# AssafSinger94/dino-tracker

Hardware: AMD Instinct MI355X
Metric: query-points*frames/s (higher is better)
Workload: dtype mixed: fp16 ViT operands (one per value), f16 conv operands in Delta-DINO, f16 candidates + f32 deciders in the tracker; f32 accumulate; 1 GPU; 854x480x90 synthetic video (model res 854x476, 67x121 tokens, C=384), 1024 grid queries; 1 video(s) per step over 1 GPU(s); features=vit, mode=single, track_method=mfma, anchor_pairs=92091, correlation_maps_per_video=8380350, rccl_ranks=1, parallelism=video-parallel x1

## Files before the change

### dino_tracker_amd/_lib.py

```python
from __future__ import annotations

import ctypes
import os

_HERE = os.path.dirname(os.path.abspath(__file__))
LIB_PATH = os.path.join(_HERE, "csrc", "libdtk.so")

c_int, c_float, c_void_p, c_size_t = ctypes.c_int, ctypes.c_float, ctypes.c_void_p, ctypes.c_size_t


class Geom(ctypes.Structure):
    _fields_ = [("T", ctypes.c_int32), ("C", ctypes.c_int32), ("ph", ctypes.c_int32), ("pw", ctypes.c_int32),
                ("video_h", ctypes.c_int32), ("video_w", ctypes.c_int32), ("patch", ctypes.c_int32),
                ("stride", ctypes.c_int32), ("radius", ctypes.c_float)]

    @property
    def HW(self) -> int:
        return self.ph * self.pw


def make_geom(T: int, C: int, video_h: int, video_w: int, patch: int = 14, stride: int = 7, radius: float = 35.0) -> Geom:
    ph = 1 + (video_h - patch) // stride
    pw = 1 + (video_w - patch) // stride
    return Geom(T, C, ph, pw, video_h, video_w, patch, stride, radius)


class VitLayer(ctypes.Structure):
    _fields_ = [(n, c_void_p) for n in ("ln1_w", "ln1_b", "qkv_w", "qkv_b", "proj_w", "proj_b", "ls1", "ln2_w", "ln2_b",
                                        "fc1_w", "fc1_b", "fc2_w", "fc2_b", "ls2",
                                        "qkv_w_lo", "proj_w_lo", "fc1_w_lo", "fc2_w_lo")] + [("w_scale", ctypes.c_float)]


class VitModel(ctypes.Structure):
    _fields_ = [("D", ctypes.c_int32), ("heads", ctypes.c_int32), ("depth", ctypes.c_int32), ("patch", ctypes.c_int32),
                ("stride", ctypes.c_int32), ("ln_eps", ctypes.c_float), ("flags", ctypes.c_int32),
                ("patch_w", c_void_p), ("patch_b", c_void_p),
                ("cls_pos", c_void_p), ("pos", c_void_p), ("mean_std", c_void_p), ("layers", ctypes.POINTER(VitLayer)),
                ("frame_batch", ctypes.c_int32), ("overflow", c_void_p),
                ("tap_out", c_void_p), ("tap_mask", ctypes.c_uint64), ("tap_scale", ctypes.c_float),
                ("ffn", ctypes.c_int32), ("hidden", ctypes.c_int32)]


VIT_TILED_GEMMS, VIT_BF16, VIT_CHECK_RANGE, VIT_GEMM_WS_V1, VIT_ATTENTION_V4, VIT_GEMM_WIDE_V1, VIT_NO_LN_FUSION = 1, 2, 4, 16, 32, 64, 128
OPERAND_F16, OPERAND_BF16, OPERAND_ATTENTION_V4 = 0, 1, 0x2000
VIT_GEMM_QKV, VIT_GEMM_QKV_FACET, VIT_GEMM_PROJ, VIT_GEMM_FC1, VIT_GEMM_FC2 = 0, 1, 2, 3, 4
VIT_GEMM_FC1_SWIGLU, VIT_GEMM_FC2_SWIGLU = 5, 6
VIT_FFN_GELU, VIT_FFN_SWIGLU = 0, 1


class VitGemmArgs(ctypes.Structure):
    _fields_ = ([(n, ctypes.c_int32) for n in ("role", "D", "flags", "operand_type")] + [("rows", ctypes.c_int64)] +
                [("S", ctypes.c_int32), ("Sp", ctypes.c_int32), ("ln_eps", ctypes.c_float), ("w_scale", ctypes.c_float)] +
                [(n, c_void_p) for n in ("a", "a_lo", "w", "w_lo", "bias", "gamma", "q", "k", "vt", "q_lo", "k_lo", "vt_lo", "out",
                                         "out_lo", "out_f32", "x", "ln_x", "ln_w", "ln_b", "ln_out", "ovf")])


class TrackOpts(ctypes.Structure):
    _fields_ = [("method", ctypes.c_int32), ("normalized", ctypes.c_int32), ("round_sources", ctypes.c_int32),
                ("tier", ctypes.c_int32), ("emb_rows", ctypes.c_int32)]


ADAM_MAX_TENSORS, ADAM_MAX_GROUPS = 32, 4


class AdamArgs(ctypes.Structure):
    _fields_ = [("param", ctypes.c_void_p * ADAM_MAX_TENSORS), ("grad", ctypes.c_void_p * ADAM_MAX_TENSORS),
                ("exp_avg", ctypes.c_void_p * ADAM_MAX_TENSORS), ("exp_avg_sq", ctypes.c_void_p * ADAM_MAX_TENSORS),
                ("numel", ctypes.c_int64 * ADAM_MAX_TENSORS), ("group", ctypes.c_int32 * ADAM_MAX_TENSORS),
                ("step", ctypes.c_int32 * ADAM_MAX_TENSORS), ("n_tensors", ctypes.c_int32), ("lr", ctypes.c_double * ADAM_MAX_GROUPS),
                ("beta1", ctypes.c_double), ("beta2", ctypes.c_double), ("eps", ctypes.c_double)]


RAFT_SPLIT, RAFT_FP16 = 0, 1
RAFT_ACT_NONE, RAFT_ACT_RELU, RAFT_ACT_SIGMOID, RAFT_ACT_TANH = 0, 1, 2, 3
RAFT_NUM_CONVS = 48


class RaftConvDesc(ctypes.Structure):
    _fields_ = ([("w_hi", c_void_p), ("w_lo", c_void_p), ("bias", c_void_p)] +
                [(n, ctypes.c_int32) for n in ("cin", "cout", "kh", "kw", "stride", "pad_h", "pad_w")] + [("inv_wscale", c_float)])


class RaftConvArgs(ctypes.Structure):
    _fields_ = ([("conv", RaftConvDesc)] +
                [(n, ctypes.c_int32) for n in ("N", "H", "W", "mode", "act", "res_relu", "in_split", "reserved")] +
                [(n, c_void_p) for n in ("in_", "in2", "out", "res", "mul", "gate")] +
                [(n, ctypes.c_int64) for n in ("in_stride", "in2_stride", "out_stride", "res_stride", "mul_stride", "gate_stride")])


class RaftModel(ctypes.Structure):
    _fields_ = [("conv", RaftConvDesc * RAFT_NUM_CONVS)]


class TrackStats(ctypes.Structure):
    _fields_ = [("sources", ctypes.c_int32), ("whole_map_tier", ctypes.c_int32), ("exact_tier", ctypes.c_int32),
                ("syncs", ctypes.c_int32)]

    def as_dict(self):
        return {k: int(getattr(self, k)) for k, _ in self._fields_}


SIGNATURES = {
    "dtk_version": (c_int, []),
    "dtk_last_error": (ctypes.c_char_p, []),
    "dtk_profile_enable": (c_int, [c_int]),
    "dtk_profile_collect": (c_int, []),
    "dtk_profile_name": (ctypes.c_char_p, [c_int]),
    "dtk_profile_ms": (ctypes.c_double, [c_int]),
    "dtk_profile_launches": (ctypes.c_longlong, [c_int]),
    "dtk_pack_features": (c_int, [c_void_p, c_void_p, c_void_p, c_int, c_int, c_int, c_void_p]),
    "dtk_unpack_features": (c_int, [c_void_p, c_void_p, c_int, c_int, c_int, c_void_p]),
    "dtk_feature_norms": (c_int, [c_void_p, c_void_p, c_int, c_int, c_int, c_void_p]),
    "dtk_vit_workspace_bytes": (c_size_t, [ctypes.POINTER(VitModel), c_int, c_int, c_int]),
    "dtk_vit_forward": (c_int, [ctypes.POINTER(VitModel), c_void_p, c_int, c_int, c_int, c_void_p, c_void_p, c_void_p,
                                c_void_p, c_size_t, c_void_p]),
    "dtk_vit_attention": (c_int, [c_void_p, c_void_p, c_void_p, c_void_p, c_int, c_int, c_int, c_int, c_int, c_void_p]),
    "dtk_vit_attention_split": (c_int, [c_void_p] * 8 + [c_int, c_int, c_int, c_int, c_int, c_void_p]),
    "dtk_vit_gemm": (c_int, [ctypes.POINTER(VitGemmArgs), c_void_p]),
    "dtk_vit_gemm_split": (c_int, [ctypes.POINTER(VitGemmArgs), c_void_p]),
    "dtk_delta_dino_packed_floats": (c_size_t, [c_int, c_int]),
    "dtk_delta_dino_pack": (c_int, [c_int, c_int, c_void_p, c_void_p, c_void_p, c_void_p, c_void_p, c_void_p, c_float,
                                    c_void_p, c_void_p]),
    "dtk_delta_dino_workspace_bytes": (c_size_t, [ctypes.POINTER(Geom)]),
    "dtk_delta_dino_refine": (c_int, [ctypes.POINTER(Geom), c_void_p, c_void_p, ctypes.POINTER(c_void_p), c_void_p,
                                      c_void_p, c_int, c_int, c_void_p, c_size_t, c_void_p]),
    "dtk_delta_dino_refine_mode": (c_int, [ctypes.POINTER(Geom), c_void_p, c_void_p, ctypes.POINTER(c_void_p), c_void_p,
                                           c_void_p, c_int, c_int, c_int, c_void_p, c_size_t, c_void_p]),
    "dtk_sample_points": (c_int, [ctypes.POINTER(Geom), c_void_p, c_void_p, c_void_p, c_void_p, c_void_p, c_int, c_void_p]),
    "dtk_sample_grid": (c_int, [c_void_p, c_int, c_int, c_int, c_int, c_void_p, c_void_p, c_int, c_void_p]),
    "dtk_normalized_conv2d": (c_int, [c_void_p, c_void_p, c_void_p, c_void_p, c_int, c_int, c_int, c_int, c_int, c_int,
                                      c_void_p]),
    "dtk_corr_maps": (c_int, [ctypes.POINTER(Geom), c_void_p, c_void_p, c_void_p, c_void_p, c_void_p, c_void_p, c_void_p,
                              c_int, c_int, c_void_p]),
    "dtk_head_prepare": (c_int, [c_void_p, c_void_p, c_void_p, c_void_p, c_void_p, c_void_p]),
    "dtk_head_forward": (c_int, [ctypes.POINTER(Geom), c_void_p, c_void_p, c_void_p, c_int, c_int, c_void_p]),
    "dtk_head_forward_train": (c_int, [ctypes.POINTER(Geom), c_void_p, c_void_p, c_void_p, c_void_p, c_int, c_int, c_void_p]),
    "dtk_conv_split_weight_halves": (c_size_t, [c_int, c_int]),
    "dtk_conv_split_pack": (c_int, [c_void_p, c_int, c_int, c_int, c_void_p, c_void_p, c_void_p]),
    "dtk_conv_split_input": (c_int, [c_void_p, c_int, c_int, c_int, c_int, c_int, c_void_p, c_void_p, c_void_p, c_void_p]),
    "dtk_conv_split_run": (c_int, [c_void_p, c_void_p, c_void_p, c_void_p, c_void_p, c_int, c_int, c_int, c_int, c_int, c_int,
                                   c_int, c_int, c_void_p]),
    "dtk_conv_split_output": (c_int, [c_void_p, c_int, c_int, c_int, c_int, c_int, c_int, c_void_p, c_void_p, c_void_p]),
    "dtk_conv_wgrad_split_workspace_bytes": (c_size_t, [c_int, c_int, c_int, c_int, c_int, c_int]),
    "dtk_conv_wgrad_split": (c_int, [c_void_p, c_void_p, c_void_p, c_int, c_int, c_int, c_int, c_int, c_int, c_int, c_void_p,
                                     c_int, c_void_p, c_size_t, c_void_p]),
    "dtk_gemm_nt_f32_indexed": (c_int, [c_void_p, c_void_p, c_void_p, c_int, c_int, c_int, ctypes.c_int64, ctypes.c_int64,
                                        ctypes.c_int64, c_int, ctypes.c_int64, ctypes.c_int64, ctypes.c_int64, c_int, c_int,
                                        c_void_p, c_void_p, c_void_p, c_void_p, c_void_p]),
    "dtk_contrastive_workspace_bytes": (c_size_t, [c_int, c_int, c_int, c_int]),
    "dtk_contrastive_forward": (c_int, [c_void_p, c_void_p, c_void_p, ctypes.c_float, c_int, c_int, c_int, c_int, c_int, c_void_p,
                                        c_void_p, c_void_p, c_void_p, c_void_p, c_void_p]),
    "dtk_contrastive_backward": (c_int, [c_void_p, c_void_p, c_void_p, ctypes.c_float, c_int, c_int, c_int, c_int, c_int, c_void_p,
                                         c_void_p, c_void_p, c_void_p, c_void_p, c_void_p, c_void_p, c_void_p, c_size_t, c_void_p]),
    "dtk_emb_reg_forward": (c_int, [c_void_p, c_void_p, c_int, c_int, c_int, c_void_p, c_void_p, c_void_p]),
    "dtk_sample_bilinear_forward": (c_int, [c_void_p, c_void_p, c_void_p, ctypes.c_int32, ctypes.c_int32, ctypes.c_int32, ctypes.c_int32, ctypes.c_int32, c_void_p]),
    "dtk_sample_bilinear_backward": (c_int, [c_void_p, c_void_p, c_void_p, ctypes.c_int32, ctypes.c_int32, ctypes.c_int32, ctypes.c_int32, ctypes.c_int32, c_void_p]),
    "dtk_pow2_scale": (c_int, [c_void_p, ctypes.c_int64, c_void_p, c_void_p, c_void_p]),
    "dtk_adam_step": (c_int, [ctypes.POINTER(AdamArgs), c_void_p]),
    "dtk_adam_scalars": (c_int, [ctypes.POINTER(AdamArgs), ctypes.POINTER(ctypes.c_float)]),
    "dtk_adam_step_dev": (c_int, [ctypes.POINTER(AdamArgs), c_void_p, c_void_p]),
    "dtk_emb_reg_backward": (c_int, [c_void_p, c_void_p, c_void_p, c_void_p, c_int, c_int, c_int, c_void_p, c_void_p]),
    "dtk_corr_window_backward": (c_int, [ctypes.POINTER(Geom), c_void_p, c_void_p, c_void_p, c_void_p, c_void_p, c_void_p, c_void_p,
                                         c_void_p, c_void_p, c_int, c_void_p]),
    "dtk_head_backward": (c_int, [ctypes.POINTER(Geom), c_void_p, c_void_p, c_void_p, c_void_p, c_void_p, c_void_p, c_int, c_int,
                                  c_void_p]),
    "dtk_track_workspace_bytes": (c_size_t, [ctypes.POINTER(Geom), c_int, ctypes.POINTER(TrackOpts)]),
    "dtk_track": (c_int, [ctypes.POINTER(Geom), c_void_p, c_void_p, c_void_p, c_void_p, c_void_p, c_void_p, c_void_p,
                          c_void_p, c_void_p, c_int, c_void_p, ctypes.POINTER(TrackOpts), ctypes.POINTER(TrackStats),
                          c_void_p, c_size_t, c_void_p]),
    "dtk_argmax_cells": (c_int, [ctypes.POINTER(Geom), c_void_p, c_void_p, c_void_p, c_void_p, c_void_p, c_void_p, c_void_p,
                                 c_void_p, c_int, c_int, c_void_p, c_size_t, c_void_p]),
    "dtk_bb_nms_workspace_bytes": (c_size_t, [ctypes.POINTER(Geom), c_int]),
    "dtk_bb_nms": (c_int, [ctypes.POINTER(Geom), c_void_p, c_void_p, c_void_p, c_void_p, c_void_p, c_float, c_float, c_int,
                           c_void_p, c_void_p, c_int, c_void_p, c_size_t, c_void_p]),
    "dtk_traj_start_fg": (c_int, [c_void_p, c_int, c_int, c_void_p, c_int, c_int, c_int, c_void_p, c_void_p, c_void_p]),
    "dtk_nearest_traj_workspace_bytes": (c_size_t, [c_int, c_int, c_int, c_int]),
    "dtk_nearest_traj": (c_int, [c_void_p, c_int, c_int, c_int, c_int, c_float, c_float, c_void_p, c_void_p, c_size_t, c_void_p]),
    "dtk_of_filter_keep": (c_int, [c_void_p, c_int, c_int, c_void_p, c_int, c_int, c_float, c_float, c_void_p, c_void_p,
                                   c_void_p, c_void_p, c_int, c_void_p, c_void_p, c_void_p]),
    "dtk_feat_f16_bytes": (c_size_t, [ctypes.POINTER(Geom)]),
    "dtk_make_feat_f16": (c_int, [ctypes.POINTER(Geom), c_void_p, c_void_p, c_void_p, c_void_p]),
    "dtk_traj_cos_sims": (c_int, [c_void_p, c_void_p, c_void_p, c_int, c_int, c_int, c_void_p]),
    "dtk_build_anchor_sources": (c_int, [c_void_p, c_float, c_int, c_int, c_void_p, c_void_p, c_void_p, c_void_p,
                                         c_void_p, c_void_p, c_void_p, c_void_p, c_void_p]),
    "dtk_occlusion": (c_int, [c_void_p, c_void_p, c_void_p, c_void_p, c_void_p, c_float, c_float, c_void_p, c_int,
                              c_int, c_void_p]),
    "dtk_build_anchor_sources_needed": (c_int, [c_void_p, c_float, c_float, c_int, c_int, c_void_p, c_void_p, c_void_p,
                                                c_void_p, c_void_p, c_void_p, c_void_p, c_void_p, c_void_p]),
    "dtk_occlusion_needed": (c_int, [c_void_p, c_void_p, c_void_p, c_void_p, c_void_p, c_float, c_float, c_void_p, c_int,
                                     c_int, c_void_p]),
    "dtk_tapvid_counts": (c_int, [c_void_p, c_void_p, c_void_p, c_void_p, c_void_p, c_float, c_float, c_float, c_float,
                                  c_int, c_int, c_int, c_void_p, c_void_p]),
    "dtk_badja_counts": (c_int, [c_void_p, c_void_p, c_void_p, c_void_p, c_int, c_float, c_float, c_int, c_int, c_int, c_int, c_int,
                                 c_void_p, c_void_p, c_void_p]),
    "dtk_blurpool_forward": (c_int, [c_void_p, c_void_p, ctypes.c_int64, c_int, c_int, c_void_p]),
    "dtk_blurpool_backward": (c_int, [c_void_p, c_void_p, ctypes.c_int64, c_int, c_int, c_void_p]),
    "dtk_gemm_nt_f32": (c_int, [c_void_p, c_void_p, c_void_p, c_int, c_int, c_int, ctypes.c_int64, ctypes.c_int64, ctypes.c_int64,
                                c_int, ctypes.c_int64, ctypes.c_int64, ctypes.c_int64, c_int, c_int, c_void_p, c_void_p, c_void_p]),
    "dtk_im2col": (c_int, [c_void_p, c_void_p, c_int, c_int, c_int, c_int, c_int, c_int, c_int, c_int, c_int, c_int,
                           ctypes.c_int64, c_void_p]),
    "dtk_col2im": (c_int, [c_void_p, c_void_p, c_int, c_int, c_int, c_int, c_int, c_int, c_int, c_int, c_int, c_void_p]),
    "dtk_transpose_f32": (c_int, [c_void_p, c_void_p, ctypes.c_int64, ctypes.c_int64, c_int, c_void_p]),
    "dtk_resample2d_forward": (c_int, [c_void_p, c_void_p, ctypes.c_int64, c_int, c_int, c_int, c_int, c_void_p, c_void_p, c_void_p,
                                       c_void_p, c_void_p]),
    "dtk_resample2d_backward": (c_int, [c_void_p, c_void_p, ctypes.c_int64, c_int, c_int, c_int, c_int, c_void_p, c_void_p,
                                        c_void_p, c_void_p, c_void_p]),
    "dtk_batchnorm_workspace_bytes": (c_size_t, [c_int]),
    "dtk_batchnorm_train_forward": (c_int, [c_void_p, c_void_p, c_void_p, c_void_p, c_void_p, c_void_p, c_float, c_float,
                                            c_int, c_void_p, c_void_p, c_void_p, c_int, c_int, c_int, c_void_p, c_size_t,
                                            c_void_p]),
    "dtk_batchnorm_train_backward": (c_int, [c_void_p, c_void_p, c_void_p, c_void_p, c_void_p, c_void_p, c_int, c_void_p,
                                             c_void_p, c_void_p, c_void_p, c_int, c_int, c_int, c_void_p, c_size_t, c_void_p]),
    "dtk_pca_moments_workspace_bytes": (c_size_t, [ctypes.c_int64, c_int, ctypes.c_int64]),
    "dtk_pca_moments": (c_int, [c_void_p, ctypes.c_int64, c_int, c_int, ctypes.c_int64, c_void_p, c_void_p, c_void_p, c_size_t,
                                c_void_p]),
    "dtk_pca_project_workspace_bytes": (c_size_t, [ctypes.c_int64]),
    "dtk_pca_project": (c_int, [c_void_p, ctypes.c_int64, c_int, c_int, c_void_p, c_int, c_void_p, c_void_p, c_void_p, c_size_t,
                                c_void_p]),
    "dtk_fg_mask": (c_int, [c_void_p, c_int, c_int, c_void_p, c_float, c_int, c_int, c_int, c_int, c_int, c_int, c_void_p, c_void_p,
                            c_void_p]),
    "dtk_flow_pack": (c_int, [c_void_p, c_void_p, c_int, c_int, c_int, c_void_p]),
    "dtk_flow_cycle_masks": (c_int, [c_void_p, c_void_p, c_int, c_int, c_int, c_float, c_void_p, c_void_p]),
    "dtk_flow_traj_workspace_bytes": (c_size_t, [c_int, c_int, c_int]),
    "dtk_flow_traj_start": (c_int, [c_void_p, c_void_p, c_void_p, c_void_p, c_int, c_int, c_int, c_int, c_float, c_int, c_void_p,
                                    c_void_p, c_int, c_float, c_void_p, c_void_p, c_size_t, c_void_p]),
    "dtk_flow_traj_emit": (c_int, [c_int, c_int, c_int, c_int, c_int, c_int, c_void_p, c_void_p, c_void_p, c_size_t, c_void_p]),
    "dtk_render_prim_count": (ctypes.c_int64, [c_int, c_int, c_int, c_int]),
    "dtk_render_group_bytes": (c_size_t, [ctypes.c_int64, ctypes.c_int64, c_int, c_int, c_int]),
    "dtk_render_prims": (c_int, [c_void_p, c_void_p, c_void_p, c_void_p, c_int, c_int, c_int, c_int, c_int, c_int, c_int, c_int,
                                 c_float, c_float, c_int, c_void_p, c_void_p]),
    "dtk_render_pred_gt_prims": (c_int, [c_void_p, c_void_p, c_void_p, c_void_p, c_void_p, c_int, c_int, c_int, c_int, c_int,
                                         c_int, c_int, c_void_p, c_void_p]),
    "dtk_render_tile_counts": (c_int, [c_void_p, ctypes.c_int64, c_int, c_int, c_int, c_void_p, c_void_p]),
    "dtk_render_tile_keys": (c_int, [c_void_p, c_void_p, ctypes.c_int64, c_int, c_int, c_int, ctypes.c_int64, c_void_p, c_void_p]),
    "dtk_render_blend": (c_int, [c_void_p, c_void_p, ctypes.c_int64, c_void_p, ctypes.c_int64, c_void_p, c_int, c_int, c_int,
                                 c_void_p, c_void_p, c_void_p]),
    "dtk_resize_workspace_bytes": (c_size_t, [c_int, c_int, c_int, c_int, c_int, c_int, c_int, c_int]),
    "dtk_resize_u8": (c_int, [c_void_p, c_int, c_int, c_int, c_int, c_int, c_int, c_void_p, c_void_p, c_int, c_void_p, c_void_p, c_int,
                              c_void_p, c_int, c_int, c_void_p, c_void_p, c_size_t, c_void_p]),
    "dtk_raft_conv_packed_halves": (c_size_t, [c_int, c_int, c_int, c_int]),
    "dtk_raft_conv_pack": (c_int, [c_void_p, c_int, c_int, c_int, c_int, c_float, c_void_p, c_void_p, c_void_p]),
    "dtk_raft_conv": (c_int, [ctypes.POINTER(RaftConvArgs), c_void_p]),
    "dtk_raft_instance_norm_workspace_bytes": (c_size_t, [c_int, c_int, c_int, c_int]),
    "dtk_raft_instance_norm": (c_int, [c_void_p, c_void_p, c_void_p, c_int, c_int, c_int, c_int, c_float, c_int, c_void_p, c_size_t,
                                       c_void_p]),
    "dtk_raft_pyramid_floats": (c_size_t, [c_int, c_int, c_int]),
    "dtk_raft_corr_pyramid": (c_int, [c_void_p, c_void_p, c_int, c_int, c_int, c_int, c_int, c_void_p, c_void_p]),
    "dtk_raft_lookup": (c_int, [c_void_p, c_void_p, ctypes.c_int64, c_int, c_int, c_int, c_void_p, ctypes.c_int64, c_void_p]),
    "dtk_raft_upsample": (c_int, [c_void_p, ctypes.c_int64, c_void_p, c_int, c_int, c_int, c_void_p, c_void_p]),
    "dtk_raft_workspace_bytes": (c_size_t, [c_int, c_int, c_int]),
    "dtk_raft_forward": (c_int, [ctypes.POINTER(RaftModel), c_void_p, c_void_p, c_int, c_int, c_int, c_int, c_int, c_void_p, c_void_p,
                                 c_size_t, c_void_p]),
}

_LIB = None


def lib() -> ctypes.CDLL:
    global _LIB
    if _LIB is None:
        if not os.path.isfile(LIB_PATH):
            raise RuntimeError(
                f"{LIB_PATH} is missing: build the HIP extension first (python -c 'import __graft_entry__ as g; "
                "g.build()' or make -C dino_tracker_amd/csrc). There is no CPU fallback for the hot path.")
        handle = ctypes.CDLL(LIB_PATH)
        for name, (res, args) in SIGNATURES.items():
            fn = getattr(handle, name)
            fn.restype = res
            fn.argtypes = args
        _LIB = handle
    return _LIB


def check(rc: int) -> None:
    if rc != 0:
        raise RuntimeError(f"libdtk error {rc}: {lib().dtk_last_error().decode()}")
```

### dino_tracker_amd/csrc/vit.hip

```cpp
#include <stdlib.h>
#include "common.h"
#include "vit_attention4.h"
#include "vit_attention6.h"
#include "vit_gemm_common.h"
#include "vit_gemm_tiled.h"
#include "vit_gemm_ws.h"
#include "vit_gemm_ws_ln.h"
#include "vit_gemm_wide.h"
#include "vit_split.h"

namespace {

__global__ __launch_bounds__(256) void patch_embed_kernel(const float* __restrict__ frames, const float* __restrict__ Wp,
                                                          const float* __restrict__ bp, const float* __restrict__ pos,
                                                          const float* __restrict__ cls_pos,
                                                          const float* __restrict__ mean_std, float* __restrict__ x,
                                                          int H, int W, int ph, int pw, int D, int patch, int stride,
                                                          int S) {
    const int HW = ph * pw;
    const int K = 3 * patch * patch;
    const int frame = blockIdx.z;
    const int tid = threadIdx.x, lane = tid & 63, w = tid >> 6;
    const int p0 = blockIdx.x * 64 + (w >> 1) * 32;
    const int n0 = blockIdx.y * 64 + (w & 1) * 32;
    const int li = lane & 31, lk = lane >> 5;
    const float* img = frames + (size_t)frame * 3 * H * W;
    const int p = min(p0 + li, HW - 1);
    const int pr = p / pw, pc = p % pw;
    const int n = min(n0 + li, D - 1);
    const float* wrow = Wp + (size_t)n * K;
    f16v acc;
#pragma unroll
    for (int r = 0; r < 16; ++r) acc[r] = 0.f;
    for (int k = lk; k < K; k += 2) {
        const int ch = k / (patch * patch), rem = k - ch * patch * patch;
        const int ky = rem / patch, kx = rem - ky * patch;
        const float px = img[((size_t)ch * H + pr * stride + ky) * W + pc * stride + kx];
        const float a = (px - mean_std[ch]) / mean_std[3 + ch];
        acc = __builtin_amdgcn_mfma_f32_32x32x2f32(a, wrow[k], acc, 0, 0, 0);
    }
    const int co = n0 + li;
    if (co < D) {
        const float b = bp[co];
#pragma unroll
        for (int r = 0; r < 16; ++r) {
            const int i = (r & 3) + 8 * (r >> 2) + 4 * lk;
            const int pp = p0 + i;
            if (pp < HW) x[((size_t)frame * S + 1 + pp) * D + co] = acc[r] + b + pos[(size_t)pp * D + co];
        }
    }
    if (blockIdx.x == 0 && (w >> 1) == 0 && lk == 0 && co < D) x[(size_t)frame * S * D + co] = cls_pos[co];
}

constexpr int PE_P = 14, PE_S = 7, PE_TOK = 128, PE_NF = 96;
constexpr int PE_ROWPX = (PE_TOK - 1) * PE_S + PE_P;
constexpr int PE_K = PE_P * PE_P * 4;
constexpr int PE_CK = 2 * PE_P * 4;
constexpr int PE_WP = PE_CK + 8;
constexpr float PE_WSCALE = 256.f;

__global__ __launch_bounds__(256) void frame_split4_kernel(const float* __restrict__ frames, const float* __restrict__ mean_std,
                                                           h4v* __restrict__ hi_, h4v* __restrict__ lo_, int H, int W,
                                                           long long npix) {
    const long long i = (long long)blockIdx.x * 256 + threadIdx.x;
    if (i >= npix) return;
    const long long f = i / ((long long)H * W), p = i - f * (long long)H * W;
    const float* fr = frames + f * 3 * (long long)H * W + p;
    h4v h, l;
#pragma unroll
    for (int c = 0; c < 3; ++c) {
        const float v = (fr[(long long)c * H * W] - mean_std[c]) / mean_std[3 + c];
        h[c] = (half_t)v;
        l[c] = (half_t)(v - (float)h[c]);
    }
    h[3] = (half_t)0.f;
    l[3] = (half_t)0.f;
    hi_[i] = h;
    lo_[i] = l;
}

__global__ void pack_patch_split_kernel(const float* __restrict__ w, int D, half_t* __restrict__ Wh, half_t* __restrict__ Wl) {
    const long long idx = (long long)blockIdx.x * 256 + threadIdx.x;
    if (idx >= (long long)D * PE_K) return;
    const int n = (int)(idx / PE_K), k = (int)(idx - (long long)n * PE_K);
    const int tap = k >> 2, c = k & 3;
    const float v = c < 3 ? w[((size_t)n * 3 + c) * (PE_P * PE_P) + tap] * PE_WSCALE : 0.f;
    const half_t h = (half_t)v;
    Wh[idx] = h;
    Wl[idx] = (half_t)(v - (float)h);
}

__global__ __launch_bounds__(256) void patch_embed_split_kernel(const h4v* __restrict__ in_hi, const h4v* __restrict__ in_lo,
                                                                const half_t* __restrict__ Wh, const half_t* __restrict__ Wl,
                                                                const float* __restrict__ bp, const float* __restrict__ pos,
                                                                const float* __restrict__ cls_pos, float* __restrict__ x,
                                                                int H, int W, int ph, int pw, int D, int S, int groups_x,
                                                                int units, int slabs) {
    __shared__ h4v Xh[2 * PE_ROWPX], Xl[2 * PE_ROWPX];
    __shared__ __attribute__((aligned(16))) half_t Wsh[PE_NF * PE_WP], Wsl[PE_NF * PE_WP];
    const int tid = threadIdx.x, lane = tid & 63, w = tid >> 6;
    const int per_xcd = (units + 7) / 8;
    const int within = blockIdx.x >> 3;
    const int unit = (blockIdx.x & 7) * per_xcd + within / slabs;
    if (within / slabs >= per_xcd || unit >= units) return;
    const int n0 = (within % slabs) * PE_NF;
    const int pc0 = (unit % groups_x) * PE_TOK, pr = (unit / groups_x) % ph;
    const size_t frame = unit / (groups_x * ph);
    const int li = lane & 31, hh = lane >> 5;
    const h4v* fh = in_hi + frame * (size_t)H * W;
    const h4v* fl = in_lo + frame * (size_t)H * W;
    const int tokl = w * 32 + li;
    f16v acc[3];
#pragma unroll
    for (int n = 0; n < 3; ++n)
#pragma unroll
        for (int r = 0; r < 16; ++r) acc[n][r] = 0.f;
    for (int c = 0; c < PE_P / 2; ++c) {
        __syncthreads();
        for (int idx = tid; idx < 2 * PE_ROWPX; idx += 256) {
            const int r = idx / PE_ROWPX, px = idx - r * PE_ROWPX;
            const size_t g = (size_t)(pr * PE_S + 2 * c + r) * W + min(pc0 * PE_S + px, W - 1);
            Xh[idx] = fh[g];
            Xl[idx] = fl[g];
        }
        for (int idx = tid; idx < PE_NF * (PE_CK / 8); idx += 256) {
            const int f = idx / (PE_CK / 8), piece = idx - f * (PE_CK / 8);
            const size_t src = (size_t)min(n0 + f, D - 1) * PE_K + c * PE_CK + piece * 8;
            *reinterpret_cast<uint4*>(Wsh + f * PE_WP + piece * 8) = *reinterpret_cast<const uint4*>(Wh + src);
            *reinterpret_cast<uint4*>(Wsl + f * PE_WP + piece * 8) = *reinterpret_cast<const uint4*>(Wl + src);
        }
        __syncthreads();
#pragma unroll
        for (int ls = 0; ls < PE_CK / 16; ++ls) {
            const int t0 = 2 * (2 * ls + hh);
            const int p0 = (t0 / PE_P) * PE_ROWPX + tokl * PE_S + t0 % PE_P;
            const h4v a0 = Xh[p0], a1 = Xh[p0 + 1], b0 = Xl[p0], b1 = Xl[p0 + 1];
            const h8 xh = {a0[0], a0[1], a0[2], a0[3], a1[0], a1[1], a1[2], a1[3]};
            const h8 xl = {b0[0], b0[1], b0[2], b0[3], b1[0], b1[1], b1[2], b1[3]};
#pragma unroll
            for (int n = 0; n < 3; ++n) {
                const int wo = (n * 32 + li) * PE_WP + ls * 16 + hh * 8;
                const h8 wh = *reinterpret_cast<const h8*>(Wsh + wo), wl = *reinterpret_cast<const h8*>(Wsl + wo);
                acc[n] = __builtin_amdgcn_mfma_f32_32x32x16_f16(xl, wh, acc[n], 0, 0, 0);
                acc[n] = __builtin_amdgcn_mfma_f32_32x32x16_f16(xh, wl, acc[n], 0, 0, 0);
                acc[n] = __builtin_amdgcn_mfma_f32_32x32x16_f16(xh, wh, acc[n], 0, 0, 0);
            }
        }
    }
#pragma unroll
    for (int n = 0; n < 3; ++n) {
        const int co = n0 + n * 32 + li;
        if (co >= D) continue;
        const float b = bp[co];
#pragma unroll
        for (int r = 0; r < 16; ++r) {
            const int pc = pc0 + w * 32 + (r & 3) + 8 * (r >> 2) + 4 * hh;
            if (pc < pw) {
                const int pp = pr * pw + pc;
                x[((size_t)frame * S + 1 + pp) * D + co] = acc[n][r] * (1.f / PE_WSCALE) + b + pos[(size_t)pp * D + co];
            }
        }
        if (pr == 0 && pc0 == 0 && w == 0 && hh == 0) x[(size_t)frame * S * D + co] = cls_pos[co];
    }
}

template <typename T, int NIT = 4>
__global__ __launch_bounds__(256) void layernorm_kernel(float* __restrict__ x, const T* __restrict__ delta,
                                                        const float* __restrict__ gam, const float* __restrict__ bet,
                                                        T* __restrict__ y, long long rows, int D, float eps,
                                                        int* __restrict__ overflow) {
    typedef typename Vec<T>::t8 T8;
    typedef typename Vec<T>::t4 T4;
    (void)sizeof(T8); (void)sizeof(T4);
    operand_mode<T>();
    const long long row = (long long)blockIdx.x * 4 + (threadIdx.x >> 6);
    if (row >= rows) return;
    const int lane = threadIdx.x & 63;
    float* p = x + row * D;
    float4 v[NIT];
    float s = 0.f;
    bool sat = false;
#pragma unroll
    for (int it = 0; it < NIT; ++it) {
        const int c = lane * 4 + it * 256;
        if (c < D) {
            v[it] = *reinterpret_cast<const float4*>(p + c);
            if (delta) {
                const T4 d = *reinterpret_cast<const T4*>(delta + row * D + c);
                const float d0 = (float)d[0], d1 = (float)d[1], d2 = (float)d[2], d3 = (float)d[3];
                if (IsF16<T>::value) sat |= !(fmaxf(fmaxf(fabsf(d0), fabsf(d1)), fmaxf(fabsf(d2), fabsf(d3))) < 65504.f);
                v[it].x += d0; v[it].y += d1; v[it].z += d2; v[it].w += d3;
                *reinterpret_cast<float4*>(p + c) = v[it];
            }
            s += (v[it].x + v[it].y) + (v[it].z + v[it].w);
        }
    }
    if (IsF16<T>::value && overflow && __any(sat) && lane == 0) atomicOr(overflow, 1);
    const float mean = wave_sum(s) / (float)D;
    float q = 0.f;
#pragma unroll
    for (int it = 0; it < NIT; ++it) {
        if (lane * 4 + it * 256 < D) {
            const float a = v[it].x - mean, b = v[it].y - mean, cc = v[it].z - mean, d = v[it].w - mean;
            q += (a * a + b * b) + (cc * cc + d * d);
        }
    }
    const float rstd = rsqrtf(wave_sum(q) / (float)D + eps);
    if (!y) return;
    T* o = y + row * D;
#pragma unroll
    for (int it = 0; it < NIT; ++it) {
        const int c = lane * 4 + it * 256;
        if (c < D) {
            const float4 g = *reinterpret_cast<const float4*>(gam + c), b = *reinterpret_cast<const float4*>(bet + c);
            T4 r = {(T)((v[it].x - mean) * rstd * g.x + b.x), (T)((v[it].y - mean) * rstd * g.y + b.y),
                     (T)((v[it].z - mean) * rstd * g.z + b.z), (T)((v[it].w - mean) * rstd * g.w + b.w)};
            *reinterpret_cast<T4*>(o + c) = r;
        }
    }
}

__global__ __launch_bounds__(256) void zero_kernel(uint4* __restrict__ p, long long n16) {
    const long long i = (long long)blockIdx.x * 256 + threadIdx.x;
    if (i < n16) p[i] = make_uint4(0, 0, 0, 0);
}

template <typename T>
__global__ __launch_bounds__(256) void final_update_kernel(const float* __restrict__ x, const T* __restrict__ delta,
                                                           float* __restrict__ tokens_out, float* __restrict__ feat_out, int S, int D,
                                                           long long total4, int* __restrict__ overflow) {
    typedef typename Vec<T>::t4 T4;
    const long long i = (long long)blockIdx.x * 256 + threadIdx.x;
    bool sat = false;
    if (i < total4) {
        const int d4 = D / 4;
        const long long row = i / d4;
        const int c = (int)(i - row * d4);
        const long long f = row / S, s = row - f * S;
        float4 v = reinterpret_cast<const float4*>(x)[i];
        const T4 d = reinterpret_cast<const T4*>(delta)[i];
        const float d0 = (float)d[0], d1 = (float)d[1], d2 = (float)d[2], d3 = (float)d[3];
        if (IsF16<T>::value) sat = !(fmaxf(fmaxf(fabsf(d0), fabsf(d1)), fmaxf(fabsf(d2), fabsf(d3))) < 65504.f);
        v.x += d0; v.y += d1; v.z += d2; v.w += d3;
        if (tokens_out) reinterpret_cast<float4*>(tokens_out)[i] = v;
        if (feat_out && s > 0) reinterpret_cast<float4*>(feat_out)[(f * (S - 1) + s - 1) * d4 + c] = v;
    }
    if (IsF16<T>::value && overflow && __any(sat) && (threadIdx.x & 63) == 0) atomicOr(overflow, 1);
}

template <typename T>
__global__ __launch_bounds__(256) void tap_kernel(const float* __restrict__ x, const T* __restrict__ delta, float* __restrict__ out,
                                                  float scale, long long total4) {
    typedef typename Vec<T>::t4 T4;
    const long long i = (long long)blockIdx.x * 256 + threadIdx.x;
    if (i >= total4) return;
    float4 v = reinterpret_cast<const float4*>(x)[i];
    if (delta) {
        const T4 d = reinterpret_cast<const T4*>(delta)[i];
        v.x += (float)d[0]; v.y += (float)d[1]; v.z += (float)d[2]; v.w += (float)d[3];
    }
    float4 o = reinterpret_cast<float4*>(out)[i];
    o.x += scale * v.x; o.y += scale * v.y; o.z += scale * v.z; o.w += scale * v.w;
    reinterpret_cast<float4*>(out)[i] = o;
}

__global__ __launch_bounds__(256) void drop_cls_kernel(const float* __restrict__ x, float* __restrict__ out, int S, int D,
                                                       long long total4) {
    const long long i = (long long)blockIdx.x * 256 + threadIdx.x;
    if (i >= total4) return;
    const int d4 = D / 4;
    const long long row = i / d4;
    const int c = (int)(i - row * d4);
    const long long f = row / (S - 1), s = row - f * (S - 1);
    reinterpret_cast<float4*>(out)[i] = reinterpret_cast<const float4*>(x)[(f * S + 1 + s) * d4 + c];
}

constexpr int VIT_FRAME_BATCH = 90;

struct VitPlan {
    int S, Sp, FB;
    size_t x, xn, q, k, vt, ao, hid, delta, total;
    bool split;
    size_t xn_lo, q_lo, k_lo, vt_lo, ao_lo, hid_lo;
};

inline bool vit_layer_split(const dtk_vit_layer& L) { return L.qkv_w_lo != nullptr; }

VitPlan vit_plan(const dtk_vit_model* m, int ph, int pw, int frames) {
    VitPlan p;
    p.S = ph * pw + 1;
    p.Sp = (p.S + 127) / 128 * 128;
    const int fb = m->frame_batch > 0 ? m->frame_batch : VIT_FRAME_BATCH;
    p.FB = frames < fb ? frames : fb;
    auto al = [](size_t v) { return (v + 255) & ~(size_t)255; };
    size_t off = 0;
    const size_t rows = (size_t)p.FB * p.S;
    p.x = off; off = al(off + rows * m->D * 4);
    p.xn = off; off = al(off + rows * m->D * 2);
    p.q = off; off = al(off + (size_t)p.FB * m->heads * p.Sp * 64 * 2);
    p.k = off; off = al(off + (size_t)p.FB * m->heads * p.Sp * 64 * 2);
    p.vt = off; off = al(off + (size_t)p.FB * m->heads * p.Sp * 64 * 2);
    p.ao = off; off = al(off + rows * m->D * 2);
    p.hid = off; off = al(off + rows * 4 * m->D * 2);
    p.delta = off; off = al(off + rows * m->D * 2);
    p.split = false;
    for (int l = 0; l < m->depth; ++l) p.split |= vit_layer_split(m->layers[l]);
    p.xn_lo = p.q_lo = p.k_lo = p.vt_lo = p.ao_lo = p.hid_lo = 0;
    if (p.split) {
        p.xn_lo = off; off = al(off + rows * m->D * 2);
        p.q_lo = off; off = al(off + (size_t)p.FB * m->heads * p.Sp * 64 * 2);
        p.k_lo = off; off = al(off + (size_t)p.FB * m->heads * p.Sp * 64 * 2);
        p.vt_lo = off; off = al(off + (size_t)p.FB * m->heads * p.Sp * 64 * 2);
        p.ao_lo = off; off = al(off + rows * m->D * 2);
        p.hid_lo = off; off = al(off + rows * 4 * m->D * 2);
    }
    p.total = off;
    return p;
}

template <typename T>
int attention_launch(const T* q, const T* k, const T* vt, T* o, int S, int Sp, int heads, int D, int FH, bool v4, hipStream_t st) {
    int QB;
    if (v4) {
        const unsigned grid = attn::attention_grid(FH, S, 256, &QB);
        DTK_LAUNCH("vit_attention", (attn::attention4_kernel<T, 0>), dim3(grid), dim3(256), 0, st, q, k, vt, o, S, Sp, heads, D,
                   FH, QB);
    } else {
        const unsigned grid = attn::attention_grid(FH, S, 128 * attn::A6_NQ, &QB);
        DTK_LAUNCH("vit_attention", (attn::attention6_kernel<T, 0>), dim3(grid), dim3(256), 0, st, q, k, vt, o, S, Sp, heads, D,
                   FH, QB);
    }
    return DTK_OK;
}

template <typename T>
__global__ __launch_bounds__(256) void range_scan_kernel(const T* __restrict__ p, long long n8, int* __restrict__ flag, int bit) {
    typedef typename Vec<T>::t8 T8;
    bool bad = false;
    for (long long i = (long long)blockIdx.x * 256 + threadIdx.x; i < n8; i += (long long)gridDim.x * 256) {
        const T8 v = reinterpret_cast<const T8*>(p)[i];
#pragma unroll
        for (int e = 0; e < 8; ++e) bad |= !(fabsf((float)v[e]) < 65504.f);
    }
    if (__any(bad) && (threadIdx.x & 63) == 0) atomicOr(flag, bit);
}

constexpr int VIT_MAX_D = 1536;
template <typename T>
int launch_layernorm(float* x, const T* delta, const float* gam, const float* bet, T* y, long long rows, int D, float eps, int* ovf,
                     hipStream_t st) {
    if (D <= 1024)
        DTK_LAUNCH("vit_layernorm", (layernorm_kernel<T, 4>), dim3(dtk_cdiv(rows, 4)), dim3(256), 0, st, x, delta, gam, bet, y, rows, D, eps, ovf);
    else
        DTK_LAUNCH("vit_layernorm", (layernorm_kernel<T, 6>), dim3(dtk_cdiv(rows, 4)), dim3(256), 0, st, x, delta, gam, bet, y, rows, D, eps, ovf);
    return DTK_OK;
}
template <typename T>
int launch_layernorm_split(float* x, const T* delta, const float* gam, const float* bet, T* y_hi, T* y_lo, long long rows, int D,
                           float eps, int* ovf, hipStream_t st) {
    if (D <= 1024)
        DTK_LAUNCH("vit_layernorm_split", (layernorm_split_kernel<T, 4>), dim3(dtk_cdiv(rows, 4)), dim3(256), 0, st, x, delta, gam, bet, y_hi,
                   y_lo, rows, D, eps, ovf);
    else
        DTK_LAUNCH("vit_layernorm_split", (layernorm_split_kernel<T, 6>), dim3(dtk_cdiv(rows, 4)), dim3(256), 0, st, x, delta, gam, bet, y_hi,
                   y_lo, rows, D, eps, ovf);
    return DTK_OK;
}

struct GemmPath {
    bool tiled;
    bool ws;
    bool wide;
    bool ws_v1;
    bool wide_v1;
    bool fc2_ln;
    bool proj_ln;
};
inline GemmPath gemm_path(int D, int f) {
    const bool tiled = (f & DTK_VIT_TILED_GEMMS) != 0, ws = !tiled && D == WS_K, wide_v1 = (f & DTK_VIT_GEMM_WIDE_V1) != 0;
    static_assert(WS_K == WD_N, "fc2 of the weight-stationary width is gemm_wide_delta_kernel's shape");
    const bool ws_v1 = (f & DTK_VIT_GEMM_WS_V1) != 0, fc2_ln = ws && !wide_v1 && !(f & DTK_VIT_NO_LN_FUSION);
    return {tiled, ws, !tiled && D % W2_N == 0, ws_v1, wide_v1, fc2_ln, fc2_ln && !ws_v1};
}
inline GemmPath gemm_path(const dtk_vit_model* m) { return gemm_path(m->D, m->flags); }

template <typename T, int EPI>
int launch_gemm(const char* name, const GemmPath& path, const T* A, const T* W, long long rows, int N, int K, const GemmEpi<T>& e,
                hipStream_t st) {
    if constexpr (EPI != EPI_F32) {
        const bool ws_fits = EPI != EPI_QKV || e.S >= WS_ROWS || rows <= e.S;
        if constexpr (EPI == EPI_DELTA) {
            if (path.ws && K == WS_K && N == WS_K && e.ln_out) {
                const auto gr = gemm_ws_ln_grid(rows);
                DTK_LAUNCH(name, (gemm_ws_ln_kernel<T>), gr.first, dim3(256), 0, st, A, W, rows, e, gr.second);
                return DTK_OK;
            }
        }
        if (path.ws && K == WS_K && ws_fits) {
            const auto gr = gemm_ws_grid(N, rows);
            if (path.ws_v1)
                DTK_LAUNCH(name, (gemm_ws_kernel<T, EPI, 0>), gr.first, dim3(256), 0, st, A, W, rows, N, e, gr.second);
            else if (N % 64 != 0 || DTK_DBG(e.no_store, 128))
                DTK_LAUNCH(name, (gemm_ws_kernel<T, EPI, 3, false>), gr.first, dim3(256), 0, st, A, W, rows, N, e, gr.second);
            else
                DTK_LAUNCH(name, (gemm_ws_kernel<T, EPI>), gr.first, dim3(256), 0, st, A, W, rows, N, e, gr.second);
            return DTK_OK;
        }
        if (path.ws && EPI == EPI_DELTA) {
            const dim3 grid(dtk_cdiv(rows, WD_M));
            if (path.wide_v1)
                DTK_LAUNCH(name, (gemm_wide_delta_kernel<T, false>), grid, dim3(512), 0, st, A, W, rows, K, e);
            else if (e.ln_out)
                DTK_LAUNCH(name, (gemm_wide_delta_kernel<T, true, true>), grid, dim3(512), 0, st, A, W, rows, K, e);
            else
                DTK_LAUNCH(name, (gemm_wide_delta_kernel<T, true>), grid, dim3(512), 0, st, A, W, rows, K, e);
            return DTK_OK;
        }
        if (path.wide) {
            const dim3 grid(gemm_wide_grid(N, rows));
            if (path.wide_v1)
                DTK_LAUNCH(name, (gemm_wide_kernel<T, EPI, false>), grid, dim3(512), 0, st, A, W, rows, N, K, e);
            else
                DTK_LAUNCH(name, (gemm_wide_kernel<T, EPI, true>), grid, dim3(512), 0, st, A, W, rows, N, K, e);
            return DTK_OK;
        }
    }
    DTK_LAUNCH(name, (gemm_tiled_kernel<T, EPI>), dim3(gemm_grid(N, rows)), dim3(256), 0, st, A, W, rows, N, K, e);
    return DTK_OK;
}

template <typename T>
int launch_gemm_swiglu(const char* name, const GemmPath& path, const T* A, const T* W, long long rows, int N, int K, const GemmEpi<T>& e,
                       hipStream_t st) {
    if (path.wide)
        DTK_LAUNCH(name, (gemm_wide_kernel<T, EPI_SWIGLU, true>), dim3(gemm_wide_grid(N, rows)), dim3(512), 0, st, A, W, rows, N, K, e);
    else
        DTK_LAUNCH(name, (gemm_tiled_kernel<T, EPI_SWIGLU>), dim3(gemm_grid(N, rows)), dim3(256), 0, st, A, W, rows, N, K, e);
    return DTK_OK;
}
inline bool vit_swiglu_flags_ok(int flags, const char* who) {
    if (!(flags & (DTK_VIT_GEMM_WIDE_V1 | DTK_VIT_GEMM_WS_V1))) return true;
    dtk_set_error("%s: the SwiGLU feed-forward has no A / B kernel forms: clear %s", who,
                  (flags & DTK_VIT_GEMM_WIDE_V1) ? "DTK_VIT_GEMM_WIDE_V1" : "DTK_VIT_GEMM_WS_V1");
    return false;
}

template <typename T, int SEPI>
int launch_gemm_split(const char* name, const GemmPath& path, const T* Ah, const T* Al, const T* Wh, const T* Wl, long long rows,
                      int N, int K, const SplitEpi<T>& se, hipStream_t st) {
    if (!path.tiled && N % SD_N == 0) {
        const dim3 grid(gemm_split_dma_grid(N, rows));
        if constexpr (SEPI == SEPI_SWIGLU)
            DTK_LAUNCH(name, (gemm_split_dma_kernel<T, SEPI, true>), grid, dim3(512), 0, st, Ah, Al, Wh, Wl, rows, N, K, se);
        else if (path.wide_v1)
            DTK_LAUNCH(name, (gemm_split_dma_kernel<T, SEPI, false>), grid, dim3(512), 0, st, Ah, Al, Wh, Wl, rows, N, K, se);
        else
            DTK_LAUNCH(name, (gemm_split_dma_kernel<T, SEPI, true>), grid, dim3(512), 0, st, Ah, Al, Wh, Wl, rows, N, K, se);
        return DTK_OK;
    }
    DTK_LAUNCH(name, (gemm_split_kernel<T, SEPI>), dim3(gemm_split_grid(N, rows)), dim3(256), 0, st, Ah, Al, Wh, Wl, rows, N, K, se);
    return DTK_OK;
}

template <typename T>
int vit_run(const dtk_vit_model* m, const float* frames, int nframes, int video_h, int video_w, float* tokens_out,
            float* feat_out, float* qkv_out, unsigned char* ws, const VitPlan& p, int ph, int pw, hipStream_t st) {
    const int HW = ph * pw, D = m->D;
    const bool swiglu = m->ffn == DTK_VIT_FFN_SWIGLU;
    const int HID = m->hidden > 0 ? m->hidden : 4 * D;
    float* x = reinterpret_cast<float*>(ws + p.x);
    auto at = [&](size_t off) { return reinterpret_cast<T*>(ws + off); };
    T *xn = at(p.xn), *q = at(p.q), *k = at(p.k), *vt = at(p.vt), *ao = at(p.ao), *hid = at(p.hid), *delta = at(p.delta);
    T *xn_lo = at(p.xn_lo), *q_lo = at(p.q_lo), *k_lo = at(p.k_lo), *vt_lo = at(p.vt_lo), *ao_lo = at(p.ao_lo), *hid_lo = at(p.hid_lo);
    int* ovf = m->overflow;
    const bool scan_all = ovf && (m->flags & DTK_VIT_CHECK_RANGE);
    int* const epi_ovf = IsF16<T>::value ? ovf : nullptr;
    const int S = p.S, Sp = p.Sp;
    {
        const long long n16 = (long long)((p.ao - p.q) / 16);
        DTK_LAUNCH("vit_zero", zero_kernel, dim3(dtk_cdiv(n16, 256)), dim3(256), 0, st, reinterpret_cast<uint4*>(q), n16);
        if (p.split) {
            const long long m16 = (long long)((p.ao_lo - p.q_lo) / 16);
            DTK_LAUNCH("vit_zero", zero_kernel, dim3(dtk_cdiv(m16, 256)), dim3(256), 0, st, reinterpret_cast<uint4*>(q_lo), m16);
        }
    }
    for (int f0 = 0; f0 < nframes; f0 += p.FB) {
        const int nf = (nframes - f0) < p.FB ? (nframes - f0) : p.FB;
        const long long rows = (long long)nf * S;
        auto scan_range = [&](const T* t, long long n, int bit) -> int {
            const int blocks = (int)(dtk_cdiv(n / 8, 256) < 1024 ? dtk_cdiv(n / 8, 256) : 1024);
            DTK_LAUNCH("vit_range_scan", range_scan_kernel<T>, dim3(blocks), dim3(256), 0, st, t, n / 8, ovf, bit);
            return DTK_OK;
        };
        const bool pe_fits = (size_t)nf * video_h * video_w * 16 <= p.delta - p.hid &&
                             (size_t)D * PE_K * 4 <= p.total - p.delta;
        if (m->patch == PE_P && m->stride == PE_S && pe_fits) {
            h4v* fh = reinterpret_cast<h4v*>(hid);
            h4v* fl = fh + (size_t)nf * video_h * video_w;
            half_t* wh = reinterpret_cast<half_t*>(delta);
            half_t* wl = wh + (size_t)D * PE_K;
            const long long npix = (long long)nf * video_h * video_w;
            DTK_LAUNCH("vit_frame_split", frame_split4_kernel, dim3(dtk_cdiv(npix, 256)), dim3(256), 0, st,
                       frames + (size_t)f0 * 3 * video_h * video_w, m->mean_std, fh, fl, video_h, video_w, npix);
            DTK_LAUNCH("vit_frame_split", pack_patch_split_kernel, dim3(dtk_cdiv((long long)D * PE_K, 256)), dim3(256), 0, st,
                       m->patch_w, D, wh, wl);
            const int groups_x = dtk_cdiv(pw, PE_TOK);
            const int units = groups_x * ph * nf, slabs = dtk_cdiv(D, PE_NF);
            DTK_LAUNCH("vit_patch_embed", patch_embed_split_kernel, dim3(8 * dtk_cdiv(units, 8) * slabs), dim3(256), 0, st, fh,
                       fl, wh, wl, m->patch_b, m->pos, m->cls_pos, x, video_h, video_w, ph, pw, D, S, groups_x, units, slabs);
        } else {
            DTK_LAUNCH("vit_patch_embed", patch_embed_kernel, dim3(dtk_cdiv(HW, 64), dtk_cdiv(D, 64), nf), dim3(256), 0, st,
                       frames + (size_t)f0 * 3 * video_h * video_w, m->patch_w, m->patch_b, m->pos, m->cls_pos, m->mean_std,
                       x, video_h, video_w, ph, pw, D, m->patch, m->stride, S);
        }
        const GemmPath path = gemm_path(m);
        const int dbg_ns = DTK_DBG(dtk_dev_flags() >> 16, 0xff);
        bool pending = false;
        bool ln1_done = false;
        auto tap = [&](int l, bool with_delta) -> int {
            if (!m->tap_out || !((m->tap_mask >> l) & 1)) return DTK_OK;
            const long long t4 = rows * (D / 4);
            DTK_LAUNCH("vit_tap", tap_kernel<T>, dim3(dtk_cdiv(t4, 256)), dim3(256), 0, st, x, with_delta ? (const T*)delta : (const T*)nullptr,
                       m->tap_out + (size_t)f0 * S * D, m->tap_scale, t4);
            return DTK_OK;
        };
        for (int l = 0; l < m->depth; ++l) {
            const dtk_vit_layer& L = m->layers[l];
            const T* qkv_w = reinterpret_cast<const T*>(L.qkv_w);
            const T* proj_w = reinterpret_cast<const T*>(L.proj_w);
            const T* fc1_w = reinterpret_cast<const T*>(L.fc1_w);
            const T* fc2_w = reinterpret_cast<const T*>(L.fc2_w);
            if (vit_layer_split(L)) {
                const T* qkv_wl = reinterpret_cast<const T*>(L.qkv_w_lo);
                const T* proj_wl = reinterpret_cast<const T*>(L.proj_w_lo);
                const T* fc1_wl = reinterpret_cast<const T*>(L.fc1_w_lo);
                const T* fc2_wl = reinterpret_cast<const T*>(L.fc2_w_lo);
                const float inv_ws = 1.f / (L.w_scale > 0.f ? L.w_scale : 1.f);
                if (launch_layernorm_split<T>(x, pending ? (const T*)delta : (const T*)nullptr, L.ln1_w, L.ln1_b, xn, xn_lo, rows, D, m->ln_eps,
                                              ovf, st)) return DTK_E_HIP;
                pending = false;
                SplitEpi<T> se{};
                if (qkv_out && l == m->depth - 1) {
                    se.bias = L.qkv_b; se.inv_wscale = inv_ws; se.out_f32 = qkv_out + (size_t)f0 * S * 3 * D;
                    if (launch_gemm_split<T, SEPI_F32>("vit_gemm_qkv_facet", path, xn, xn_lo, qkv_w, qkv_wl, rows, 3 * D, D, se, st)) return DTK_E_HIP;
                    se = SplitEpi<T>{};
                }
                se.bias = L.qkv_b; se.inv_wscale = inv_ws; se.q_hi = q; se.q_lo = q_lo; se.k_hi = k; se.k_lo = k_lo; se.vt_hi = vt;
                se.vt_lo = vt_lo; se.S = S; se.Sp = Sp; se.heads = m->heads; se.D = D; se.qscale = 0.125f * 1.4426950408889634f;
                se.ovf = epi_ovf;
                if (launch_gemm_split<T, SEPI_QKV>("vit_gemm_qkv_split", path, xn, xn_lo, qkv_w, qkv_wl, rows, 3 * D, D, se, st)) return DTK_E_HIP;
                const int nqb = dtk_cdiv(Sp, 128);
                DTK_LAUNCH("vit_attention_split", attention_split_kernel<T>, dim3((unsigned)(nf * m->heads * nqb)), dim3(256), 0, st,
                           (const T*)q, (const T*)q_lo, (const T*)k, (const T*)k_lo, (const T*)vt, (const T*)vt_lo, ao, ao_lo, S, Sp,
                           m->heads, nqb);
                se = SplitEpi<T>{};
                se.bias = L.proj_b; se.inv_wscale = inv_ws; se.x = x; se.gamma = L.ls1;
                if (launch_gemm_split<T, SEPI_RESID>("vit_gemm_proj_split", path, ao, ao_lo, proj_w, proj_wl, rows, D, D, se, st)) return DTK_E_HIP;
                if (launch_layernorm_split<T>(x, (const T*)nullptr, L.ln2_w, L.ln2_b, xn, xn_lo, rows, D, m->ln_eps, ovf, st)) return DTK_E_HIP;
                se = SplitEpi<T>{};
                se.bias = L.fc1_b; se.inv_wscale = inv_ws; se.out_hi = hid; se.out_lo = hid_lo; se.ovf = epi_ovf;
                if (swiglu ? launch_gemm_split<T, SEPI_SWIGLU>("vit_gemm_fc1_split", path, xn, xn_lo, fc1_w, fc1_wl, rows, 2 * HID, D, se, st)
                           : launch_gemm_split<T, SEPI_GELU>("vit_gemm_fc1_split", path, xn, xn_lo, fc1_w, fc1_wl, rows, HID, D, se, st)) return DTK_E_HIP;
                se = SplitEpi<T>{};
                se.bias = L.fc2_b; se.inv_wscale = inv_ws; se.x = x; se.gamma = L.ls2;
                if (launch_gemm_split<T, SEPI_RESID>("vit_gemm_fc2_split", path, hid, hid_lo, fc2_w, fc2_wl, rows, D, HID, se, st)) return DTK_E_HIP;
                if (tap(l, false)) return DTK_E_HIP;
                continue;
            }
            GemmEpi<T> e{};
            if (!ln1_done && launch_layernorm<T>(x, pending ? (const T*)delta : (const T*)nullptr, L.ln1_w, L.ln1_b, xn, rows, D, m->ln_eps, ovf, st))
                return DTK_E_HIP;
            ln1_done = false;
            pending = true;
            if (qkv_out && l == m->depth - 1) {
                e.bias = L.qkv_b; e.out_f32 = qkv_out + (size_t)f0 * S * 3 * D;
                if (launch_gemm<T, EPI_F32>("vit_gemm_qkv_facet", path, xn, qkv_w, rows, 3 * D, D, e, st)) return DTK_E_HIP;
                e = GemmEpi<T>{};
            }
            e.bias = L.qkv_b; e.q = q; e.k = k; e.vt = vt; e.S = S; e.Sp = Sp; e.heads = m->heads; e.D = D;
            e.qscale = 0.125f * 1.4426950408889634f; e.no_store = dbg_ns; e.ovf = epi_ovf;
            if (launch_gemm<T, EPI_QKV>("vit_gemm_qkv", path, xn, qkv_w, rows, 3 * D, D, e, st)) return DTK_E_HIP;
            if (scan_all && scan_range(q, (long long)(p.ao - p.q) / 2, 2)) return DTK_E_HIP;
            if (attention_launch(q, k, vt, ao, S, Sp, m->heads, D, nf * m->heads, (m->flags & DTK_VIT_ATTENTION_V4) != 0, st)) return DTK_E_HIP;
            e = GemmEpi<T>{};
            e.bias = L.proj_b; e.delta = delta; e.gamma = L.ls1; e.no_store = dbg_ns;
            if (path.proj_ln) { e.ln_x = x; e.ln_w = L.ln2_w; e.ln_b = L.ln2_b; e.ln_out = xn; e.ln_eps = m->ln_eps; e.ln_ovf = ovf; }
            if (launch_gemm<T, EPI_DELTA>("vit_gemm_proj", path, ao, proj_w, rows, D, D, e, st)) return DTK_E_HIP;
            if (!path.proj_ln && launch_layernorm<T>(x, (const T*)delta, L.ln2_w, L.ln2_b, xn, rows, D, m->ln_eps, ovf, st)) return DTK_E_HIP;
            e = GemmEpi<T>{};
            e.bias = L.fc1_b; e.out = hid; e.no_store = dbg_ns; e.ovf = epi_ovf;
            if (swiglu ? launch_gemm_swiglu<T>("vit_gemm_fc1", path, xn, fc1_w, rows, 2 * HID, D, e, st)
                       : launch_gemm<T, EPI_GELU>("vit_gemm_fc1", path, xn, fc1_w, rows, HID, D, e, st)) return DTK_E_HIP;
            if (scan_all && scan_range(hid, rows * HID, 4)) return DTK_E_HIP;
            e = GemmEpi<T>{};
            e.bias = L.fc2_b; e.delta = delta; e.gamma = L.ls2; e.no_store = dbg_ns;
            if (path.fc2_ln && l + 1 < m->depth && !vit_layer_split(m->layers[l + 1])) {
                const dtk_vit_layer& Ln = m->layers[l + 1];
                e.ln_x = x; e.ln_w = Ln.ln1_w; e.ln_b = Ln.ln1_b; e.ln_out = xn; e.ln_eps = m->ln_eps; e.ln_ovf = ovf;
                pending = false;
                ln1_done = true;
            }
            if (launch_gemm<T, EPI_DELTA>("vit_gemm_fc2", path, hid, fc2_w, rows, D, HID, e, st)) return DTK_E_HIP;
            if (tap(l, pending)) return DTK_E_HIP;
        }
        if (pending && (tokens_out || feat_out)) {
            const long long t4 = rows * (D / 4);
            DTK_LAUNCH("vit_final_update", final_update_kernel<T>, dim3(dtk_cdiv(t4, 256)), dim3(256), 0, st, x, (const T*)delta,
                       tokens_out ? tokens_out + (size_t)f0 * S * D : (float*)nullptr,
                       feat_out ? feat_out + (size_t)f0 * HW * D : (float*)nullptr, S, D, t4, ovf);
        } else {
            if (pending &&
                launch_layernorm<T>(x, (const T*)delta, (const float*)nullptr, (const float*)nullptr, (T*)nullptr, rows, D, m->ln_eps, ovf, st))
                return DTK_E_HIP;
            if (tokens_out)
                DTK_HIP(hipMemcpyAsync(tokens_out + (size_t)f0 * S * D, x, (size_t)rows * D * sizeof(float),
                                       hipMemcpyDeviceToDevice, st));
            if (feat_out) {
                const long long total4 = (long long)nf * HW * (D / 4);
                DTK_LAUNCH("vit_drop_cls", drop_cls_kernel, dim3(dtk_cdiv(total4, 256)), dim3(256), 0, st, x,
                           feat_out + (size_t)f0 * HW * D, S, D, total4);
            }
        }
    }
    return DTK_OK;
}

constexpr int VITG_HIDDEN = 4096;
int vit_gemm_check(const dtk_vit_gemm_args* g, const char* who, bool split, int* N, int* K) {
    DTK_REQUIRE(g, "%s: null pointer", who);
    DTK_REQUIRE(g->D == 384 || g->D == 768 || g->D == 1024 || g->D == 1536, "%s: D must be 384, 768 or 1024, or ViT-g's 1536 (got %d)", who, g->D);
    DTK_REQUIRE(g->operand_type == DTK_OPERAND_F16 || g->operand_type == DTK_OPERAND_BF16, "%s: operand_type", who);
    DTK_REQUIRE(g->rows > 0 && g->rows < (1ll << 31), "%s: rows", who);
    DTK_REQUIRE(g->a && g->w && (!split || (g->a_lo && g->w_lo)), "%s: null operand", who);
    const int D = g->D;
    switch (g->role) {
        case DTK_VIT_GEMM_QKV:
            *N = 3 * D; *K = D;
            DTK_REQUIRE(g->q && g->k && g->vt && (!split || (g->q_lo && g->k_lo && g->vt_lo)), "%s: QKV needs q, k and vt", who);
            DTK_REQUIRE(g->S > 0 && g->Sp >= g->S && g->Sp % 64 == 0 && g->rows % g->S == 0,
                        "%s: bad sizes (Sp %% 64 == 0, Sp >= S, rows a multiple of S)", who);
            break;
        case DTK_VIT_GEMM_QKV_FACET:
            *N = 3 * D; *K = D;
            DTK_REQUIRE(g->out_f32, "%s: QKV_FACET needs out_f32", who);
            break;
        case DTK_VIT_GEMM_FC1:
            *N = 4 * D; *K = D;
            DTK_REQUIRE(g->out && (!split || g->out_lo), "%s: FC1 needs out", who);
            break;
        case DTK_VIT_GEMM_PROJ:
        case DTK_VIT_GEMM_FC2:
            *N = D; *K = g->role == DTK_VIT_GEMM_FC2 ? 4 * D : D;
            DTK_REQUIRE(g->gamma && (split ? g->x != nullptr : g->out != nullptr), "%s: PROJ / FC2 need gamma and %s", who, split ? "x" : "out");
            break;
        case DTK_VIT_GEMM_FC1_SWIGLU:
        case DTK_VIT_GEMM_FC2_SWIGLU:
            DTK_REQUIRE(D == 1536, "%s: the SwiGLU roles are ViT-g's, D = 1536 (got %d)", who, D);
            if (!vit_swiglu_flags_ok(g->flags, who)) return DTK_E_INVALID;
            if (g->role == DTK_VIT_GEMM_FC1_SWIGLU) {
                *N = 2 * VITG_HIDDEN; *K = D;
                DTK_REQUIRE(g->out && (!split || g->out_lo), "%s: FC1_SWIGLU needs out", who);
            } else {
                *N = D; *K = VITG_HIDDEN;
                DTK_REQUIRE(g->gamma && (split ? g->x != nullptr : g->out != nullptr), "%s: FC2_SWIGLU needs gamma and %s", who, split ? "x" : "out");
            }
            break;
        default:
            DTK_REQUIRE(false, "%s: unknown role %d", who, g->role);
    }
    return DTK_OK;
}

template <typename T>
int vit_gemm_stage(const dtk_vit_gemm_args* g, int N, int K, hipStream_t st) {
    const GemmPath path = gemm_path(g->D, g->flags);
    const T *A = reinterpret_cast<const T*>(g->a), *W = reinterpret_cast<const T*>(g->w);
    int* const epi_ovf = IsF16<T>::value ? g->ovf : nullptr;
    GemmEpi<T> e{};
    e.bias = g->bias;
    switch (g->role) {
        case DTK_VIT_GEMM_QKV:
            e.q = reinterpret_cast<T*>(g->q); e.k = reinterpret_cast<T*>(g->k); e.vt = reinterpret_cast<T*>(g->vt);
            e.S = g->S; e.Sp = g->Sp; e.heads = g->D / 64; e.D = g->D; e.qscale = 0.125f * 1.4426950408889634f; e.ovf = epi_ovf;
            return launch_gemm<T, EPI_QKV>("vit_gemm_qkv", path, A, W, g->rows, N, K, e, st);
        case DTK_VIT_GEMM_QKV_FACET:
            e.out_f32 = g->out_f32;
            return launch_gemm<T, EPI_F32>("vit_gemm_qkv_facet", path, A, W, g->rows, N, K, e, st);
        case DTK_VIT_GEMM_FC1:
            e.out = reinterpret_cast<T*>(g->out); e.ovf = epi_ovf;
            return launch_gemm<T, EPI_GELU>("vit_gemm_fc1", path, A, W, g->rows, N, K, e, st);
        case DTK_VIT_GEMM_FC1_SWIGLU:
            e.out = reinterpret_cast<T*>(g->out); e.ovf = epi_ovf;
            return launch_gemm_swiglu<T>("vit_gemm_fc1", path, A, W, g->rows, N, K, e, st);
        default:
            e.delta = reinterpret_cast<T*>(g->out); e.gamma = g->gamma;
            if (g->ln_out) {
                DTK_REQUIRE(g->role == DTK_VIT_GEMM_PROJ ? path.proj_ln : path.fc2_ln,
                            "dtk_vit_gemm: the fused LayerNorm is fc2's or the projection's at D = 384 without TILED_GEMMS / GEMM_WIDE_V1 / NO_LN_FUSION (the projection's: nor GEMM_WS_V1)");
                DTK_REQUIRE(g->ln_x && g->ln_w && g->ln_b, "dtk_vit_gemm: the fused LayerNorm needs ln_x, ln_w and ln_b");
                e.ln_x = g->ln_x; e.ln_w = g->ln_w; e.ln_b = g->ln_b; e.ln_out = reinterpret_cast<T*>(g->ln_out); e.ln_eps = g->ln_eps;
                e.ln_ovf = g->ovf;
            }
            return launch_gemm<T, EPI_DELTA>(g->role == DTK_VIT_GEMM_PROJ ? "vit_gemm_proj" : "vit_gemm_fc2", path, A, W, g->rows, N, K, e, st);
    }
}

template <typename T>
int vit_gemm_split_stage(const dtk_vit_gemm_args* g, int N, int K, hipStream_t st) {
    const GemmPath path = gemm_path(g->D, g->flags);
    const T *Ah = reinterpret_cast<const T*>(g->a), *Al = reinterpret_cast<const T*>(g->a_lo);
    const T *Wh = reinterpret_cast<const T*>(g->w), *Wl = reinterpret_cast<const T*>(g->w_lo);
    int* const epi_ovf = IsF16<T>::value ? g->ovf : nullptr;
    SplitEpi<T> se{};
    se.bias = g->bias; se.inv_wscale = 1.f / (g->w_scale > 0.f ? g->w_scale : 1.f);
    switch (g->role) {
        case DTK_VIT_GEMM_QKV:
            se.q_hi = reinterpret_cast<T*>(g->q); se.q_lo = reinterpret_cast<T*>(g->q_lo); se.k_hi = reinterpret_cast<T*>(g->k);
            se.k_lo = reinterpret_cast<T*>(g->k_lo); se.vt_hi = reinterpret_cast<T*>(g->vt); se.vt_lo = reinterpret_cast<T*>(g->vt_lo);
            se.S = g->S; se.Sp = g->Sp; se.heads = g->D / 64; se.D = g->D; se.qscale = 0.125f * 1.4426950408889634f; se.ovf = epi_ovf;
            return launch_gemm_split<T, SEPI_QKV>("vit_gemm_qkv_split", path, Ah, Al, Wh, Wl, g->rows, N, K, se, st);
        case DTK_VIT_GEMM_QKV_FACET:
            se.out_f32 = g->out_f32;
            return launch_gemm_split<T, SEPI_F32>("vit_gemm_qkv_facet", path, Ah, Al, Wh, Wl, g->rows, N, K, se, st);
        case DTK_VIT_GEMM_FC1:
            se.out_hi = reinterpret_cast<T*>(g->out); se.out_lo = reinterpret_cast<T*>(g->out_lo); se.ovf = epi_ovf;
            return launch_gemm_split<T, SEPI_GELU>("vit_gemm_fc1_split", path, Ah, Al, Wh, Wl, g->rows, N, K, se, st);
        case DTK_VIT_GEMM_FC1_SWIGLU:
            se.out_hi = reinterpret_cast<T*>(g->out); se.out_lo = reinterpret_cast<T*>(g->out_lo); se.ovf = epi_ovf;
            return launch_gemm_split<T, SEPI_SWIGLU>("vit_gemm_fc1_split", path, Ah, Al, Wh, Wl, g->rows, N, K, se, st);
        default:
            se.x = g->x; se.gamma = g->gamma;
            return launch_gemm_split<T, SEPI_RESID>(g->role == DTK_VIT_GEMM_PROJ ? "vit_gemm_proj_split" : "vit_gemm_fc2_split", path, Ah, Al,
                                                    Wh, Wl, g->rows, N, K, se, st);
    }
}

constexpr int VIT_KNOWN_FLAGS = DTK_VIT_TILED_GEMMS | DTK_VIT_BF16 | DTK_VIT_CHECK_RANGE | DTK_VIT_GEMM_WS_V1 | DTK_VIT_ATTENTION_V4 |
                                DTK_VIT_GEMM_WIDE_V1 | DTK_VIT_NO_LN_FUSION;

}

extern "C" size_t dtk_vit_workspace_bytes(const dtk_vit_model* m, int video_h, int video_w, int frames) {
    if (!m || frames <= 0) return 0;
    const int ph = 1 + (video_h - m->patch) / m->stride, pw = 1 + (video_w - m->patch) / m->stride;
    return vit_plan(m, ph, pw, frames).total;
}

extern "C" int dtk_vit_forward(const dtk_vit_model* m, const float* frames, int nframes, int video_h, int video_w,
                               float* tokens_out, float* feat_out, float* qkv_out, void* workspace,
                               size_t workspace_bytes, void* stream) {
    DTK_REQUIRE(m && frames && workspace && (tokens_out || feat_out || qkv_out || m->tap_out), "dtk_vit_forward: null pointer");
    DTK_REQUIRE(!(m->flags & ~VIT_KNOWN_FLAGS), "dtk_vit_forward: unknown flag bits 0x%x (bit 8 selected a kernel that left the library)",
                (unsigned)(m->flags & ~VIT_KNOWN_FLAGS));
    DTK_REQUIRE(!qkv_out || m->depth > 0, "dtk_vit_forward: qkv_out needs at least one block");
    DTK_REQUIRE(m->D > 0 && m->heads > 0 && m->D == m->heads * 64, "dtk_vit_forward: d_head must be 64 (D=%d heads=%d)",
                m->D, m->heads);
    DTK_REQUIRE(m->D % 32 == 0 && m->depth >= 0 && m->layers, "dtk_vit_forward: bad model");
    DTK_REQUIRE(m->D <= VIT_MAX_D, "dtk_vit_forward: D = %d: the LayerNorm kernels hold rows of at most %d channels", m->D, VIT_MAX_D);
    if (m->ffn == DTK_VIT_FFN_SWIGLU) {
        DTK_REQUIRE(m->D == 1536 && m->hidden == VITG_HIDDEN, "dtk_vit_forward: the SwiGLU feed-forward is ViT-g's: D = 1536, hidden = %d (got D = %d, hidden = %d)",
                    VITG_HIDDEN, m->D, m->hidden);
        if (!vit_swiglu_flags_ok(m->flags, "dtk_vit_forward")) return DTK_E_INVALID;
    } else {
        DTK_REQUIRE(m->ffn == DTK_VIT_FFN_GELU, "dtk_vit_forward: unknown ffn %d", m->ffn);
        DTK_REQUIRE(m->hidden == 0 || m->hidden == 4 * m->D, "dtk_vit_forward: a GELU MLP has hidden = 4 D (got %d)", m->hidden);
    }
    DTK_REQUIRE(video_h >= m->patch && video_w >= m->patch, "dtk_vit_forward: frame smaller than a patch");
    const int ph = 1 + (video_h - m->patch) / m->stride, pw = 1 + (video_w - m->patch) / m->stride;
    const VitPlan p = vit_plan(m, ph, pw, nframes);
    if (workspace_bytes < p.total) {
        dtk_set_error("dtk_vit_forward: workspace %zu B < required %zu B", workspace_bytes, p.total);
        return DTK_E_WORKSPACE;
    }
    hipStream_t st = dtk_stream(stream);
    unsigned char* ws = reinterpret_cast<unsigned char*>(workspace);
    if (m->flags & DTK_VIT_BF16)
        return vit_run<__bf16>(m, frames, nframes, video_h, video_w, tokens_out, feat_out, qkv_out, ws, p, ph, pw, st);
    return vit_run<_Float16>(m, frames, nframes, video_h, video_w, tokens_out, feat_out, qkv_out, ws, p, ph, pw, st);
}

extern "C" int dtk_vit_attention(const void* q, const void* k, const void* vt, void* out, int frames, int heads, int S,
                                 int Sp, int operand_type, void* stream) {
    DTK_REQUIRE(q && k && vt && out, "dtk_vit_attention: null pointer");
    DTK_REQUIRE(frames > 0 && heads > 0 && S > 0 && Sp >= S && Sp % 64 == 0, "dtk_vit_attention: bad sizes (Sp %% 64 == 0, Sp >= S)");
    const bool v4 = (operand_type & DTK_OPERAND_ATTENTION_V4) != 0;
    operand_type &= ~DTK_OPERAND_ATTENTION_V4;
    DTK_REQUIRE(operand_type == DTK_OPERAND_F16 || operand_type == DTK_OPERAND_BF16, "dtk_vit_attention: operand_type");
    if (operand_type == DTK_OPERAND_BF16)
        return attention_launch(reinterpret_cast<const __bf16*>(q), reinterpret_cast<const __bf16*>(k),
                                reinterpret_cast<const __bf16*>(vt), reinterpret_cast<__bf16*>(out), S, Sp, heads, heads * 64,
                                frames * heads, v4, dtk_stream(stream));
    return attention_launch(reinterpret_cast<const _Float16*>(q), reinterpret_cast<const _Float16*>(k),
                            reinterpret_cast<const _Float16*>(vt), reinterpret_cast<_Float16*>(out), S, Sp, heads, heads * 64,
                            frames * heads, v4, dtk_stream(stream));
}

extern "C" int dtk_vit_attention_split(const void* q_hi, const void* q_lo, const void* k_hi, const void* k_lo, const void* vt_hi,
                                       const void* vt_lo, void* out_hi, void* out_lo, int frames, int heads, int S, int Sp,
                                       int operand_type, void* stream) {
    DTK_REQUIRE(q_hi && q_lo && k_hi && k_lo && vt_hi && vt_lo && out_hi && out_lo, "dtk_vit_attention_split: null pointer");
    DTK_REQUIRE(frames > 0 && heads > 0 && S > 0 && Sp >= S && Sp % 64 == 0, "dtk_vit_attention_split: bad sizes (Sp %% 64 == 0, Sp >= S)");
    DTK_REQUIRE(operand_type == DTK_OPERAND_F16 || operand_type == DTK_OPERAND_BF16, "dtk_vit_attention_split: operand_type");
    hipStream_t st = dtk_stream(stream);
    const int nqb = dtk_cdiv(Sp, 128);
    const unsigned grid = (unsigned)(frames * heads * nqb);
    if (operand_type == DTK_OPERAND_BF16) {
        typedef __bf16 T;
        DTK_LAUNCH("vit_attention_split", attention_split_kernel<T>, dim3(grid), dim3(256), 0, st, (const T*)q_hi, (const T*)q_lo,
                   (const T*)k_hi, (const T*)k_lo, (const T*)vt_hi, (const T*)vt_lo, (T*)out_hi, (T*)out_lo, S, Sp, heads, nqb);
    } else {
        typedef _Float16 T;
        DTK_LAUNCH("vit_attention_split", attention_split_kernel<T>, dim3(grid), dim3(256), 0, st, (const T*)q_hi, (const T*)q_lo,
                   (const T*)k_hi, (const T*)k_lo, (const T*)vt_hi, (const T*)vt_lo, (T*)out_hi, (T*)out_lo, S, Sp, heads, nqb);
    }
    return DTK_OK;
}


extern "C" int dtk_vit_gemm(const dtk_vit_gemm_args* g, void* stream) {
    int N = 0, K = 0;
    if (const int rc = vit_gemm_check(g, "dtk_vit_gemm", false, &N, &K)) return rc;
    if (g->operand_type == DTK_OPERAND_BF16) return vit_gemm_stage<__bf16>(g, N, K, dtk_stream(stream));
    return vit_gemm_stage<_Float16>(g, N, K, dtk_stream(stream));
}

extern "C" int dtk_vit_gemm_split(const dtk_vit_gemm_args* g, void* stream) {
    int N = 0, K = 0;
    if (const int rc = vit_gemm_check(g, "dtk_vit_gemm_split", true, &N, &K)) return rc;
    DTK_REQUIRE(!g->ln_out, "dtk_vit_gemm_split: the split blocks have their own LayerNorm");
    if (g->operand_type == DTK_OPERAND_BF16) return vit_gemm_split_stage<__bf16>(g, N, K, dtk_stream(stream));
    return vit_gemm_split_stage<_Float16>(g, N, K, dtk_stream(stream));
}
```

### dino_tracker_amd/csrc/vit_attention6.h

```cpp
#pragma once
#include "vit_attention_common.h"

namespace attn {

constexpr int A6_NQ = 4;

template <typename T>
__device__ __forceinline__ void a6_s_first(f16v& acc, const typename Operand<T>::v8& a, const typename Operand<T>::v8& b,
                                           const f16v& c) {
    if constexpr (Operand<T>::F16) asm volatile("v_mfma_f32_32x32x16_f16 %0, %1, %2, %3" : "=&v"(acc) : "a"(a), "a"(b), "v"(c));
    else asm volatile("v_mfma_f32_32x32x16_bf16 %0, %1, %2, %3" : "=&v"(acc) : "a"(a), "a"(b), "v"(c));
}
template <typename T>
__device__ __forceinline__ void a6_s_next(f16v& acc, const typename Operand<T>::v8& a, const typename Operand<T>::v8& b) {
    if constexpr (Operand<T>::F16) asm volatile("v_mfma_f32_32x32x16_f16 %0, %1, %2, %0" : "+v"(acc) : "a"(a), "a"(b));
    else asm volatile("v_mfma_f32_32x32x16_bf16 %0, %1, %2, %0" : "+v"(acc) : "a"(a), "a"(b));
}
template <typename T>
__device__ __forceinline__ void a6_pv(f16v& c, const typename Operand<T>::v8& a, const typename Operand<T>::v8& b) {
    if constexpr (Operand<T>::F16) asm volatile("v_mfma_f32_32x32x16_f16 %0, %1, %2, %0" : "+a"(c) : "a"(a), "v"(b));
    else asm volatile("v_mfma_f32_32x32x16_bf16 %0, %1, %2, %0" : "+a"(c) : "a"(a), "v"(b));
}
template <int OFF, typename V8>
__device__ __forceinline__ void a6_lds_frag(V8& dst, unsigned addr) {
    asm volatile("ds_read_b128 %0, %1 offset:%2" : "=a"(dst) : "v"(addr), "i"(OFF) : "memory");
}

template <typename T, int ABL = 0>
__global__ __launch_bounds__(256, 1) void attention6_kernel(const T* __restrict__ Q, const T* __restrict__ Kg,
                                                            const T* __restrict__ Vt, T* __restrict__ O, int S, int Sp,
                                                            int heads, int D, int FH, int QB) {
    typedef Operand<T> Op;
    typedef typename Op::v8 op8;
    typedef typename Op::v4 op4;
    typedef typename Op::v2 op2;
    constexpr int NQ = A6_NQ;
    __shared__ __attribute__((aligned(1024))) unsigned char tiles[A4_NB][TILE_BYTES];
    const int tid = threadIdx.x, lane = tid & 63;
    const int w = __builtin_amdgcn_readfirstlane(tid >> 6);
    const int xcd = blockIdx.x & 7, seq = blockIdx.x >> 3;
    const int fh = (seq / QB) * 8 + xcd;
    const int qb = seq % QB;
    if (fh >= FH) return;
    const int frame = fh / heads, head = fh - frame * heads;
    const int q0 = qb * (128 * NQ) + w * (32 * NQ);
    const int lq = lane & 31, hi = lane >> 5;
    const T* Qb = Q + (size_t)fh * Sp * 64;
    const T* Kb = Kg + (size_t)fh * Sp * 64;
    const T* Vb = Vt + (size_t)fh * 64 * Sp;
    if (Op::F16) dtk_fp16_saturate_mode();

    op8 qf[NQ][4];
#pragma unroll
    for (int qt = 0; qt < NQ; ++qt) {
        const int qrow = min(q0 + qt * 32 + lq, Sp - 1);
#pragma unroll
        for (int ks = 0; ks < 4; ++ks)
            asm volatile("global_load_dwordx4 %0, %1, off" : "=a"(qf[qt][ks]) : "v"(Qb + (size_t)qrow * 64 + ks * 16 + hi * 8) : "memory");
    }
    op8 kq[2 + NQ][4];
    if (!(ABL & 8)) {
#pragma unroll
        for (int blk = 0; blk < 2 + NQ; ++blk) {
            const int kr0 = blk < 2 ? blk * 32 : q0 + (blk - 2) * 32;
            const T* kp = Kb + (size_t)min(kr0 + lq, Sp - 1) * 64 + hi * 8;
#pragma unroll
            for (int ks = 0; ks < 4; ++ks) kq[blk][ks] = *reinterpret_cast<const op8*>(kp + ks * 16);
        }
    }
    unsigned kvo[2], vvo[2];
#pragma unroll
    for (int r = 0; r < 2; ++r) {
        const int lrow = (w * 2 + r) * 8 + (lane >> 3), lpc = (lane & 7) ^ ((lrow >> 1) & 7);
        kvo[r] = (unsigned)(lrow * 64 + lpc * 8) * 2u;
        vvo[r] = (unsigned)(lrow * Sp + lpc * 8) * 2u;
    }
    const unsigned lds_base = (unsigned)(size_t)&tiles[0][0];
    const int ntiles = (S + 63) / 64;
    const dtk_u4 srd_k = dtk_make_srd(Kb), srd_v = dtk_make_srd(Vb);
    unsigned dma_dst[4];
#pragma unroll
    for (int i = 0; i < 4; ++i) dma_dst[i] = __builtin_amdgcn_readfirstlane(lds_base + (i >> 1) * 8192 + (w * 2 + (i & 1)) * 1024);
    auto issue_one = [&](int t, auto buf_tag, int i) {
        constexpr int BUF = decltype(buf_tag)::value;
        const unsigned tt = (unsigned)min(t, ntiles - 1);
        if (i < 2) dtk_buffer_lds16<BUF * TILE_BYTES>(srd_k, tt * 8192u, kvo[i & 1], dma_dst[i]);
        else dtk_buffer_lds16<BUF * TILE_BYTES>(srd_v, tt * 128u, vvo[i & 1], dma_dst[i]);
    };
#pragma unroll
    for (int j = 0; j < 4; ++j) {
        issue_one(0, std::integral_constant<int, 0>{}, j);
        issue_one(1, std::integral_constant<int, 1>{}, j);
        issue_one(2, std::integral_constant<int, 2>{}, j);
    }
    static_assert(A4_AHEAD == 3 && A4_NB == 4, "prologue requests tiles 0..2 into a ring of four");
    asm volatile("s_waitcnt vmcnt(0)" ::: "memory");
#pragma unroll
    for (int qt = 0; qt < NQ; ++qt)
#pragma unroll
        for (int ks = 0; ks < 4; ++ks) asm volatile("" : "+a"(qf[qt][ks]));
    __syncthreads();

    float m_run[NQ], l_run[NQ];
#pragma unroll
    for (int qt = 0; qt < NQ; ++qt) { m_run[qt] = 0.f; l_run[qt] = 0.f; }
    if (!(ABL & 8)) {
#pragma unroll
        for (int qt = 0; qt < NQ; ++qt) {
            float tm = -3e38f;
#pragma unroll
            for (int blk = 0; blk < 3; ++blk) {
                const int kr0 = blk < 2 ? blk * 32 : q0 + qt * 32;
                const int kb = blk < 2 ? blk : 2 + qt;
                f16v so = {0.f, 0.f, 0.f, 0.f, 0.f, 0.f, 0.f, 0.f, 0.f, 0.f, 0.f, 0.f, 0.f, 0.f, 0.f, 0.f};
#pragma unroll
                for (int ks = 0; ks < 4; ++ks) so = Op::mfma(kq[kb][ks], qf[qt][ks], so);
#pragma unroll
                for (int r = 0; r < 16; ++r) {
                    const int key = kr0 + (r & 3) + 8 * (r >> 2) + 4 * hi;
                    tm = fmaxf(tm, key < S ? so[r] : -3e38f);
                }
            }
            float a, b;
            halves(tm, a, b);
            m_run[qt] = fmaxf(a, b);
        }
    }
    f16v negm[NQ];
#pragma unroll
    for (int qt = 0; qt < NQ; ++qt)
#pragma unroll
        for (int r = 0; r < 16; ++r) negm[qt][r] = -m_run[qt];

    f16v o[NQ][2];
    f16v sc[2][2];
    dtk_u4 pf[NQ][4];
    op8 kf[8], vf[8];
#pragma unroll
    for (int qt = 0; qt < NQ; ++qt) {
#pragma unroll
        for (int db = 0; db < 2; ++db)
#pragma unroll
            for (int r = 0; r < 16; ++r) o[qt][db][r] = 0.f;
#pragma unroll
        for (int g = 0; g < 4; ++g)
#pragma unroll
            for (int e = 0; e < 4; ++e) pf[qt][g][e] = 0u;
    }
#pragma unroll
    for (int s = 0; s < 2; ++s)
#pragma unroll
        for (int b = 0; b < 2; ++b)
#pragma unroll
            for (int r = 0; r < 16; ++r) sc[s][b][r] = -1e30f;
#pragma unroll
    for (int g = 0; g < 8; ++g) {
#pragma unroll
        for (int e = 0; e < 8; ++e) vf[g][e] = (T)0.f;
        asm volatile("" : "+a"(vf[g]));
    }
    const int krow = (lq & 19) | ((lq & 4) << 1) | ((lq & 8) >> 1);
    unsigned ka[4], va[4];
    {
        const unsigned koff0 = krow * 128 + ((hi ^ ((krow >> 1) & 7)) << 4);
        const unsigned voff0 = 8192 + lq * 128 + ((hi ^ ((lq >> 1) & 7)) << 4);
#pragma unroll
        for (int j = 0; j < 4; ++j) {
            ka[j] = lds_base + (koff0 ^ (j << 5));
            va[j] = lds_base + (voff0 ^ (j << 5));
        }
    }
#pragma unroll
    for (int f = 0; f < 8; ++f) {
        if (f & 1) a6_lds_frag<4096>(kf[f], ka[f >> 1]);
        else a6_lds_frag<0>(kf[f], ka[f >> 1]);
    }
    asm volatile("s_waitcnt lgkmcnt(0)" ::: "memory");

    auto mask_tail = [&](f16v (&s2)[2], int t) {
#pragma unroll
        for (int b = 0; b < 2; ++b)
#pragma unroll
            for (int r = 0; r < 16; ++r) {
                const int key = t * 64 + b * 32 + 16 * (r >> 3) + 8 * hi + (r & 7);
                if (key >= S) s2[b][r] = -1e30f;
            }
    };
    auto guard_tripped = [&](auto qt_tag, auto set_tag, float lsum, bool scores_live) {
        constexpr int qt = decltype(qt_tag)::value, set = decltype(set_tag)::value;
        asm volatile("; guard tripped" ::: "memory");
        agpr_settle();
        float a, b;
        halves(lsum, a, b);
        const float tot = a + b;
        if (!(a < Op::POISON_T && b < Op::POISON_T)) {
            l_run[qt] = __builtin_nanf("");
        } else if (tot >= Op::RESC_T) {
            const float k = floorf(__builtin_amdgcn_logf(tot));
            const float alpha = __builtin_amdgcn_exp2f(-k);
            m_run[qt] += k;
            if (scores_live) {
#pragma unroll
                for (int b2 = 0; b2 < 2; ++b2)
#pragma unroll
                    for (int r = 0; r < 16; ++r) sc[set][b2][r] -= k;
            }
            l_run[qt] *= alpha;
#pragma unroll
            for (int db = 0; db < 2; ++db)
#pragma unroll
                for (int r = 0; r < 16; ++r) o[qt][db][r] *= alpha;
#pragma unroll
            for (int r = 0; r < 16; ++r) negm[qt][r] = -m_run[qt];
        }
    };

    const int tail_tile = (S & 63) != 0 ? ntiles - 1 : -1;
    int pend[NQ];
    float lsum[NQ];
#pragma unroll
    for (int qt = 0; qt < NQ; ++qt) { pend[qt] = 0; lsum[qt] = 0.f; }

    auto sub_step = [&](auto u_tag, auto vb_tag, int t) {
        constexpr int U = decltype(u_tag)::value, VB = decltype(vb_tag)::value;
        constexpr int SET = U & 1, SQ = (U + NQ - 1) % NQ;
        constexpr int KB = (VB + 1) & (A4_NB - 1), DB = (VB + A4_AHEAD) & (A4_NB - 1);
        constexpr bool REFILL = U == NQ - 1, DMA = U == 0;
        float lta = 0.f, ltb = 0.f, q0e = 0.f, q1e = 0.f;
        auto chunk_exp = [&](int c, float& p0, float& p1) {
            const int bj = c >> 2, e = 2 * (c & 3);
            const float s0 = sc[1 - SET][bj >> 1][8 * (bj & 1) + e], s1 = sc[1 - SET][bj >> 1][8 * (bj & 1) + e + 1];
            p0 = (ABL & 1) ? s0 * 0.01f : __builtin_amdgcn_exp2f(s0);
            p1 = (ABL & 1) ? s1 * 0.01f : __builtin_amdgcn_exp2f(s1);
        };
        auto chunk_fin = [&](int c, float p0, float p1) {
            const int bj = c >> 2, e = 2 * (c & 3);
            if (c == 0) {
                lta = p0;
                ltb = p1;
            } else {
                asm volatile("v_add_f32 %0, %0, %1" : "+v"(lta) : "v"(p0));
                asm volatile("v_add_f32 %0, %0, %1" : "+v"(ltb) : "v"(p1));
            }
            unsigned wv;
            if constexpr (Op::F16) asm volatile("v_cvt_pk_f16_f32 %0, %1, %2" : "=v"(wv) : "v"(p0), "v"(p1));
            else asm volatile("v_cvt_pk_bf16_f32 %0, %1, %2" : "=v"(wv) : "v"(p0), "v"(p1));
            pf[SQ][bj][e >> 1] = wv;
        };
#pragma unroll
        for (int i = 0; i < 16; ++i) {
            const int j = i >> 1;
            if ((i & 1) == 0) {
                if (j < 2) a6_s_first<T>(sc[SET][j & 1], kf[j], qf[U][j >> 1], negm[U]);
                else a6_s_next<T>(sc[SET][j & 1], kf[j], qf[U][j >> 1]);
            } else {
                a6_pv<T>(o[U][j & 1], vf[j], __builtin_bit_cast(op8, pf[U][j >> 1]));
            }
            if (!(ABL & 128) && REFILL) {
                if (i & 1) {
                    if (j & 1) a6_lds_frag<VB * TILE_BYTES + 4096>(vf[j], va[j >> 1]);
                    else a6_lds_frag<VB * TILE_BYTES>(vf[j], va[j >> 1]);
                } else {
                    if (j & 1) a6_lds_frag<KB * TILE_BYTES + 4096>(kf[j], ka[j >> 1]);
                    else a6_lds_frag<KB * TILE_BYTES>(kf[j], ka[j >> 1]);
                }
            }
            if (DMA && (i & 3) == 2 && !((ABL & 2) && t > 0)) issue_one(t + A4_AHEAD, std::integral_constant<int, DB>{}, i >> 2);
            if (U == 0 && i == 7) asm volatile("s_waitcnt lgkmcnt(0)" ::: "memory");
            float p0, p1;
            chunk_exp(i, p0, p1);
            if (i > 0) chunk_fin(i - 1, q0e, q1e);
            asm volatile("" : "+v"(p0), "+v"(p1));
            q0e = p0;
            q1e = p1;
            __builtin_amdgcn_sched_barrier(0);
        }
        chunk_fin(15, q0e, q1e);
        const float lt = lta + ltb;
        l_run[SQ] += lt;
        if (t == tail_tile) {
            asm volatile("s_nop 15" ::: "memory");
            mask_tail(sc[SET], t);
        }
        if (ABL & 8) return;
        if (pend[U]) {
            guard_tripped(u_tag, std::integral_constant<int, SET>{}, lsum[U], true);
            pend[U] = 0;
        }
        lsum[SQ] = lt;
        pend[SQ] = __builtin_amdgcn_ballot_w64(!(lt < Op::RESC_T)) != 0ull;
    };
    auto key_tile = [&](auto vb_tag, int t) {
        dtk_vm_wait<4>();
        asm volatile("s_waitcnt lgkmcnt(8)" ::: "memory");
        if (!(ABL & 16)) __syncthreads();
        sub_step(std::integral_constant<int, 0>{}, vb_tag, t);
        sub_step(std::integral_constant<int, 1>{}, vb_tag, t);
        sub_step(std::integral_constant<int, 2>{}, vb_tag, t);
        sub_step(std::integral_constant<int, 3>{}, vb_tag, t);
    };
    static_assert(A6_NQ == 4, "score sets alternate by U & 1: an even number of tiles");
    for (int t = 0; t < ntiles; t += A4_NB) {
        key_tile(std::integral_constant<int, 0>{}, t);
        if (t + 1 < ntiles) key_tile(std::integral_constant<int, 1>{}, t + 1);
        if (t + 2 < ntiles) key_tile(std::integral_constant<int, 2>{}, t + 2);
        if (t + 3 < ntiles) key_tile(std::integral_constant<int, 3>{}, t + 3);
    }
    asm volatile("s_waitcnt lgkmcnt(0)" ::: "memory");
    {
        float lta = 0.f;
#pragma unroll
        for (int c = 0; c < 16; ++c) {
            const int bj = c >> 2, e = 2 * (c & 3);
            const float p0 = __builtin_amdgcn_exp2f(sc[1][bj >> 1][8 * (bj & 1) + e]), p1 = __builtin_amdgcn_exp2f(sc[1][bj >> 1][8 * (bj & 1) + e + 1]);
            lta += p0 + p1;
            const op2 pk = {(T)p0, (T)p1};
            pf[NQ - 1][bj][e >> 1] = __builtin_bit_cast(unsigned, pk);
        }
        l_run[NQ - 1] += lta;
        lsum[NQ - 1] = lta;
        pend[NQ - 1] = (ABL & 8) ? 0 : (__builtin_amdgcn_ballot_w64(!(lta < Op::RESC_T)) != 0ull);
        asm volatile("s_nop 4" ::: "memory");
#pragma unroll
        for (int g = 0; g < 8; ++g) a6_pv<T>(o[0][g & 1], vf[g], __builtin_bit_cast(op8, pf[0][g >> 1]));
#pragma unroll
        for (int g = 0; g < 8; ++g) a6_pv<T>(o[1][g & 1], vf[g], __builtin_bit_cast(op8, pf[1][g >> 1]));
#pragma unroll
        for (int g = 0; g < 8; ++g) a6_pv<T>(o[2][g & 1], vf[g], __builtin_bit_cast(op8, pf[2][g >> 1]));
#pragma unroll
        for (int g = 0; g < 8; ++g) a6_pv<T>(o[3][g & 1], vf[g], __builtin_bit_cast(op8, pf[3][g >> 1]));
    }
    if (pend[0]) guard_tripped(std::integral_constant<int, 0>{}, std::integral_constant<int, 0>{}, lsum[0], false);
    if (pend[1]) guard_tripped(std::integral_constant<int, 1>{}, std::integral_constant<int, 0>{}, lsum[1], false);
    if (pend[2]) guard_tripped(std::integral_constant<int, 2>{}, std::integral_constant<int, 0>{}, lsum[2], false);
    if (pend[3]) guard_tripped(std::integral_constant<int, 3>{}, std::integral_constant<int, 0>{}, lsum[3], false);
    agpr_settle();
    dtk_vm_wait<0>();
    float l_tot[NQ];
    bool redo = false;
#pragma unroll
    for (int qt = 0; qt < NQ; ++qt) {
        float a, b;
        halves(l_run[qt], a, b);
        l_tot[qt] = a + b;
        redo |= __any(!(l_tot[qt] > Op::LOW_T && l_tot[qt] < 0x1p120f));
    }
    if (redo && !(ABL & 8)) {
        safe_pass<T, 6>(Qb, Kb, Vb, O + (size_t)frame * S * D + head * 64, q0, 32 * NQ, S, Sp, D);
        return;
    }
#pragma unroll
    for (int qt = 0; qt < NQ; ++qt) {
        const float inv = 1.f / l_tot[qt];
        const int qi = q0 + qt * 32 + lq;
        if (qi < S) {
            T* orow = O + ((size_t)frame * S + qi) * D + head * 64;
#pragma unroll
            for (int db = 0; db < 2; ++db)
#pragma unroll
                for (int pr = 0; pr < 2; ++pr) {
                    typedef unsigned u2v __attribute__((ext_vector_type(2)));
                    const op4 ve = {(T)(o[qt][db][8 * pr + 0] * inv), (T)(o[qt][db][8 * pr + 1] * inv),
                                    (T)(o[qt][db][8 * pr + 2] * inv), (T)(o[qt][db][8 * pr + 3] * inv)};
                    const op4 vo = {(T)(o[qt][db][8 * pr + 4] * inv), (T)(o[qt][db][8 * pr + 5] * inv),
                                    (T)(o[qt][db][8 * pr + 6] * inv), (T)(o[qt][db][8 * pr + 7] * inv)};
                    const u2v e = __builtin_bit_cast(u2v, ve), od = __builtin_bit_cast(u2v, vo);
                    dtk_u4 out;
#pragma unroll
                    for (int k = 0; k < 2; ++k) {
                        const auto sw = __builtin_amdgcn_permlane32_swap(e[k], od[k], false, false);
                        const unsigned first = sw[0], second = sw[1];
                        out[k] = first;
                        out[2 + k] = second;
                    }
                    const int d = db * 32 + 16 * pr + 8 * hi;
                    *reinterpret_cast<dtk_u4*>(orow + d) = out;
                }
        }
    }
}

}
```

### dino_tracker_amd/csrc/vit_attention_common.h

```cpp
#pragma once
#include <type_traits>
#include "common.h"

namespace attn {

typedef float f2 __attribute__((ext_vector_type(2)));
typedef float f16v __attribute__((ext_vector_type(16)));

template <typename T>
struct Operand {
    typedef T v8 __attribute__((ext_vector_type(8)));
    typedef T v4 __attribute__((ext_vector_type(4)));
    typedef T v2 __attribute__((ext_vector_type(2)));
    static constexpr bool F16 = std::is_same<T, _Float16>::value;
    static __device__ __forceinline__ f16v mfma(v8 a, v8 b, f16v c) {
        if constexpr (F16) return __builtin_amdgcn_mfma_f32_32x32x16_f16(a, b, c, 0, 0, 0);
        else return __builtin_amdgcn_mfma_f32_32x32x16_bf16(a, b, c, 0, 0, 0);
    }
    static constexpr float RESC_T = F16 ? 0x1p9f : 0x1p40f;
    static constexpr float POISON_T = F16 ? 0x1p15f : 0x1p120f;
    static constexpr float LOW_T = F16 ? 0x1p-7f : 0x1p-100f;
};

constexpr int TILE_KEYS = 64;
constexpr int TILE_BYTES = 2 * TILE_KEYS * 64 * 2;
constexpr int A4_NB = 4;
constexpr int A4_AHEAD = 3;

inline unsigned attention_grid(int FH, int S, int queries, int* qb_out) {
    const int QB = (S + queries - 1) / queries;
    *qb_out = QB;
    return (unsigned)(((FH + 7) / 8) * 8 * QB);
}

__device__ __forceinline__ void halves(float x, float& lo_all, float& hi_all) {
    const auto sw = __builtin_amdgcn_permlane32_swap(__float_as_uint(x), __float_as_uint(x), false, false);
    const unsigned r0 = sw[0], r1 = sw[1];
    lo_all = __uint_as_float(r0);
    hi_all = __uint_as_float(r1);
}

template <typename T>
__device__ __forceinline__ void safe_pass_impl(const T* Qb, const T* Kb, const T* Vb, T* Ob, int q0, int nq, int S, int Sp,
                                               int D) {
    typedef Operand<T> Op;
    typedef typename Op::v8 op8;
    typedef typename Op::v4 op4;
    const int lane = threadIdx.x & 63, lq = lane & 31, hi = lane >> 5;
    const int krow = (lq & 19) | ((lq & 4) << 1) | ((lq & 8) >> 1);
    const int ntiles = (S + 63) / 64;
#pragma unroll 1
    for (int qq = q0; qq < q0 + nq; qq += 32) {
        op8 qf[4];
        const int qrow = min(qq + lq, Sp - 1);
#pragma unroll
        for (int ks = 0; ks < 4; ++ks) qf[ks] = *reinterpret_cast<const op8*>(Qb + (size_t)qrow * 64 + ks * 16 + hi * 8);
        f16v oa[2];
        float m = -3e38f;
        f2 l = {0.f, 0.f};
#pragma unroll
        for (int db = 0; db < 2; ++db)
#pragma unroll
            for (int r = 0; r < 16; ++r) oa[db][r] = 0.f;
#pragma unroll 1
        for (int t = 0; t < ntiles; ++t) {
            f16v s2[2];
#pragma unroll
            for (int b = 0; b < 2; ++b) {
#pragma unroll
                for (int r = 0; r < 16; ++r) s2[b][r] = 0.f;
#pragma unroll
                for (int ks = 0; ks < 4; ++ks) {
                    const op8 kf = *reinterpret_cast<const op8*>(Kb + (size_t)(t * 64 + b * 32 + krow) * 64 + ks * 16 + hi * 8);
                    s2[b] = Op::mfma(kf, qf[ks], s2[b]);
                }
            }
            float tm = -3e38f;
#pragma unroll
            for (int b = 0; b < 2; ++b)
#pragma unroll
                for (int r = 0; r < 16; ++r) {
                    const int key = t * 64 + b * 32 + 16 * (r >> 3) + 8 * hi + (r & 7);
                    if (key >= S) s2[b][r] = -1e30f;
                    tm = fmaxf(tm, s2[b][r]);
                }
            tm = fmaxf(tm, __shfl_xor(tm, 32, 64));
            const float mn = fmaxf(m, tm);
            const float alpha = __builtin_amdgcn_exp2f(m - mn);
            m = mn;
            l *= f2{alpha, alpha};
#pragma unroll
            for (int db = 0; db < 2; ++db)
#pragma unroll
                for (int r = 0; r < 16; ++r) oa[db][r] *= alpha;
#pragma unroll
            for (int bj = 0; bj < 4; ++bj) {
                op8 pfr;
#pragma unroll
                for (int e = 0; e < 8; ++e) {
                    const float pv = __builtin_amdgcn_exp2f(s2[bj >> 1][8 * (bj & 1) + e] - m);
                    l[e & 1] += pv;
                    pfr[e] = (T)pv;
                }
#pragma unroll
                for (int db = 0; db < 2; ++db) {
                    const op8 vf = *reinterpret_cast<const op8*>(Vb + (size_t)(db * 32 + lq) * Sp + t * 64 + bj * 16 + hi * 8);
                    oa[db] = Op::mfma(vf, pfr, oa[db]);
                }
            }
        }
        const float lh = l[0] + l[1];
        const float inv = 1.f / (lh + __shfl_xor(lh, 32, 64));
        const int qi = qq + lq;
        if (qi < S) {
            T* orow = Ob + (size_t)qi * D;
#pragma unroll
            for (int db = 0; db < 2; ++db)
#pragma unroll
                for (int rq = 0; rq < 4; ++rq) {
                    const int d = db * 32 + 8 * rq + 4 * hi;
                    op4 v = {(T)(oa[db][4 * rq + 0] * inv), (T)(oa[db][4 * rq + 1] * inv), (T)(oa[db][4 * rq + 2] * inv),
                             (T)(oa[db][4 * rq + 3] * inv)};
                    *reinterpret_cast<op4*>(orow + d) = v;
                }
        }
    }
}
template <typename T, int TAG>
__device__ __noinline__ void safe_pass(const T* Qb, const T* Kb, const T* Vb, T* Ob, int q0, int nq, int S, int Sp, int D) {
    safe_pass_impl(Qb, Kb, Vb, Ob, q0, nq, S, Sp, D);
}

template <typename T>
__device__ __forceinline__ void mfma_acc_agpr(f16v& c, typename Operand<T>::v8 a, typename Operand<T>::v8 b) {
    if constexpr (Operand<T>::F16) asm volatile("v_mfma_f32_32x32x16_f16 %0, %1, %2, %0" : "+a"(c) : "v"(a), "v"(b));
    else asm volatile("v_mfma_f32_32x32x16_bf16 %0, %1, %2, %0" : "+a"(c) : "v"(a), "v"(b));
}
__device__ __forceinline__ void agpr_settle() { asm volatile("s_nop 15\n\ts_nop 15\n\ts_nop 15" ::: "memory"); }

}
```

### dino_tracker_amd/csrc/vit_gemm_common.h

```cpp
#pragma once
#include "common.h"

namespace {

typedef float f2 __attribute__((ext_vector_type(2)));
typedef float f4 __attribute__((ext_vector_type(4)));
typedef float f16v __attribute__((ext_vector_type(16)));
typedef _Float16 half_t;
typedef _Float16 h8 __attribute__((ext_vector_type(8)));
typedef _Float16 h4v __attribute__((ext_vector_type(4)));
typedef __bf16 bf8 __attribute__((ext_vector_type(8)));

template <typename T> struct Vec {
    typedef T t8 __attribute__((ext_vector_type(8)));
    typedef T t4 __attribute__((ext_vector_type(4)));
    typedef T t2 __attribute__((ext_vector_type(2)));
};
template <typename T> struct IsF16 { static constexpr bool value = false; };
template <> struct IsF16<_Float16> { static constexpr bool value = true; };
__device__ __forceinline__ f4 mfma16(h8 a, h8 b, f4 c) { return __builtin_amdgcn_mfma_f32_16x16x32_f16(a, b, c, 0, 0, 0); }
__device__ __forceinline__ f4 mfma16(bf8 a, bf8 b, f4 c) { return __builtin_amdgcn_mfma_f32_16x16x32_bf16(a, b, c, 0, 0, 0); }
__device__ __forceinline__ f16v mfma32(h8 a, h8 b, f16v c) { return __builtin_amdgcn_mfma_f32_32x32x16_f16(a, b, c, 0, 0, 0); }
__device__ __forceinline__ f16v mfma32(bf8 a, bf8 b, f16v c) { return __builtin_amdgcn_mfma_f32_32x32x16_bf16(a, b, c, 0, 0, 0); }
template <typename T> __device__ __forceinline__ void operand_mode() {
    if (IsF16<T>::value) dtk_fp16_saturate_mode();
}

constexpr int GM = 128, GN = 128, GK = 32;
enum { EPI_QKV = 0, EPI_GELU = 1, EPI_DELTA = 2, EPI_F32 = 3, EPI_SWIGLU = 4 };

template <typename T>
struct GemmEpi {
    const float* bias;
    T* q;
    T* k;
    T* vt;
    int S, Sp, heads, D;
    float qscale;
    T* out;
    int no_store;
    T* delta;
    const float* gamma;
    float* out_f32;
    int* ovf;
    float* ln_x;
    const float *ln_w, *ln_b;
    T* ln_out;
    float ln_eps;
    int* ln_ovf;
};

__device__ __forceinline__ float amax2(float m, float a, float b) { return fmaxf(fmaxf(m, fabsf(a)), fabsf(b)); }
template <typename T, int EPI>
__device__ __forceinline__ void amax_report(float amax, int* ovf) {
    if (IsF16<T>::value && (EPI == EPI_QKV || EPI == EPI_GELU || EPI == EPI_SWIGLU) && ovf) {
        if (__any(amax >= 65488.f) && (threadIdx.x & 63) == 0) atomicOr(ovf, EPI == EPI_QKV ? 2 : 4);
    }
}

__device__ __forceinline__ int swiglu_col(int n) { return ((n >> 6) << 5) + (n & 31); }
__device__ __forceinline__ float silu_f32(float v) {
    const float e = __builtin_amdgcn_exp2f(v * -1.4426950408889634f);
    return v * __builtin_amdgcn_rcpf(1.f + e);
}
__device__ __forceinline__ float swiglu_pair(float gate, float value, float& amax) {
    const float h = silu_f32(gate) * value;
    amax = fmaxf(amax, fabsf(h));
    return h;
}

__device__ __forceinline__ int gswz_f(int row) { return (0x1230 >> (((row >> 2) & 3) * 4)) & 3; }
__device__ __forceinline__ int gswz(int row, int piece) { return row * 4 + (piece ^ gswz_f(row)); }
__device__ __forceinline__ uint4 staged16(const unsigned char* sp) {
    const uint2 lo = *reinterpret_cast<const uint2*>(sp), hi = *reinterpret_cast<const uint2*>(sp + 8);
    return make_uint4(lo.x, lo.y, hi.x, hi.y);
}

template <typename T, int EPI>
__device__ __forceinline__ void gemm_store_tile(const f4& a, long long mb, int n, float bias, long long M, int N,
                                                const GemmEpi<T>& e, float& amax) {
    if (IsF16<T>::value && (EPI == EPI_QKV || EPI == EPI_GELU)) {
        const float sc = (EPI == EPI_QKV && n < e.D) ? e.qscale : 1.f;
        if (EPI == EPI_GELU) amax = fmaxf(fmaxf(fmaxf(amax, a[0] + bias), fmaxf(a[1] + bias, a[2] + bias)), a[3] + bias);
        else amax = amax2(amax2(amax, (a[0] + bias) * sc, (a[1] + bias) * sc), (a[2] + bias) * sc, (a[3] + bias) * sc);
    }
    if (EPI == EPI_QKV) {
        const int which = n / e.D, rem = n - which * e.D;
        const int head = rem >> 6, dh = rem & 63;
        const int frame = (int)(mb / e.S);
        (void)frame;
        if (which == 2) {
#pragma unroll
            for (int r = 0; r < 4; ++r) {
                const long long m = mb + r;
                if (m < M) {
                    const int f = (int)(m / e.S), s = (int)(m - (long long)f * e.S);
                    e.vt[(((size_t)f * e.heads + head) * 64 + dh) * e.Sp + s] = (T)(a[r] + bias);
                }
            }
        } else {
            T* dst = which == 0 ? e.q : e.k;
            const float sc = which == 0 ? e.qscale : 1.f;
#pragma unroll
            for (int r = 0; r < 4; ++r) {
                const long long m = mb + r;
                if (m < M) {
                    const int f = (int)(m / e.S), s = (int)(m - (long long)f * e.S);
                    dst[(((size_t)f * e.heads + head) * e.Sp + s) * 64 + dh] = (T)((a[r] + bias) * sc);
                }
            }
        }
    } else if (EPI == EPI_GELU) {
#pragma unroll
        for (int r = 0; r < 4; ++r) {
            const long long m = mb + r;
            if (m < M) {
                const float v = a[r] + bias;
                e.out[m * N + n] = (T)(0.5f * v * (1.f + erff(v * 0.70710678118654752f)));
            }
        }
    } else if (EPI == EPI_F32) {
#pragma unroll
        for (int r = 0; r < 4; ++r) {
            const long long m = mb + r;
            if (m < M) e.out_f32[m * N + n] = a[r] + bias;
        }
    } else {
        const float gm = e.gamma[n];
#pragma unroll
        for (int r = 0; r < 4; ++r) {
            const long long m = mb + r;
            if (m < M) e.delta[m * N + n] = (T)(gm * (a[r] + bias));
        }
    }
}

template <typename T>
__device__ __forceinline__ void gemm_store_tile_swiglu(const f4& a, const f4& b, long long mb, int n, float bg, float bv, long long M,
                                                       int N, const GemmEpi<T>& e, float& amax) {
    const int hc = swiglu_col(n), NH = N >> 1;
#pragma unroll
    for (int r = 0; r < 4; ++r) {
        const float h = swiglu_pair(a[r] + bg, b[r] + bv, amax);
        if (mb + r < M) e.out[(mb + r) * NH + hc] = (T)h;
    }
}

template <int REQ, int I = 0>
__device__ __forceinline__ void wd_issue(const dtk_u4 (&srd)[REQ], const unsigned (&voff)[REQ], unsigned soff, unsigned lds_dst) {
    dtk_buffer_lds16<I * 1024>(srd[I], soff, voff[I], lds_dst);
    if constexpr (I + 1 < REQ) wd_issue<REQ, I + 1>(srd, voff, soff, lds_dst);
}

__device__ __forceinline__ f2 gelu2(f2 x) {
    const f2 c = {4.25f, 4.25f};
    const f2 sx = __builtin_elementwise_min(__builtin_elementwise_max(x, -c), c);
    const f2 u = sx * sx;
    f2 p = {1.112979639e-10f, 1.112979639e-10f};
    p = __builtin_elementwise_fma(p, u, f2{-1.065557687e-08f, -1.065557687e-08f});
    p = __builtin_elementwise_fma(p, u, f2{4.510875158e-07f, 4.510875158e-07f});
    p = __builtin_elementwise_fma(p, u, f2{-1.125288873e-05f, -1.125288873e-05f});
    p = __builtin_elementwise_fma(p, u, f2{1.868377149e-04f, 1.868377149e-04f});
    p = __builtin_elementwise_fma(p, u, f2{-2.217123518e-03f, -2.217123518e-03f});
    p = __builtin_elementwise_fma(p, u, f2{1.963194646e-02f, 1.963194646e-02f});
    p = __builtin_elementwise_fma(p, u, f2{-1.326889843e-01f, -1.326889843e-01f});
    p = __builtin_elementwise_fma(p, u, f2{7.978046536e-01f, 7.978046536e-01f});
    const f2 one = {1.f, 1.f};
    const f2 e = __builtin_elementwise_min(__builtin_elementwise_max(sx * p, -one), one);
    const f2 hx = x * f2{0.5f, 0.5f};
    return __builtin_elementwise_fma(hx, e, hx);
}

template <typename T, int EPI>
__device__ __forceinline__ void gemm_store_tile_t(const f4& a, long long m, int nb, long long M, int N, const GemmEpi<T>& e,
                                                  float& amax) {
    typedef typename Vec<T>::t4 T4;
    const float4 b4 = e.bias ? *reinterpret_cast<const float4*>(e.bias + nb) : make_float4(0.f, 0.f, 0.f, 0.f);
    float v[4] = {a[0] + b4.x, a[1] + b4.y, a[2] + b4.z, a[3] + b4.w};
    if (EPI == EPI_QKV) {
        const int which = nb / e.D, rem = nb - which * e.D;
        const int head = rem >> 6, dh = rem & 63;
        const float sc = which == 0 ? e.qscale : 1.f;
#pragma unroll
        for (int r = 0; r < 4; ++r) v[r] *= sc;
        if (IsF16<T>::value) amax = amax2(amax2(amax, v[0], v[1]), v[2], v[3]);
        if (m >= M || DTK_DBG(e.no_store, 4)) return;
        const int f = (int)(m / e.S), sp = (int)(m - (long long)f * e.S);
        if (which == 2) {
            T* vp = e.vt + (((size_t)f * e.heads + head) * 64 + dh) * e.Sp + sp;
#pragma unroll
            for (int r = 0; r < 4; ++r) vp[(size_t)r * e.Sp] = (T)v[r];
        } else {
            T* dst = (which == 0 ? e.q : e.k) + (((size_t)f * e.heads + head) * e.Sp + sp) * 64 + dh;
            *reinterpret_cast<T4*>(dst) = T4{(T)v[0], (T)v[1], (T)v[2], (T)v[3]};
        }
    } else if (EPI == EPI_GELU) {
        if (IsF16<T>::value) amax = fmaxf(fmaxf(fmaxf(amax, v[0]), fmaxf(v[1], v[2])), v[3]);
        if (m >= M || DTK_DBG(e.no_store, 4)) return;
        const f2 g0 = gelu2(f2{v[0], v[1]}), g1 = gelu2(f2{v[2], v[3]});
        *reinterpret_cast<T4*>(e.out + m * N + nb) = T4{(T)g0[0], (T)g0[1], (T)g1[0], (T)g1[1]};
    } else {
        if (m >= M || DTK_DBG(e.no_store, 4)) return;
        const float4 g4 = *reinterpret_cast<const float4*>(e.gamma + nb);
        *reinterpret_cast<T4*>(e.delta + m * N + nb) = T4{(T)(g4.x * v[0]), (T)(g4.y * v[1]), (T)(g4.z * v[2]), (T)(g4.w * v[3])};
    }
}

template <typename T, int EPI>
__device__ __forceinline__ typename Vec<T>::t4 gemm_value_tile_t(const f4& a, const float4& b4, const float4& g4, float& amax) {
    typedef typename Vec<T>::t4 T4;
    const float v[4] = {a[0] + b4.x, a[1] + b4.y, a[2] + b4.z, a[3] + b4.w};
    if (EPI == EPI_GELU) {
        if (IsF16<T>::value) amax = fmaxf(fmaxf(fmaxf(amax, v[0]), fmaxf(v[1], v[2])), v[3]);
        const f2 g0 = gelu2(f2{v[0], v[1]}), g1 = gelu2(f2{v[2], v[3]});
        return T4{(T)g0[0], (T)g0[1], (T)g1[0], (T)g1[1]};
    }
    return T4{(T)(g4.x * v[0]), (T)(g4.y * v[1]), (T)(g4.z * v[2]), (T)(g4.w * v[3])};
}

}
```

### dino_tracker_amd/csrc/vit_gemm_ws.h

```cpp
#pragma once
#include <type_traits>
#include <utility>
#include "vit_gemm_common.h"

namespace {

constexpr int WS_KS = 24, WS_K = 16 * WS_KS, WS_ROWS = 32, WS_COLS = 256;
constexpr int WS_TILE_BYTES = WS_ROWS * WS_K * 2;
constexpr int WS_LQ = WS_KS / 4;
constexpr int WS_PITCH = 144;
constexpr int WS_UNIT_BYTES = WS_ROWS * WS_PITCH;

template <class F, int... I>
__device__ __forceinline__ void ws_for_each(F&& f, std::integer_sequence<int, I...>) { (f(std::integral_constant<int, I>{}), ...); }
template <int N, class F>
__device__ __forceinline__ void ws_for_each(F&& f) { ws_for_each(f, std::make_integer_sequence<int, N>{}); }

template <typename T, int EPI, int V2M = 3, bool HC = (V2M == 3)>
__global__ __launch_bounds__(256) void gemm_ws_kernel(const T* __restrict__ A, const T* __restrict__ Wt,
                                                      long long M, int N, GemmEpi<T> e, int tiles_per_chunk) {
    typedef typename Vec<T>::t8 T8;
    typedef typename Vec<T>::t4 T4;
    (void)sizeof(T8); (void)sizeof(T4);
    constexpr bool V2 = (V2M & 1) != 0;
    constexpr bool V2D = (V2M & 2) != 0;
    static_assert(!HC || V2M == 3, "the hand-cut step is built on the AGPR weights and the descriptor LDS-DMA");
    operand_mode<T>();
    __shared__ __attribute__((aligned(1024))) unsigned char toks[3][WS_TILE_BYTES];
    __shared__ __attribute__((aligned(16))) unsigned char stage[4][2][WS_UNIT_BYTES];
    __shared__ __attribute__((aligned(16))) float s_bias[4][64], s_gamma[4][64];
    const int tid = threadIdx.x, lane = tid & 63;
    const int w = __builtin_amdgcn_readfirstlane(tid >> 6);
    const int j = lane & 31, h = lane >> 5;
    const int n0 = blockIdx.x * WS_COLS + w * 64;
    const long long total_tiles = (M + WS_ROWS - 1) / WS_ROWS;
    const long long tile0 = (long long)blockIdx.y * tiles_per_chunk;
    if (tile0 >= total_tiles) return;
    const int NT = (int)((total_tiles - tile0) < tiles_per_chunk ? (total_tiles - tile0) : tiles_per_chunk);
    const int nl = (j & 3) + 4 * (j >> 3) + 16 * ((j >> 2) & 1);
    T8 wf[2][WS_KS];
#pragma unroll
    for (int t = 0; t < 2; ++t) {
        const int row = min(n0 + t * 32 + nl, N - 1);
        const T* wp = Wt + (size_t)row * WS_K + h * 8;
#pragma unroll
        for (int ks = 0; ks < WS_KS; ++ks) {
            if (V2) asm volatile("global_load_dwordx4 %0, %1, off" : "=a"(wf[t][ks]) : "v"(wp + ks * 16) : "memory");
            else wf[t][ks] = *reinterpret_cast<const T8*>(wp + ks * 16);
        }
    }
    if (V2) {
        asm volatile("s_waitcnt vmcnt(0)" ::: "memory");
#pragma unroll
        for (int t = 0; t < 2; ++t)
#pragma unroll
            for (int ks = 0; ks < WS_KS; ++ks) asm volatile("" : "+a"(wf[t][ks]));
    }
    if constexpr (!HC) {
        const int n = min(n0 + lane, N - 1);
        s_bias[w][lane] = e.bias ? e.bias[n] : 0.f;
        s_gamma[w][lane] = (EPI == EPI_DELTA) ? e.gamma[n] : 1.f;
    }
    const int which = (EPI == EPI_QKV) ? min(n0, N - 1) / e.D : 0;
    const int head = (EPI == EPI_QKV) ? (min(n0, N - 1) - which * e.D) >> 6 : 0;
    const float qsc = (EPI == EPI_QKV && which == 0) ? e.qscale : 1.f;
    long long m_ep = tile0 * WS_ROWS + j;
    int f_ep = 0, s_ep = 0;
    if (EPI == EPI_QKV) { f_ep = (int)(m_ep / e.S); s_ep = (int)(m_ep - (long long)f_ep * e.S); }
    const unsigned lds_base = (unsigned)(size_t)&toks[0][0];
    const int l_tt = lane & 3, l_pp = lane >> 2;
    const dtk_u4 srd = dtk_make_srd(A + tile0 * WS_ROWS * WS_K);
    unsigned a_voff[2], a_voff_last[2];
    const int last_rows = (int)(M - (total_tiles - 1) * WS_ROWS);
#pragma unroll
    for (int gg = 0; gg < 2; ++gg) {
        const int g = 2 * w + gg;
        a_voff[gg] = (unsigned)(((4 * g + l_tt) * WS_K + ((l_pp - g) & 15) * 8) * 2);
        a_voff_last[gg] = (unsigned)((min(4 * g + l_tt, last_rows - 1) * WS_K + ((l_pp - g) & 15) * 8) * 2);
    }
    const unsigned a_dst = __builtin_amdgcn_readfirstlane(lds_base + (2 * w) * 3 * 1024);
    auto issue = [&](int n, int buf) {
        if (V2D) {
            const unsigned toff = __builtin_amdgcn_readfirstlane((unsigned)n * (unsigned)WS_TILE_BYTES);
            const unsigned dst = __builtin_amdgcn_readfirstlane(a_dst + (unsigned)buf * (unsigned)WS_TILE_BYTES);
            const bool last = tile0 + n == total_tiles - 1;
            const unsigned v0 = last ? a_voff_last[0] : a_voff[0], v1 = last ? a_voff_last[1] : a_voff[1];
            dtk_buffer_lds16<0>(srd, toff, v0, dst);
            dtk_buffer_lds16<1024>(srd, toff + 256u, v0, dst);
            dtk_buffer_lds16<2048>(srd, toff + 512u, v0, dst);
            dtk_buffer_lds16<3072>(srd, toff, v1, dst);
            dtk_buffer_lds16<4096>(srd, toff + 256u, v1, dst);
            dtk_buffer_lds16<5120>(srd, toff + 512u, v1, dst);
            return;
        }
#pragma unroll
        for (int gg = 0; gg < 2; ++gg) {
            const int g = 2 * w + gg;
            const long long m = min((tile0 + n) * WS_ROWS + 4 * g + l_tt, M - 1);
            const T* gp = A + m * WS_K + ((l_pp - g) & 15) * 8;
#pragma unroll
            for (int c = 0; c < 3; ++c)
                dtk_glds16(gp + c * 128, __builtin_amdgcn_readfirstlane(lds_base + buf * WS_TILE_BYTES + (g * 3 + c) * 1024));
        }
    };
    unsigned frag_off[8];
#pragma unroll
    for (int k8 = 0; k8 < 8; ++k8)
        frag_off[k8] = (unsigned)((j >> 2) * 3 * 1024 + ((((2 * k8 + h + (j >> 2)) & 15) * 4 + (j & 3)) * 16));
    float amax = 0.f;
    unsigned dbg_sink = 0;
    auto dbg_fold = [&](const auto& val) {
        unsigned b[sizeof(val) / 4];
        __builtin_memcpy(b, &val, sizeof(val));
#pragma unroll
        for (unsigned i = 0; i < sizeof(val) / 4; ++i) dbg_sink |= b[i];
    };
    if constexpr (HC) {
        typedef std::integral_constant<bool, true> Yes;
        typedef std::integral_constant<bool, false> No;
        if (n0 >= N) {
            issue(0, 0);
            issue(min(1, NT - 1), 1);
            dtk_vm_wait<WS_LQ>();
            __syncthreads();
            int b0 = 0;
            for (int n = 0; n + 1 < NT; n += 2) {
                const int b1 = b0 == 2 ? 0 : b0 + 1, b2 = b1 == 2 ? 0 : b1 + 1;
                issue(min(n + 2, NT - 1), b2);
                dtk_vm_wait<WS_LQ>();
                __syncthreads();
                issue(min(n + 3, NT - 1), b0);
                dtk_vm_wait<WS_LQ>();
                __syncthreads();
                b0 = b2;
            }
            dtk_vm_wait<0>();
            return;
        }
        float bia[2][16], gam[2][16];
#pragma unroll
        for (int t = 0; t < 2; ++t)
#pragma unroll
            for (int r = 0; r < 16; ++r) {
                const int nf = n0 + 32 * t + 16 * h + r;
                bia[t][r] = e.bias ? e.bias[nf] : 0.f;
                gam[t][r] = (EPI == EPI_DELTA) ? e.gamma[nf] : 1.f;
            }
        const bool dbg_nost = DTK_DBG(e.no_store, 3) || DTK_DBG(e.no_store, 32);
        const bool dbg_noar = DTK_DBG(e.no_store, 64);
        auto run = [&](auto vt_tag) {
            constexpr bool VT = decltype(vt_tag)::value;
            constexpr bool STG = EPI != EPI_GELU && !VT;
            const long long mt0 = tile0 * WS_ROWS;
            T* op = nullptr;
            T* up = nullptr;
            int s0 = 0;
            unsigned cross = 0;
            if constexpr (EPI == EPI_GELU) op = e.out + (mt0 + j) * N + n0 + 16 * h;
            if constexpr (EPI == EPI_DELTA) up = e.delta + mt0 * N + n0;
            if constexpr (EPI == EPI_QKV) {
                const int f0 = (int)(mt0 / e.S);
                s0 = (int)(mt0 - (long long)f0 * e.S);
                if (VT) {
                    up = e.vt + (((size_t)f0 * e.heads + head) * 64) * e.Sp + s0;
                    cross = (unsigned)(e.heads * 64 * e.Sp - e.S);
                } else {
                    up = (which == 0 ? e.q : e.k) + (((size_t)f0 * e.heads + head) * e.Sp + s0) * 64;
                    cross = (unsigned)((e.heads * e.Sp - e.S) * 64);
                }
            }
            const size_t out_step = (size_t)WS_ROWS * N;
            unsigned char* const sw = &stage[w][0][0] + j * WS_PITCH + 32 * h;
            const unsigned char* const sr = &stage[w][0][0] + (lane >> 3) * WS_PITCH + (lane & 7) * 16;
            auto next_tile = [&]() {
                if constexpr (EPI == EPI_GELU) op += out_step;
                if constexpr (EPI == EPI_DELTA) up += out_step;
                if constexpr (EPI == EPI_QKV) {
                    s0 += WS_ROWS;
                    up += VT ? WS_ROWS : WS_ROWS * 64;
                    if (s0 >= e.S) { s0 -= e.S; up += cross; }
                }
            };
            auto st16 = [&](T* p, unsigned off, dtk_u4 val, bool ok) {
                if (!dbg_nost) { if (ok) *reinterpret_cast<dtk_u4*>(p + off) = val; }
                else dbg_fold(val);
            };
            float v[8];
            f2 sx[4], uu[4], pp[4];
            T8 o;
            dtk_u4 fv[4];
            unsigned voff = 0;
            constexpr float GC[9] = {1.112979639e-10f, -1.065557687e-08f, 4.510875158e-07f, -1.125288873e-05f, 1.868377149e-04f,
                                     -2.217123518e-03f, 1.963194646e-02f, -1.326889843e-01f, 7.978046536e-01f};
            auto flush_reads = [&]() {
                ws_for_each<4>([&](auto p_tag) {
                    constexpr int p = decltype(p_tag)::value;
                    fv[p] = *reinterpret_cast<const dtk_u4*>(sr + 8 * p * WS_PITCH);
                });
            };
            auto flush_store = [&](auto pred_tag, auto p_tag, int valid) {
                constexpr int p = decltype(p_tag)::value;
                const int row = 8 * p + (lane >> 3);
                const bool ok = decltype(pred_tag)::value ? row < valid : true;
                if constexpr (EPI == EPI_DELTA) st16(up, (unsigned)(row * N + (lane & 7) * 8), fv[p], ok);
                else st16(up, (unsigned)(row * 64 + (lane & 7) * 8) + (s0 + row >= e.S ? cross : 0u), fv[p], ok);
            };
            auto slot = [&](auto pred_tag, auto fl_tag, const f16v (&acc)[2], auto s_tag, int valid) {
                constexpr bool PRED = decltype(pred_tag)::value, FL = decltype(fl_tag)::value;
                constexpr int s = decltype(s_tag)::value;
                const bool ok = PRED ? j < valid : true;
                if constexpr (EPI == EPI_GELU) {
                    constexpr int u = s / 12, ph = s % 12, t = u >> 1, hv = u & 1;
                    if (ph < 2) {
#pragma unroll
                        for (int r = 4 * ph; r < 4 * ph + 4; ++r) v[r] = acc[t][8 * hv + r] + bia[t][8 * hv + r];
                        if (IsF16<T>::value) {
#pragma unroll
                            for (int r = 4 * ph; r < 4 * ph + 4; r += 2) amax = fmaxf(fmaxf(amax, v[r]), v[r + 1]);
                        }
                    }
                    if (dbg_noar) {
                        if (ph == 9) {
#pragma unroll
                            for (int r = 0; r < 8; ++r) o[r] = (T)v[r];
                        }
                    } else if (ph == 2) {
                        const f2 c = {4.25f, 4.25f};
#pragma unroll
                        for (int q = 0; q < 4; ++q) sx[q] = __builtin_elementwise_min(__builtin_elementwise_max(f2{v[2 * q], v[2 * q + 1]}, -c), c);
#pragma unroll
                        for (int q = 0; q < 4; ++q) uu[q] = sx[q] * sx[q];
                    } else if (ph >= 3 && ph <= 6) {
#pragma unroll
                        for (int l = 2 * (ph - 3); l < 2 * (ph - 3) + 2; ++l)
#pragma unroll
                            for (int q = 0; q < 4; ++q)
                                pp[q] = __builtin_elementwise_fma(l == 0 ? f2{GC[0], GC[0]} : pp[q], uu[q], f2{GC[l + 1], GC[l + 1]});
                    } else if (ph == 7) {
                        const f2 one = {1.f, 1.f};
#pragma unroll
                        for (int q = 0; q < 4; ++q) pp[q] = __builtin_elementwise_min(__builtin_elementwise_max(sx[q] * pp[q], -one), one);
                    } else if (ph == 8) {
#pragma unroll
                        for (int q = 0; q < 4; ++q) {
                            const f2 hx = f2{v[2 * q], v[2 * q + 1]} * f2{0.5f, 0.5f};
                            uu[q] = __builtin_elementwise_fma(hx, pp[q], hx);
                        }
                    } else if (ph == 9) {
#pragma unroll
                        for (int q = 0; q < 4; ++q) { o[2 * q] = (T)uu[q][0]; o[2 * q + 1] = (T)uu[q][1]; }
                    }
                    if (ph == 10) {
                        st16(op, (unsigned)(32 * t + 8 * hv), __builtin_bit_cast(dtk_u4, o), ok);
                    }
                } else if constexpr (STG) {
                    if constexpr (FL && s == 0) flush_reads();
                    if constexpr (FL && s >= 1 && s <= 4) flush_store(No{}, std::integral_constant<int, s - 1>{}, WS_ROWS);
                    constexpr int u = s / 12, ph = s % 12, t = u >> 1, hv = u & 1;
                    if (ph & 1) {
                        if (ph < 9) {
                            constexpr int r0 = (ph - 1) & 7, r1 = ph & 7;
                            const float v0 = acc[t][8 * hv + r0] + bia[t][8 * hv + r0], v1 = acc[t][8 * hv + r1] + bia[t][8 * hv + r1];
                            if (EPI == EPI_QKV && IsF16<T>::value && !dbg_noar) amax = amax2(amax, v0 * qsc, v1 * qsc);
                            if (dbg_noar) { o[r0] = (T)v0; o[r1] = (T)v1; }
                            else if (EPI == EPI_DELTA) { o[r0] = (T)(v0 * gam[t][8 * hv + r0]); o[r1] = (T)(v1 * gam[t][8 * hv + r1]); }
                            else { o[r0] = (T)(v0 * qsc); o[r1] = (T)(v1 * qsc); }
                        } else if (ph == 9) {
                            *reinterpret_cast<T8*>(sw + 64 * t + 16 * hv) = o;
                        }
                    }
                } else {
                    if (s == 0) voff = (unsigned)(16 * h * e.Sp + j) + (s0 + j >= e.S ? cross : 0u);
                    if (s < 32) {
                        constexpr int u = (s & 31) / 8, r = s % 8, t = u >> 1, hv = u & 1;
                        v[r] = acc[t][8 * hv + r] + bia[t][8 * hv + r];
                        if (IsF16<T>::value && (r & 1) && !dbg_noar) amax = amax2(amax, v[r - 1] * qsc, v[r] * qsc);
                        const T val = (T)v[r];
                        T* const p = up + (size_t)(32 * t + 8 * hv + r) * e.Sp;
                        if (!dbg_nost) { if (ok) p[voff] = val; }
                        else dbg_fold(typename Vec<T>::t2{val, val});
                    }
                }
            };
            auto tail_epi = [&](const f16v (&acc)[2], int valid) {
                ws_for_each<2 * WS_KS>([&](auto s_tag) { slot(Yes{}, No{}, acc, s_tag, valid); });
                if (!STG) next_tile();
            };
            auto tail_flush = [&](int valid) {
                if constexpr (STG) {
                    flush_reads();
                    ws_for_each<4>([&](auto p_tag) { flush_store(Yes{}, p_tag, valid); });
                    next_tile();
                }
            };
            auto step = [&](auto prev_tag, auto fl_tag, int buf, f16v (&accN)[2], const f16v (&accP)[2]) {
                constexpr bool PREV = decltype(prev_tag)::value, FL = decltype(fl_tag)::value;
                const unsigned char* base = &toks[0][0] + buf * WS_TILE_BYTES;
                const f16v zero16 = {0.f, 0.f, 0.f, 0.f, 0.f, 0.f, 0.f, 0.f, 0.f, 0.f, 0.f, 0.f, 0.f, 0.f, 0.f, 0.f};
                T8 b[3];
                b[0] = *reinterpret_cast<const T8*>(base + frag_off[0]);
                b[1] = *reinterpret_cast<const T8*>(base + frag_off[1]);
                ws_for_each<2 * WS_KS>([&](auto s_tag) {
                    constexpr int ks = decltype(s_tag)::value / 2, t = decltype(s_tag)::value % 2;
                    if constexpr (t == 0 && ks + 2 < WS_KS)
                        b[(ks + 2) % 3] = *reinterpret_cast<const T8*>(base + frag_off[(ks + 2) & 7] + ((ks + 2) >> 3) * 1024);
                    accN[t] = mfma32(wf[t][ks], b[ks % 3], ks == 0 ? zero16 : accN[t]);
                    if constexpr (PREV) {
                        __builtin_amdgcn_sched_barrier(0);
                        slot(No{}, fl_tag, accP, s_tag, WS_ROWS);
                        __builtin_amdgcn_sched_barrier(0);
                    }
                });
                if (STG ? FL : PREV) next_tile();
            };
            f16v accA[2], accB[2];
            issue(0, 0);
            issue(min(1, NT - 1), 1);
            dtk_vm_wait<WS_LQ>();
            __syncthreads();
            int n = 0, b0 = 0;
            auto pair = [&](auto first_tag) {
                constexpr bool FIRST = decltype(first_tag)::value;
                const int b1 = b0 == 2 ? 0 : b0 + 1, b2 = b1 == 2 ? 0 : b1 + 1;
                issue(min(n + 2, NT - 1), b2);
                if (FIRST) step(No{}, No{}, b0, accA, accB);
                else step(Yes{}, Yes{}, b0, accA, accB);
                dtk_vm_wait<WS_LQ>();
                __syncthreads();
                issue(min(n + 3, NT - 1), b0);
                if (FIRST) step(Yes{}, No{}, b1, accB, accA);
                else step(Yes{}, Yes{}, b1, accB, accA);
                dtk_vm_wait<WS_LQ>();
                __syncthreads();
                b0 = b2;
                n += 2;
            };
            if (NT >= 2) pair(Yes{});
            while (n + 1 < NT) pair(No{});
            const long long left = M - (tile0 + NT - 1) * WS_ROWS;
            const int valid = left < WS_ROWS ? (int)left : WS_ROWS;
            const bool odd = n < NT;
            if (odd) {
                if (n > 0) step(Yes{}, Yes{}, b0, accA, accB);
                else step(No{}, No{}, b0, accA, accB);
            }
            if (NT > 1) tail_flush(WS_ROWS);
            const f16v accL[2] = {odd ? accA[0] : accB[0], odd ? accA[1] : accB[1]};
            tail_epi(accL, valid);
            tail_flush(valid);
        };
        if constexpr (EPI == EPI_QKV) {
            if (which == 2) run(Yes{});
            else run(No{});
        } else {
            run(No{});
        }
        if (DTK_DBG(e.no_store, 32) && dbg_sink == 0x9e3779b9u) amax = 65504.f;
        amax_report<T, EPI>(amax, e.ovf);
        dtk_vm_wait<0>();
        return;
    }
    auto epi8 = [&](const f16v (&acc)[2], int t, int hv) {
        const int fl = 32 * t + 16 * h + 8 * hv;
        const int nb = n0 + fl;
        const float4 b0 = *reinterpret_cast<const float4*>(&s_bias[w][fl]), b1 = *reinterpret_cast<const float4*>(&s_bias[w][fl + 4]);
        float v[8];
#pragma unroll
        for (int r = 0; r < 8; ++r) v[r] = acc[t][8 * hv + r];
        v[0] += b0.x; v[1] += b0.y; v[2] += b0.z; v[3] += b0.w;
        v[4] += b1.x; v[5] += b1.y; v[6] += b1.z; v[7] += b1.w;
        const bool ok = m_ep < M && nb < N && !DTK_DBG(e.no_store, 3);
        if (IsF16<T>::value && (EPI == EPI_QKV || EPI == EPI_GELU)) {
#pragma unroll
            for (int r = 0; r < 8; r += 2) {
                if (EPI == EPI_GELU) amax = fmaxf(fmaxf(amax, v[r]), v[r + 1]);
                else if (!DTK_DBG(e.no_store, 64)) amax = amax2(amax, v[r] * qsc, v[r + 1] * qsc);
            }
        }
        if (EPI == EPI_GELU) {
            T8 o;
#pragma unroll
            for (int r = 0; r < 8; r += 2) {
                const f2 g = DTK_DBG(e.no_store, 64) ? f2{v[r], v[r + 1]} : gelu2(f2{v[r], v[r + 1]});
                o[r] = (T)g[0];
                o[r + 1] = (T)g[1];
            }
            if (DTK_DBG(e.no_store, 32)) dbg_fold(o);
            else if (ok) *reinterpret_cast<T8*>(e.out + m_ep * N + nb) = o;
        } else if (EPI == EPI_DELTA) {
            const float4 g0 = *reinterpret_cast<const float4*>(&s_gamma[w][fl]), g1 = *reinterpret_cast<const float4*>(&s_gamma[w][fl + 4]);
            T8 o = {(T)(v[0] * g0.x), (T)(v[1] * g0.y), (T)(v[2] * g0.z), (T)(v[3] * g0.w),
                     (T)(v[4] * g1.x), (T)(v[5] * g1.y), (T)(v[6] * g1.z), (T)(v[7] * g1.w)};
            *reinterpret_cast<T8*>(&stage[w][0][0] + j * WS_PITCH + fl * 2) = o;
        } else {
            const int dh = fl;
            if (which == 2) {
                if (DTK_DBG(e.no_store, 32)) {
#pragma unroll
                    for (int r = 0; r < 8; r += 2) dbg_fold(typename Vec<T>::t2{(T)v[r], (T)v[r + 1]});
                } else if (ok) {
                    T* vp = e.vt + (((size_t)f_ep * e.heads + head) * 64 + dh) * e.Sp + s_ep;
#pragma unroll
                    for (int r = 0; r < 8; ++r) vp[(size_t)r * e.Sp] = (T)v[r];
                }
            } else {
                T8 o;
#pragma unroll
                for (int r = 0; r < 8; ++r) o[r] = DTK_DBG(e.no_store, 64) ? (T)v[r] : (T)(v[r] * qsc);
                *reinterpret_cast<T8*>(&stage[w][0][0] + j * WS_PITCH + fl * 2) = o;
            }
        }
    };
    long long mt_fl = tile0 * WS_ROWS;
    int f0_fl = 0, s0_fl = 0;
    if (EPI == EPI_QKV) { f0_fl = (int)(mt_fl / e.S); s0_fl = (int)(mt_fl - (long long)f0_fl * e.S); }
    auto flush = [&]() {
        if (EPI != EPI_GELU && n0 < N && !DTK_DBG(e.no_store, 3) && !(EPI == EPI_QKV && which == 2)) {
#pragma unroll
            for (int u = 0; u < 1; ++u) {
#pragma unroll
                for (int p = 0; p < 4; ++p) {
                    const int row = 8 * p + (lane >> 3), piece = lane & 7;
                    const uint4 val = *reinterpret_cast<const uint4*>(&stage[w][u][0] + row * WS_PITCH + piece * 16);
                    if (DTK_DBG(e.no_store, 32)) dbg_fold(val);
                    else if (mt_fl + row < M) {
                        if (EPI == EPI_DELTA) {
                            *reinterpret_cast<uint4*>(e.delta + (mt_fl + row) * N + n0 + piece * 8) = val;
                        } else {
                            int f = f0_fl, sp = s0_fl + row;
                            if (sp >= e.S) { sp -= e.S; ++f; }
                            T* dst = which == 0 ? e.q : e.k;
                            *reinterpret_cast<uint4*>(dst + (((size_t)f * e.heads + head) * e.Sp + sp) * 64 + piece * 8) = val;
                        }
                    }
                }
            }
        }
        mt_fl += WS_ROWS;
        if (EPI == EPI_QKV) {
            s0_fl += WS_ROWS;
            if (s0_fl >= e.S) { s0_fl -= e.S; ++f0_fl; }
        }
    };
    auto advance = [&]() {
        m_ep += WS_ROWS;
        if (EPI == EPI_QKV) {
            s_ep += WS_ROWS;
            if (s_ep >= e.S) { s_ep -= e.S; ++f_ep; }
        }
    };
    auto step = [&](int buf, f16v (&accN)[2], const f16v (&accP)[2], bool have_prev, bool have_flush) {
        if (!V2) {
#pragma unroll
            for (int t = 0; t < 2; ++t)
#pragma unroll
                for (int r = 0; r < 16; ++r) accN[t][r] = 0.f;
        }
        const unsigned char* base = &toks[0][0] + buf * WS_TILE_BYTES;
        const f16v zero16 = {0.f, 0.f, 0.f, 0.f, 0.f, 0.f, 0.f, 0.f, 0.f, 0.f, 0.f, 0.f, 0.f, 0.f, 0.f, 0.f};
        T8 b[3];
        b[0] = *reinterpret_cast<const T8*>(base + frag_off[0]);
        b[1] = *reinterpret_cast<const T8*>(base + frag_off[1]);
#pragma unroll
        for (int ks = 0; ks < WS_KS; ++ks) {
            if (ks + 2 < WS_KS)
                b[(ks + 2) % 3] = *reinterpret_cast<const T8*>(base + frag_off[(ks + 2) & 7] + ((ks + 2) >> 3) * 1024);
#pragma unroll
            for (int t = 0; t < 2; ++t) {
                if (V2) accN[t] = mfma32(wf[t][ks], b[ks % 3], ks == 0 ? zero16 : accN[t]);
                else accN[t] = mfma32(wf[t][ks], b[ks % 3], accN[t]);
            }
            if (have_flush && ks == 0) flush();
            if (have_prev && ks % 6 == 2) epi8(accP, (ks / 6) >> 1, (ks / 6) & 1);
        }
        if (have_prev) advance();
    };
    f16v accA[2], accB[2];
    issue(0, 0);
    issue(min(1, NT - 1), 1);
    dtk_vm_wait<WS_LQ>();
    __syncthreads();
    int n = 0, b0 = 0;
    for (; n + 1 < NT; n += 2) {
        const int b1 = b0 == 2 ? 0 : b0 + 1, b2 = b1 == 2 ? 0 : b1 + 1;
        issue(min(n + 2, NT - 1), b2);
        step(b0, accA, accB, n > 0, n > 1);
        dtk_vm_wait<WS_LQ>();
        __syncthreads();
        issue(min(n + 3, NT - 1), b0);
        step(b1, accB, accA, true, n > 0);
        dtk_vm_wait<WS_LQ>();
        __syncthreads();
        b0 = b2;
    }
    if (n < NT) {
        step(b0, accA, accB, n > 0, n > 1);
        if (n > 0) flush();
#pragma unroll
        for (int u = 0; u < 4; ++u) epi8(accA, u >> 1, u & 1);
    } else {
        if (n > 1) flush();
#pragma unroll
        for (int u = 0; u < 4; ++u) epi8(accB, u >> 1, u & 1);
    }
    flush();
    if (DTK_DBG(e.no_store, 32) && dbg_sink == 0x9e3779b9u) amax = 65504.f;
    amax_report<T, EPI>(amax, e.ovf);
    dtk_vm_wait<0>();
}

inline std::pair<dim3, int> gemm_ws_grid(int N, long long rows) {
    const int colwg = dtk_cdiv(N, WS_COLS);
    const int chunks = 256 / colwg > 0 ? 256 / colwg : 1;
    const long long tiles = dtk_cdiv(rows, WS_ROWS);
    const int tpc = (int)dtk_cdiv(tiles, chunks);
    return std::make_pair(dim3(colwg, (unsigned)dtk_cdiv(tiles, tpc)), tpc);
}

}
```

### dino_tracker_amd/extractor.py

```python
from __future__ import annotations

import ctypes
import math
import os
from typing import Dict, List, Optional

import torch
import torch.nn as nn
import torch.nn.functional as F

from . import ops
from ._lib import VIT_FFN_SWIGLU, VIT_ATTENTION_V4, VIT_GEMM_WIDE_V1, VIT_GEMM_WS_V1, VIT_NO_LN_FUSION, VIT_BF16, VIT_CHECK_RANGE, VIT_TILED_GEMMS, VitLayer, VitModel, check, lib
from .synth import VIT_CONFIGS, make_vit_weights

IMAGENET_MEAN = (0.485, 0.456, 0.406)
IMAGENET_STD = (0.229, 0.224, 0.225)


class VitExtractor(nn.Module):
    BLOCK_KEY, ATTN_KEY, PATCH_IMD_KEY, QKV_KEY = "block", "attn", "patch_imd", "qkv"
    KEY_LIST = [BLOCK_KEY, ATTN_KEY, PATCH_IMD_KEY, QKV_KEY]

    def __init__(self, model_name, stride, device, state_dict: Optional[Dict[str, torch.Tensor]] = None,
                 random_seed: Optional[int] = None, operand_dtype: str = "fp16", check_range: bool = False,
                 on_overflow: str = "split-bf16", precision=None, auto_tol: float = 2.5e-4, calibration_frames: int = 2,
                 block_margin: float = 0.8):
        super().__init__()
        if operand_dtype not in ("fp16", "bf16"):
            raise ValueError(f"operand_dtype {operand_dtype!r}: 'fp16' or 'bf16'")
        if on_overflow not in ("split-bf16", "bf16", "raise"):
            raise ValueError(f"on_overflow {on_overflow!r}: 'split-bf16' (re-encode on split bf16 operands), 'bf16' (plain bf16 "
                             "operands) or 'raise'")
        self.operand_dtype = operand_dtype
        self.on_overflow = on_overflow
        self.range_fallbacks = 0
        self.last_overflow = 0
        self._deferred_pending = 0
        self.check_range = check_range
        self.auto_tol, self.calibration_frames = float(auto_tol), int(calibration_frames)
        self.block_margin = float(block_margin)
        self.calibration = None
        self.attention_v2 = False
        self.attention_v4 = os.environ.get("DTK_VIT_ATTENTION_V4", "0") == "1"
        self.gemm_ws_v1 = False
        self.no_ln_fusion = os.environ.get("DTK_VIT_NO_LN_FUSION", "0") == "1"
        self.gemm_wide_v1 = os.environ.get("DTK_VIT_GEMM_WIDE_V1", "0") == "1"
        self.frame_batch = 0
        if model_name not in VIT_CONFIGS:
            raise NotImplementedError(f"{model_name}: the HIP encoder covers dinov2_vit{{s,b,l,g}}14 (d_head 64)")
        self.model_name, self.stride, self.device = model_name, stride, device
        self.cfg = VIT_CONFIGS[model_name]
        if state_dict is None and os.environ.get("DTK_DINOV2_WEIGHTS"):
            state_dict = torch.load(os.environ["DTK_DINOV2_WEIGHTS"], map_location="cpu")
        if state_dict is None and random_seed is not None:
            state_dict = make_vit_weights(model_name, seed=random_seed)
        if state_dict is None:
            raise RuntimeError("no DINOv2 weights: pass state_dict=, set $DTK_DINOV2_WEIGHTS to a checkpoint in "
                               "upstream naming, or ask for random_seed= explicitly (torch.hub needs the network)")
        self.n_layers = self.get_n_layers()
        self.swiglu = self.cfg.get("ffn") == "swiglu"
        self.n_blocks = sum(1 for i in range(self.n_layers) if f"blocks.{i}.norm1.weight" in state_dict)
        self.tiled_gemms = False
        self._sd = {k: v.detach().to(device=device, dtype=torch.float32).contiguous() for k, v in state_dict.items()
                    if k.startswith(("cls_token", "pos_embed", "patch_embed.", "blocks."))}
        self._keep = []
        self._wcache = {}
        self._layers_of = {}
        self._pos_cache = {}
        self.set_precision(precision if precision is not None else os.environ.get("DTK_VIT_PRECISION", "fast"))
        self._layers = self._build_layers(self.operand_dtype, self.split_blocks)

    def set_precision(self, precision):
        depth = VIT_CONFIGS[self.model_name]["depth"]
        if isinstance(precision, str):
            if precision not in ("fast", "split", "auto", "auto-blocks"):
                raise ValueError(f"precision {precision!r}: 'fast', 'split', 'auto', 'auto-blocks' or a list of block indices")
            self.precision = precision
            self.split_blocks = frozenset(range(depth)) if precision == "split" else frozenset()
        else:
            blocks = frozenset(int(b) for b in precision)
            if any(not 0 <= b < depth for b in blocks):
                raise ValueError(f"precision: block indices must be in [0, {depth})")
            self.precision, self.split_blocks = "blocks", blocks
        self.calibration = None

    def precision_report(self):
        depth = self.cfg["depth"]
        full = len(self.split_blocks) == depth
        cls = {("fp16", True): "fp32-grade (<= 4e-6)", ("bf16", True): "2^-16 (~2e-5)", ("fp16", False): "2^-12 (1.3e-4 .. 2.1e-3)",
               ("bf16", False): "2^-9 (1e-3 .. 1.9e-2)"}[(self.operand_dtype, full)]
        return {"operand_dtype": self.operand_dtype, "precision": self.precision, "split_blocks": sorted(self.split_blocks),
                "range_fallbacks": self.range_fallbacks, "last_overflow": self.last_overflow, "calibration": self.calibration,
                "feature_error_class": cls if (full or not self.split_blocks) else f"mixed ({len(self.split_blocks)}/{depth} blocks split)"}

    def _build_layers(self, operand_dtype, split_blocks=frozenset()):
        key = (operand_dtype, frozenset(split_blocks))
        if key in self._layers_of:
            return self._layers_of[key]
        depth = self.cfg["depth"]
        arr = (VitLayer * depth)()
        sd = self._sd

        def f32(name):
            t = sd[name].contiguous()
            self._keep.append(t)
            return t.data_ptr()

        wdt = torch.float16 if operand_dtype == "fp16" else torch.bfloat16

        def b16(name):
            ck = (name, operand_dtype)
            if ck not in self._wcache:
                w = sd[name]
                if wdt == torch.float16 and float(w.abs().max()) >= 65504.0:
                    raise RuntimeError(f"{name}: |w| reaches the fp16 limit; use operand_dtype='bf16'")
                self._wcache[ck] = w.to(wdt).contiguous()
            return self._wcache[ck].data_ptr()

        def split16(names):
            ck = (names[0], operand_dtype, "split")
            if ck not in self._wcache:
                scale = 1.0
                if wdt == torch.float16:
                    amax = max(float(sd[n].abs().max()) for n in names)
                    scale = 256.0
                    while scale > 1.0 and amax * scale >= 32768.0:
                        scale /= 2.0
                    if amax * scale >= 65504.0:
                        raise RuntimeError(f"{names[0]}: |w| reaches the fp16 limit; use operand_dtype='bf16'")
                planes = []
                for n in names:
                    w = sd[n] * scale
                    hi = w.to(wdt)
                    lo = (w - hi.float()).to(wdt)
                    planes.append((hi.contiguous(), lo.contiguous()))
                self._wcache[ck] = (scale, planes)
            return self._wcache[ck]

        def pack_w12(t):
            hid = self.cfg["hidden"]
            gate, value = t[:hid].reshape(hid // 32, 32, *t.shape[1:]), t[hid:].reshape(hid // 32, 32, *t.shape[1:])
            return torch.stack((gate, value), dim=1).reshape(t.shape).contiguous()

        if self.swiglu:
            for i in range(self.n_blocks):
                for kind in ("weight", "bias"):
                    if f"blocks.{i}.mlp.w12p.{kind}" not in sd:
                        sd[f"blocks.{i}.mlp.w12p.{kind}"] = pack_w12(sd[f"blocks.{i}.mlp.w12.{kind}"])
        fc1, fc2 = ("mlp.w12p", "mlp.w3") if self.swiglu else ("mlp.fc1", "mlp.fc2")
        for i in range(self.n_blocks):
            p = f"blocks.{i}."
            L = arr[i]
            L.ln1_w, L.ln1_b = f32(p + "norm1.weight"), f32(p + "norm1.bias")
            L.qkv_b, L.proj_b = f32(p + "attn.qkv.bias"), f32(p + "attn.proj.bias")
            L.ls1 = f32(p + "ls1.gamma")
            L.ln2_w, L.ln2_b = f32(p + "norm2.weight"), f32(p + "norm2.bias")
            L.fc1_b, L.fc2_b = f32(p + fc1 + ".bias"), f32(p + fc2 + ".bias")
            L.ls2 = f32(p + "ls2.gamma")
            names = [p + "attn.qkv.weight", p + "attn.proj.weight", p + fc1 + ".weight", p + fc2 + ".weight"]
            if i in split_blocks:
                scale, planes = split16(names)
                (L.qkv_w, L.qkv_w_lo), (L.proj_w, L.proj_w_lo), (L.fc1_w, L.fc1_w_lo), (L.fc2_w, L.fc2_w_lo) = \
                    [(h.data_ptr(), l.data_ptr()) for h, l in planes]
                L.w_scale = scale
            else:
                L.qkv_w, L.proj_w, L.fc1_w, L.fc2_w = [b16(n) for n in names]
                L.qkv_w_lo = L.proj_w_lo = L.fc1_w_lo = L.fc2_w_lo = None
                L.w_scale = 1.0
        self._layers_of[key] = arr
        return arr

    def _pos_embed(self, ph: int, pw: int):
        key = (ph, pw)
        if key not in self._pos_cache:
            pe = self._sd["pos_embed"]
            n = int(math.sqrt(pe.shape[1] - 1))
            d = pe.shape[-1]
            grid = pe[:, 1:].reshape(1, n, n, d).permute(0, 3, 1, 2)
            grid = F.interpolate(grid, scale_factor=((ph + 0.1) / n, (pw + 0.1) / n), mode="bicubic",
                                 align_corners=False, recompute_scale_factor=False)
            assert grid.shape[-2] == ph and grid.shape[-1] == pw
            pos = grid.permute(0, 2, 3, 1).reshape(ph * pw, d).contiguous()
            cls_pos = (self._sd["cls_token"].reshape(-1) + pe[0, 0]).contiguous()
            self._pos_cache[key] = (pos, cls_pos)
        return self._pos_cache[key]

    @torch.no_grad()
    def encode(self, frames: torch.Tensor, layer: Optional[int] = None, normalize: bool = True, want: str = "feat",
               defer_check: bool = False, taps: Optional[List[int]] = None):
        frames = frames.to(self.device, torch.float32).contiguous()
        n, _, H, W = frames.shape
        layer = self.n_layers - 1 if layer is None else layer
        if not -1 <= layer < self.n_layers:
            raise ValueError(f"layer {layer} out of range")
        patch = self.get_patch_size()
        ph, pw = 1 + (H - patch) // self.stride, 1 + (W - patch) // self.stride
        pos, cls_pos = self._pos_embed(ph, pw)
        if not hasattr(self, "_ms"):
            self._ms = {flag: torch.tensor((IMAGENET_MEAN + IMAGENET_STD) if flag else (0.0, 0.0, 0.0, 1.0, 1.0, 1.0),
                                           dtype=torch.float32, device=self.device) for flag in (True, False)}
            self._overflow = torch.zeros(1, dtype=torch.int32, device=self.device)
        ms, overflow = self._ms[bool(normalize)], self._overflow
        D = self.cfg["dim"]
        S = ph * pw + 1
        if want not in ("tokens", "feat", "qkv", "taps"):
            raise ValueError(want)
        if want == "taps":
            taps = sorted({range(self.n_layers)[int(t)] for t in taps})
            layer = taps[-1]
        if layer >= self.n_blocks:
            raise ValueError(f"layer {layer}: the state dict holds blocks 0 .. {self.n_blocks - 1} only")

        def run(operand_dtype, split_blocks, frames=frames, n=n):
            if self.attention_v2:
                raise RuntimeError("attention_v2: the round-2/3 attention kernel left the library; it is measured by "
                                   "scripts/ubench/attn_bench.hip only (the fallback kernel is attention_v4)")
            flags = (VIT_TILED_GEMMS if self.tiled_gemms else 0) | (VIT_BF16 if operand_dtype == "bf16" else 0) | \
                (VIT_CHECK_RANGE if self.check_range else 0) | (VIT_ATTENTION_V4 if self.attention_v4 else 0) | \
                (VIT_GEMM_WS_V1 if self.gemm_ws_v1 else 0) | (VIT_GEMM_WIDE_V1 if self.gemm_wide_v1 else 0) | \
                (VIT_NO_LN_FUSION if self.no_ln_fusion else 0)
            m = VitModel(D, self.cfg["heads"], layer + 1, patch, self.stride, 1e-6, flags,
                         self._sd["patch_embed.proj.weight"].data_ptr(),
                         self._sd["patch_embed.proj.bias"].data_ptr(), cls_pos.data_ptr(), pos.data_ptr(), ms.data_ptr(),
                         ctypes.cast(self._build_layers(operand_dtype, split_blocks), ctypes.POINTER(VitLayer)),
                         int(self.frame_batch), overflow.data_ptr(), None, 0, 0.0,
                         VIT_FFN_SWIGLU if self.swiglu else 0, self.cfg["hidden"] if self.swiglu else 0)
            tap_out = None
            if want == "taps":
                tap_out = torch.zeros((n, S, D), dtype=torch.float32, device=self.device)
                m.tap_out, m.tap_mask, m.tap_scale = tap_out.data_ptr(), sum(1 << t for t in taps), 1.0 / len(taps)
            ws_bytes = int(lib().dtk_vit_workspace_bytes(m, H, W, n))
            ws = getattr(self, "_ws", None)
            if ws is None or ws.numel() < ws_bytes or ws.device != frames.device:
                self._ws = ws = torch.empty(ws_bytes, dtype=torch.uint8, device=self.device)
            tokens = torch.empty((n, S, D), dtype=torch.float32, device=self.device) if want == "tokens" else None
            feat = torch.empty((n, ph * pw, D), dtype=torch.float32, device=self.device) if want == "feat" else None
            qkv = torch.empty((n, S, 3 * D), dtype=torch.float32, device=self.device) if want == "qkv" else None
            check(lib().dtk_vit_forward(m, ops._p(frames), n, H, W, ops._p(tokens), ops._p(feat), ops._p(qkv), ops._p(ws),
                                        ws_bytes, ops._stream()))
            return {"tokens": tokens, "feat": feat, "qkv": qkv, "taps": tap_out}[want]

        if self.precision in ("auto", "auto-blocks") and self.calibration is None and layer >= 0:
            if self._deferred_pending:
                raise RuntimeError(f"VitExtractor(precision={self.precision!r}): the calibrating call cannot follow un-checked deferred calls")
            k = min(n, max(1, self.calibration_frames))
            depth_all = frozenset(range(self.cfg["depth"]))
            cal = frames[:k].contiguous()
            ref = run(self.operand_dtype, depth_all, cal, k)
            if self.check_overflow(heal=True):
                ref = run(self.operand_dtype, depth_all if self.on_overflow == "split-bf16" else self.split_blocks, cal, k)
                self.check_overflow()
            ref64, ref_norm = ref.double(), ref.double().norm()

            def measure(split_blocks):
                got = run(self.operand_dtype, frozenset(split_blocks), cal, k)
                ovf = int(self._overflow.item()) if self.operand_dtype == "fp16" else 0
                if ovf:
                    self._overflow.zero_()
                    return float("inf"), True
                return float(((got.double() - ref64).norm() / ref_norm).item()), False

            rel, fast_overflow = measure(frozenset())
            chosen = "split" if not (rel <= self.auto_tol) else "fast"
            self.calibration = {"frames": k, "layer": layer, "rel_fast_vs_split": rel, "tol": self.auto_tol, "chosen": chosen,
                                "fast_pass_saturated": bool(fast_overflow)}
            if len(self.split_blocks):
                self.split_blocks = depth_all
            elif chosen == "split" and self.precision == "auto-blocks":
                self.split_blocks = self._pick_blocks(measure, layer)
            elif chosen == "split":
                self.split_blocks = depth_all

        out = run(self.operand_dtype, self.split_blocks)
        if defer_check:
            self._deferred_pending += 1
        elif self.check_overflow(heal=True):
            out = run(self.operand_dtype, self.split_blocks)
            self.check_overflow()
        return out

    def _pick_blocks(self, measure, layer):
        used = list(range(layer + 1))
        bound = self.block_margin * self.auto_tol
        alone = {}
        for b in used:
            alone[b], sat = measure(frozenset(used) - {b})
        order = sorted(used, key=lambda b: alone[b])
        fast, acc = [], 0.0
        for b in order:
            if not (acc + alone[b] ** 2) ** 0.5 <= bound:
                break
            fast.append(b)
            acc += alone[b] ** 2
        tried = []
        while fast:
            rel, sat = measure(frozenset(used) - frozenset(fast))
            tried.append({"fast_blocks": sorted(fast), "predicted": sum(alone[b] ** 2 for b in fast) ** 0.5, "measured": rel})
            if rel <= bound:
                break
            fast.pop()
        split = frozenset(used) - frozenset(fast)
        self.calibration.update({"chosen": "blocks" if fast else "split", "blocks": {
            "bound": bound, "alone": [alone[b] for b in used], "fast_blocks": sorted(fast), "split_blocks": sorted(split),
            "passes": tried, "measured": tried[-1]["measured"] if fast else 0.0}})
        return (split | frozenset(range(layer + 1, self.cfg["depth"]))) if fast else frozenset(range(self.cfg["depth"]))

    def check_overflow(self, heal: bool = False) -> bool:
        if not hasattr(self, "_overflow"):
            return False
        self.last_overflow = int(self._overflow.item())
        pending, self._deferred_pending = self._deferred_pending, 0
        if not self.last_overflow:
            return False
        self._overflow.zero_()
        what = " and ".join(n for b, n in ((1, "a residual update"), (2, "Q / K / V"), (4, "the MLP hidden")) if self.last_overflow & b)
        if self.operand_dtype == "fp16" and self.on_overflow in ("split-bf16", "bf16"):
            self.operand_dtype = "bf16"
            to = "bf16"
            if self.on_overflow == "split-bf16":
                self.split_blocks = frozenset(range(self.cfg["depth"]))
                to = "SPLIT bf16 (hi + lo: 16 significant bits, fp32's range)"
            self.range_fallbacks += 1
            import warnings
            warnings.warn(f"VitExtractor: {what} left the fp16 range (saturated at 65504); this extractor now runs on {to} "
                          "operands (range_fallbacks counts the re-encoded calls; precision_report() describes the result)",
                          RuntimeWarning, stacklevel=3)
            if heal and not pending:
                return True
            raise RuntimeError(f"dtk_vit_forward: {what} left the fp16 range in a call whose check was deferred: its features "
                               "are saturated and must be discarded -- encode the video again (this extractor is on bf16 now)")
        raise RuntimeError(f"dtk_vit_forward: {what} left the fp16 range (saturated at 65504) or is not finite; "
                           "construct the extractor with operand_dtype='bf16' (precision='split' keeps 16 significant bits there)")

    def release_workspace(self):
        torch.cuda.current_stream().synchronize()
        self._ws = None

    def get_feature_from_input(self, input_img, layers: List[int]):
        if len(set(layers)) == len(layers) and len(layers) > 1:
            return self.encode(input_img, normalize=False, want="taps", taps=list(layers))
        outs = [self.encode(input_img, layer=l, normalize=False, want="tokens") for l in layers]
        return torch.stack(outs).mean(dim=0)

    class _PerLayer:

        def __init__(self, n, fn):
            self._n, self._fn, self._cache = n, fn, {}

        def __len__(self):
            return self._n

        def __getitem__(self, layer):
            layer = range(self._n)[layer]
            if layer not in self._cache:
                self._cache[layer] = self._fn(layer)
            return self._cache[layer]

        def __iter__(self):
            return (self[i] for i in range(self._n))

    def get_qkv_feature_from_input(self, input_img):
        return VitExtractor._PerLayer(self.n_layers, lambda l: self.encode(input_img, layer=l, normalize=False, want="qkv"))

    def get_attn_feature_from_input(self, input_img):
        heads = self.cfg["heads"]

        def attn(l):
            qkv = self.encode(input_img, layer=l, normalize=False, want="qkv")
            b, s, _ = qkv.shape
            q, k, _ = qkv.reshape(b, s, 3, heads, -1).permute(2, 0, 3, 1, 4)
            return torch.softmax((q * q.shape[-1] ** -0.5) @ k.transpose(-2, -1), dim=-1)

        return VitExtractor._PerLayer(self.n_layers, attn)

    def _from_qkv(self, qkv, input_img_shape, which):
        b = input_img_shape[0]
        return qkv.reshape(b, self.get_patch_num(input_img_shape), 3, self.cfg["dim"])[:, :, which, :]

    def get_queries_from_qkv(self, qkv, input_img_shape):
        return self._from_qkv(qkv, input_img_shape, 0)

    def get_keys_from_qkv(self, qkv, input_img_shape):
        return self._from_qkv(qkv, input_img_shape, 1)

    def get_values_from_qkv(self, qkv, input_img_shape):
        return self._from_qkv(qkv, input_img_shape, 2)

    def _facet_from_input(self, input_img, layers, which):
        qkv = self.get_qkv_feature_from_input(input_img)
        return torch.cat([self._from_qkv(qkv[l], input_img.shape, which) for l in layers], dim=2)

    def get_queries_from_input(self, input_img, layers):
        return self._facet_from_input(input_img, layers, 0)

    def get_keys_from_input(self, input_img, layers):
        return self._facet_from_input(input_img, layers, 1)

    def get_values_from_input(self, input_img, layers):
        return self._facet_from_input(input_img, layers, 2)

    def get_keys_self_sim_from_input(self, input_img, layer_num):
        keys = self.get_keys_from_input(input_img, layers=[layer_num])
        h, t, d = keys.shape
        x = keys.transpose(0, 1).reshape(t, h * d)[None]
        norm = x.norm(dim=2, keepdim=True)
        return (x @ x.permute(0, 2, 1)) / torch.clamp(norm @ norm.permute(0, 2, 1), min=1e-8)

    def get_patch_size(self):
        return 8 if "8" in self.model_name else 14

    def get_width_patch_num(self, input_img_shape):
        b, c, h, w = input_img_shape
        return 1 + (w - self.get_patch_size()) // self.stride

    def get_height_patch_num(self, input_img_shape):
        b, c, h, w = input_img_shape
        return 1 + (h - self.get_patch_size()) // self.stride

    def get_patch_num(self, input_img_shape):
        return 1 + self.get_height_patch_num(input_img_shape) * self.get_width_patch_num(input_img_shape)

    def get_n_layers(self):
        return self.cfg["depth"]

    def get_head_num(self):
        return self.cfg["heads"]

    @staticmethod
    def get_embedding_dim(model_name=None):
        return VIT_CONFIGS[model_name]["dim"]
```

### include/dtk.h

```cpp
#ifndef DTK_H_
#define DTK_H_

#include <stddef.h>
#include <stdint.h>

#ifdef __cplusplus
extern "C" {
#endif

#define DTK_OK 0
#define DTK_E_INVALID (-1)
#define DTK_E_HIP (-2)
#define DTK_E_WORKSPACE (-3)

typedef struct dtk_geom {
    int32_t T;
    int32_t C;
    int32_t ph, pw;
    int32_t video_h, video_w;
    int32_t patch, stride;
    float radius;
} dtk_geom;

#define DTK_HEAD_HIDDEN 16
#define DTK_HEAD_PARAMS (16 * 9 + 16 + 16 * 9 + 1)

int dtk_version(void);
const char* dtk_last_error(void);

int dtk_profile_enable(int on);
int dtk_profile_collect(void);
const char* dtk_profile_name(int i);
double dtk_profile_ms(int i);
long long dtk_profile_launches(int i);

int dtk_pack_features(const float* chw, float* thwc, float* norms, int T, int C, int HW, void* stream);
int dtk_unpack_features(const float* thwc, float* chw, int T, int C, int HW, void* stream);
int dtk_feature_norms(const float* thwc, float* norms, int T, int C, int HW, void* stream);

typedef struct dtk_vit_layer {
    const float *ln1_w, *ln1_b;
    const void* qkv_w;
    const float* qkv_b;
    const void* proj_w;
    const float* proj_b;
    const float* ls1;
    const float *ln2_w, *ln2_b;
    const void* fc1_w;
    const float* fc1_b;
    const void* fc2_w;
    const float* fc2_b;
    const float* ls2;
    const void *qkv_w_lo, *proj_w_lo, *fc1_w_lo, *fc2_w_lo;
    float w_scale;
} dtk_vit_layer;

typedef struct dtk_vit_model {
    int32_t D, heads;
    int32_t depth;
    int32_t patch, stride;
    float ln_eps;
    int32_t flags;
    const float* patch_w;
    const float* patch_b;
    const float* cls_pos;
    const float* pos;
    const float* mean_std;
    const dtk_vit_layer* layers;
    int32_t frame_batch;
    int32_t* overflow;
    float* tap_out;
    uint64_t tap_mask;
    float tap_scale;
    int32_t ffn;
    int32_t hidden;
} dtk_vit_model;
#define DTK_VIT_FFN_GELU 0
#define DTK_VIT_FFN_SWIGLU 1

#define DTK_VIT_TILED_GEMMS 1
#define DTK_VIT_BF16 2
#define DTK_VIT_CHECK_RANGE 4
#define DTK_VIT_GEMM_WS_V1 16
#define DTK_VIT_ATTENTION_V4 32
#define DTK_VIT_NO_LN_FUSION 128
#define DTK_VIT_GEMM_WIDE_V1 64
#define DTK_OPERAND_F16 0
#define DTK_OPERAND_BF16 1
#define DTK_OPERAND_ATTENTION_V4 0x2000

size_t dtk_vit_workspace_bytes(const dtk_vit_model* m, int video_h, int video_w, int frames);
int dtk_vit_forward(const dtk_vit_model* m, const float* frames, int nframes, int video_h, int video_w,
                    float* tokens_out, float* feat_out, float* qkv_out, void* workspace, size_t workspace_bytes,
                    void* stream);

int dtk_vit_attention(const void* q, const void* k, const void* vt, void* out, int frames, int heads, int S, int Sp,
                      int operand_type, void* stream);
int dtk_vit_attention_split(const void* q_hi, const void* q_lo, const void* k_hi, const void* k_lo, const void* vt_hi,
                            const void* vt_lo, void* out_hi, void* out_lo, int frames, int heads, int S, int Sp, int operand_type,
                            void* stream);

#define DTK_VIT_GEMM_QKV 0
#define DTK_VIT_GEMM_QKV_FACET 1
#define DTK_VIT_GEMM_PROJ 2
#define DTK_VIT_GEMM_FC1 3
#define DTK_VIT_GEMM_FC2 4
#define DTK_VIT_GEMM_FC1_SWIGLU 5
#define DTK_VIT_GEMM_FC2_SWIGLU 6
typedef struct dtk_vit_gemm_args {
    int32_t role, D, flags, operand_type;
    int64_t rows;
    int32_t S, Sp;
    float ln_eps, w_scale;
    const void *a, *a_lo, *w, *w_lo;
    const float *bias, *gamma;
    void *q, *k, *vt, *q_lo, *k_lo, *vt_lo;
    void *out, *out_lo;
    float *out_f32, *x, *ln_x;
    const float *ln_w, *ln_b;
    void* ln_out;
    int32_t* ovf;
} dtk_vit_gemm_args;
int dtk_vit_gemm(const dtk_vit_gemm_args* g, void* stream);
int dtk_vit_gemm_split(const dtk_vit_gemm_args* g, void* stream);

size_t dtk_delta_dino_packed_floats(int layer, int C);
int dtk_delta_dino_pack(int layer, int C, const float* w, const float* bias, const float* bn_w, const float* bn_b,
                        const float* bn_mean, const float* bn_var, float eps, float* packed, void* stream);
size_t dtk_delta_dino_workspace_bytes(const dtk_geom* g);
int dtk_delta_dino_refine(const dtk_geom* g, const float* video, const float* dino, const float* const* packed,
                          float* out, float* norms, int t0, int nframes, void* workspace, size_t workspace_bytes,
                          void* stream);
#define DTK_DD_SPLIT 0
#define DTK_DD_FP16 1
#define DTK_DD_FP16_V1 2
int dtk_delta_dino_refine_mode(const dtk_geom* g, const float* video, const float* dino, const float* const* packed,
                               float* out, float* norms, int t0, int nframes, int operands, void* workspace,
                               size_t workspace_bytes, void* stream);

int dtk_sample_points(const dtk_geom* g, const float* feat, const float* xy, const int32_t* t_idx,
                      const int32_t* out_row, float* out, int B, void* stream);

int dtk_sample_grid(const float* feat, int T, int C, int ph, int pw, const float* pts, float* out, int B, void* stream);

int dtk_head_prepare(const float* w1, const float* b1, const float* w2, const float* b2, float* head, void* stream);

int dtk_head_forward(const dtk_geom* g, const float* head, const float* maps, float* out_xy, int B, int normalized,
                     void* stream);

int dtk_head_forward_train(const dtk_geom* g, const float* head, const float* maps, float* out_xy, float* stats, int B,
                           int normalized, void* stream);
int dtk_head_backward(const dtk_geom* g, const float* head, const float* maps, const float* stats, const float* grad_out,
                      float* dmaps, float* dhead_partial, int B, int normalized, void* stream);

size_t dtk_conv_split_weight_halves(int Cin, int Cout);
int dtk_conv_split_pack(const float* w, int Cin, int Cout, int flip_transpose, void* Wh, void* Wl, void* stream);
int dtk_conv_split_input(const float* x, int N, int C, int H, int W, int border, const float* scale, void* hi, void* lo,
                         void* stream);
int dtk_conv_split_run(const void* in_hi, const void* in_lo, const void* Wh, const void* Wl, float* out_nhwc, int N, int H, int W,
                       int Cin, int Cout, int dilation, int zero_pad, int fp16_only, void* stream);
int dtk_conv_split_output(const float* y_nhwc, int N, int C, int H, int W, int border, int reflect_fold, const float* scale,
                          float* out_nchw, void* stream);

size_t dtk_conv_wgrad_split_workspace_bytes(int N, int Cin, int Cout, int H, int W, int dilation);
int dtk_conv_wgrad_split(const float* x, const float* dy, float* dw, int N, int Cin, int Cout, int H, int W, int dilation,
                         int reflect_pad, const float* scale_dy, int fp16_only, void* workspace, size_t workspace_bytes,
                         void* stream);

size_t dtk_contrastive_workspace_bytes(int Q, int B, int C, int n);
int dtk_contrastive_forward(const float* fe, const float* a, const int32_t* fidx, float temp, int Q, int B, int C, int n, int F,
                            float* fet, float* nf, float* na, float* S, float* lse, void* stream);
int dtk_contrastive_backward(const float* fe, const float* a, const int32_t* fidx, float temp, int Q, int B, int C, int n, int F,
                             const float* nf, const float* na, const float* S, const float* lse, const float* g, float* da,
                             float* dfe, void* workspace, size_t workspace_bytes, void* stream);

int dtk_emb_reg_forward(const float* x, const float* raw, int F, int C, int n, float* cell_sums, float* out2, void* stream);
int dtk_emb_reg_backward(const float* x, const float* raw, const float* cell_sums, const float* grad_out2, int F, int C, int n,
                         float* dx, void* stream);

int dtk_corr_window_backward(const dtk_geom* g, const float* feat, const float* norms, const float* emb, const int32_t* tgt,
                             const float* maps, const float* dmaps, const float* stats, float* demb, float* dfeat, int B,
                             void* stream);

int dtk_normalized_conv2d(const float* x, const float* w, const float* bias, float* y, int B, int Cin, int Cout, int H,
                          int W, int k, void* stream);

int dtk_corr_maps(const dtk_geom* g, const float* feat, const float* norms, const float* emb, const int32_t* src_row,
                  const int32_t* tgt, float* maps, float* snorm_scratch, int M, int relu, void* stream);

#define DTK_TRACK_EXACT 0
#define DTK_TRACK_MFMA 1
#define DTK_TIER_AUTO 0
#define DTK_TIER_WHOLE_MAP 1
typedef struct dtk_track_opts {
    int32_t method, normalized, round_sources, tier;
    int32_t emb_rows;
} dtk_track_opts;
typedef struct dtk_track_stats {
    int32_t sources;
    int32_t whole_map_tier;
    int32_t exact_tier;
    int32_t syncs;
} dtk_track_stats;
size_t dtk_track_workspace_bytes(const dtk_geom* g, int M, const dtk_track_opts* opts);
int dtk_track(const dtk_geom* g, const float* feat, const float* norms, const void* feat_f16,
              const float* head, const float* emb, const int32_t* src_row, const int32_t* tgt,
              const int32_t* out_idx, float* out_xy, int M, const int32_t* dM, const dtk_track_opts* opts,
              dtk_track_stats* stats, void* workspace, size_t workspace_bytes, void* stream);

int dtk_argmax_cells(const dtk_geom* g, const float* feat, const float* norms, const void* feat_f16, const float* emb,
                     const int32_t* src_row, const int32_t* tgt, int32_t* arg_cell, float* arg_cos, int M, int method,
                     void* workspace, size_t workspace_bytes, void* stream);

size_t dtk_bb_nms_workspace_bytes(const dtk_geom* g, int M);
int dtk_bb_nms(const dtk_geom* g, const float* feat, const float* norms, const float* emb, const int32_t* src_row,
               const int32_t* tgt, float box_size, float iou_thresh, int topk, float* peak_affs, float* r, int M,
               void* workspace, size_t workspace_bytes, void* stream);

int dtk_traj_start_fg(const float* traj, int N, int T, const uint8_t* masks, int Tm, int H, int W, uint8_t* fg, int32_t* err,
                      void* stream);

size_t dtk_nearest_traj_workspace_bytes(int N, int T, int gh, int gw);
int dtk_nearest_traj(const float* traj, int N, int T, int gh, int gw, float origin, float stride, int32_t* idx,
                     void* workspace, size_t workspace_bytes, void* stream);

int dtk_of_filter_keep(const float* traj, int N, int T, const int32_t* idx, int gh, int gw, float origin, float stride,
                       const float* src, const float* tgt, const int32_t* pair_off, const int32_t* pair_st, int P,
                       uint8_t* keep, int32_t* err, void* stream);

size_t dtk_feat_f16_bytes(const dtk_geom* g);
int dtk_make_feat_f16(const dtk_geom* g, const float* feat, const float* norms, void* feat_f16, void* stream);

int dtk_traj_cos_sims(const float* S, const int32_t* tq, float* cs, int N, int T, int C, void* stream);

int dtk_build_anchor_sources(const float* cs, float anchor_th, int N, int T, int32_t* n_anchors, int32_t* pair_off,
                             int32_t* pair_frame, int32_t* src_row, int32_t* tgt, int32_t* out_idx,
                             int32_t* counts, int32_t* scratch, void* stream);

int dtk_build_anchor_sources_needed(const float* cs, float anchor_th, float cos_th, int N, int T, int32_t* n_anchors,
                                    int32_t* pair_off, int32_t* pair_frame, int32_t* src_row, int32_t* tgt, int32_t* out_idx,
                                    int32_t* counts, int32_t* scratch, void* stream);

int dtk_occlusion(const float* green, const int32_t* pair_off, const int32_t* pair_frame, const float* traj,
                  const float* cs, float anchor_th, float cos_th, uint8_t* occ, int N, int T, void* stream);

int dtk_occlusion_needed(const float* green, const int32_t* pair_off, const int32_t* pair_frame, const float* traj,
                         const float* cs, float anchor_th, float cos_th, uint8_t* occ, int N, int T, void* stream);

int dtk_tapvid_counts(const float* pred_tracks, const uint8_t* pred_occluded, const float* gt_tracks,
                      const uint8_t* gt_occluded, const int32_t* query_frame, float pred_scale_x, float pred_scale_y,
                      float gt_scale_x, float gt_scale_y, int first_mode, int N, int T, unsigned long long* counts18,
                      void* stream);

int dtk_badja_counts(const float* pred_tracks, const double* gt_tracks, const uint8_t* gt_occluded, const void* segmentations,
                     int32_t seg_is_float, float pred_scale_x, float pred_scale_y, int32_t N, int32_t T, int32_t T_seg,
                     int32_t H, int32_t W, unsigned long long* areas, unsigned long long* counts3, void* stream);

size_t dtk_batchnorm_workspace_bytes(int32_t C);
int dtk_batchnorm_train_forward(const float* x, const float* gamma, const float* beta, const float* pre_bias,
                                float* running_mean, float* running_var, float momentum, float eps, int32_t relu, float* y,
                                float* save_mean, float* save_rstd, int32_t N, int32_t C, int32_t HW, void* workspace,
                                size_t workspace_bytes, void* stream);
int dtk_batchnorm_train_backward(const float* x, const float* dy, const float* gamma, const float* beta,
                                 const float* save_mean, const float* save_rstd, int32_t relu, float* dx, float* dgamma,
                                 float* dbeta, float* dpre_bias, int32_t N, int32_t C, int32_t HW, void* workspace,
                                 size_t workspace_bytes, void* stream);

int dtk_blurpool_forward(const float* x, float* y, int64_t planes, int32_t H, int32_t W, void* stream);
int dtk_blurpool_backward(const float* dy, float* dx, int64_t planes, int32_t H, int32_t W, void* stream);

int dtk_gemm_nt_f32(const float* A, const float* B, float* C, int32_t M, int32_t N, int32_t K, int64_t lda, int64_t ldb,
                    int64_t ldc, int32_t batch, int64_t stride_a, int64_t stride_b, int64_t stride_c, int32_t split_k,
                    int32_t accumulate, const float* scale_a, const float* scale_b, void* stream);
int dtk_gemm_nt_f32_indexed(const float* A, const float* B, float* C, int32_t M, int32_t N, int32_t K, int64_t lda, int64_t ldb,
                            int64_t ldc, int32_t batch, int64_t stride_a, int64_t stride_b, int64_t stride_c, int32_t split_k,
                            int32_t accumulate, const float* scale_a, const float* scale_b, const int32_t* index_b,
                            const int32_t* index_c, void* stream);
int dtk_im2col(const float* x, float* cols, int32_t n, int32_t C, int32_t H, int32_t W, int32_t ksize, int32_t pad, int32_t dil,
               int32_t reflect, int32_t layout, int32_t Kp, int64_t Lp, void* stream);
int dtk_col2im(const float* dcols, float* dx, int32_t n, int32_t C, int32_t H, int32_t W, int32_t ksize, int32_t pad, int32_t dil,
               int32_t reflect, int32_t Kp, void* stream);
int dtk_transpose_f32(const float* src, float* dst, int64_t rows, int64_t cols, int32_t batch, void* stream);

int dtk_resample2d_forward(const float* src, float* dst, int64_t planes, int32_t hs, int32_t ws, int32_t hd, int32_t wd,
                           const int32_t* ylo, const float* ywhi, const int32_t* xlo, const float* xwhi, void* stream);
int dtk_resample2d_backward(const float* ddst, float* dsrc, int64_t planes, int32_t hs, int32_t ws, int32_t hd, int32_t wd,
                            const int32_t* yranges, const float* ywhi, const int32_t* xranges, const float* xwhi, void* stream);

int dtk_sample_bilinear_forward(const float* feat, const float* pts, float* out, int32_t B, int32_t n, int32_t h, int32_t w, int32_t C,
                                void* stream);
int dtk_sample_bilinear_backward(const float* g, const float* pts, float* dfeat, int32_t B, int32_t n, int32_t h, int32_t w, int32_t C,
                                 void* stream);

int dtk_pow2_scale(const float* x, int64_t n, float* out, void* scratch, void* stream);

#define DTK_ADAM_MAX_TENSORS 32
#define DTK_ADAM_MAX_GROUPS 4
typedef struct dtk_adam_args {
    float* param[DTK_ADAM_MAX_TENSORS];
    const float* grad[DTK_ADAM_MAX_TENSORS];
    float* exp_avg[DTK_ADAM_MAX_TENSORS];
    float* exp_avg_sq[DTK_ADAM_MAX_TENSORS];
    int64_t numel[DTK_ADAM_MAX_TENSORS];
    int32_t group[DTK_ADAM_MAX_TENSORS];
    int32_t step[DTK_ADAM_MAX_TENSORS];
    int32_t n_tensors;
    double lr[DTK_ADAM_MAX_GROUPS];
    double beta1, beta2, eps;
} dtk_adam_args;
int dtk_adam_step(const dtk_adam_args* a, void* stream);
int dtk_adam_scalars(const dtk_adam_args* a, float* out_host);
int dtk_adam_step_dev(const dtk_adam_args* a, const float* scalars_dev, void* stream);

size_t dtk_pca_moments_workspace_bytes(int64_t N, int32_t C, int64_t chunk_rows);
int dtk_pca_moments(const float* x, int64_t N, int32_t C, int32_t normalize, int64_t chunk_rows, float* mean, float* cov,
                    void* workspace, size_t workspace_bytes, void* stream);
size_t dtk_pca_project_workspace_bytes(int64_t N);
int dtk_pca_project(const float* x, int64_t N, int32_t C, int32_t normalize, const float* V, int32_t q, float* colors,
                    float* minmax, void* workspace, size_t workspace_bytes, void* stream);
int dtk_fg_mask(const float* colors, int32_t q, int32_t comp, const float* minmax, float thr, int32_t flip, int32_t T, int32_t h,
                int32_t w, int32_t H, int32_t W, uint8_t* mask, uint8_t* token_mask, void* stream);

int dtk_flow_pack(const float* flow, float* packed, int32_t n, int32_t h, int32_t w, void* stream);
int dtk_flow_cycle_masks(const float* fflow_packed, const float* bflow_packed, int32_t T, int32_t h, int32_t w, float threshold,
                         uint8_t* consistent, void* stream);
size_t dtk_flow_traj_workspace_bytes(int32_t T, int32_t h, int32_t w);
int dtk_flow_traj_start(const float* fflow_packed, const float* bflow_packed, const uint8_t* consistent, const uint8_t* visited,
                        int32_t T, int32_t h, int32_t w, int32_t s, float threshold, int32_t min_trajectory_length,
                        const float* direct_fwd, const float* direct_back, int32_t use_direct, float direct_threshold,
                        int32_t* n_rows, void* workspace, size_t workspace_bytes, void* stream);
int dtk_flow_traj_emit(int32_t T, int32_t h, int32_t w, int32_t s, int32_t min_trajectory_length, int32_t n_rows, float* rows,
                       uint8_t* visited, const void* workspace, size_t workspace_bytes, void* stream);

#define DTK_RENDER_SEGMENT 0
#define DTK_RENDER_DISC 1
#define DTK_RENDER_DIAMOND 2
#define DTK_RENDER_RING 3
#define DTK_RENDER_DOTTED 0
#define DTK_RENDER_TAILS 1
#define DTK_RENDER_RECORD_WORDS 12
#define DTK_RENDER_TILE 16
#define DTK_RENDER_CHUNK 256
int64_t dtk_render_prim_count(int32_t mode, int32_t N, int32_t f0, int32_t F);
size_t dtk_render_group_bytes(int64_t prims, int64_t keys, int32_t F, int32_t H, int32_t W);
int dtk_render_prims(const float* points, const uint8_t* occluded, const float* maps, const float* colors, int32_t N, int32_t T,
                     int32_t f0, int32_t F, int32_t H, int32_t W, int32_t mode, int32_t marker_kind, float marker_size,
                     float half_width, int32_t trail_fade, float* records, void* stream);
int dtk_render_pred_gt_prims(const int32_t* pred_xy, const int32_t* gt_xy, const uint8_t* pred_occluded,
                             const uint8_t* gt_occluded, const float* colors, int32_t N, int32_t T, int32_t f0, int32_t F,
                             int32_t thickness, int32_t radius, int32_t cross_size, float* records, void* stream);
int dtk_render_tile_counts(const float* records, int64_t P, int32_t F, int32_t H, int32_t W, int32_t* counts, void* stream);
int dtk_render_tile_keys(const float* records, const int64_t* offsets, int64_t P, int32_t F, int32_t H, int32_t W, int64_t K,
                         int64_t* keys, void* stream);
int dtk_render_blend(const uint8_t* frames_in, const float* records, int64_t P, const int64_t* sorted_keys, int64_t K,
                     const int64_t* tile_start, int32_t F, int32_t H, int32_t W, uint8_t* out_u8, float* out_f32, void* stream);

#define DTK_RESIZE_OUT_U8_HWC 0
#define DTK_RESIZE_OUT_F32_CHW 1
#define DTK_RESIZE_FORCE_GENERAL 1
#define DTK_RESIZE_TILE_H 32
#define DTK_RESIZE_TILE_W 64
size_t dtk_resize_workspace_bytes(int32_t N, int32_t H, int32_t W, int32_t C, int32_t h, int32_t w, int32_t ksize_y,
                                  int32_t options);
int dtk_resize_u8(const uint8_t* in, int32_t N, int32_t H, int32_t W, int32_t C, int32_t h, int32_t w, const int32_t* kx,
                  const int32_t* bx, int32_t ksize_x, const int32_t* ky, const int32_t* by, int32_t ksize_y,
                  const float* u8_to_f32, int32_t out_form, int32_t options, void* out, void* workspace, size_t workspace_bytes,
                  void* stream);

#define DTK_RAFT_SPLIT 0
#define DTK_RAFT_FP16 1
#define DTK_RAFT_ACT_NONE 0
#define DTK_RAFT_ACT_RELU 1
#define DTK_RAFT_ACT_SIGMOID 2
#define DTK_RAFT_ACT_TANH 3
#define DTK_RAFT_FEATURE 0
#define DTK_RAFT_CONTEXT 16
#define DTK_RAFT_CONTEXT_HIDDEN 31
#define DTK_RAFT_CONTEXT_CONTEXT 32
#define DTK_RAFT_MOTION 33
#define DTK_RAFT_GRU 38
#define DTK_RAFT_FLOW_HEAD 44
#define DTK_RAFT_MASK 46
#define DTK_RAFT_NUM_CONVS 48
typedef struct dtk_raft_conv_desc {
    const void* w_hi;
    const void* w_lo;
    const float* bias;
    int32_t cin, cout, kh, kw, stride, pad_h, pad_w;
    float inv_wscale;
} dtk_raft_conv_desc;
typedef struct dtk_raft_conv_args {
    dtk_raft_conv_desc conv;
    int32_t N, H, W, mode, act, res_relu, in_split, reserved;
    const float* in;
    const float* in2;
    float* out;
    const float* res;
    const float* mul;
    const float* gate;
    int64_t in_stride, in2_stride, out_stride, res_stride, mul_stride, gate_stride;
} dtk_raft_conv_args;
typedef struct dtk_raft_model {
    dtk_raft_conv_desc conv[DTK_RAFT_NUM_CONVS];
} dtk_raft_model;
size_t dtk_raft_conv_packed_halves(int32_t cout, int32_t cin, int32_t kh, int32_t kw);
int dtk_raft_conv_pack(const float* w, int32_t cout, int32_t cin, int32_t kh, int32_t kw, float wscale, void* w_hi, void* w_lo,
                       void* stream);
int dtk_raft_conv(const dtk_raft_conv_args* args, void* stream);
size_t dtk_raft_instance_norm_workspace_bytes(int32_t N, int32_t H, int32_t W, int32_t C);
int dtk_raft_instance_norm(const float* x, const float* res, float* out, int32_t N, int32_t H, int32_t W, int32_t C, float eps,
                           int32_t relu, void* workspace, size_t workspace_bytes, void* stream);
size_t dtk_raft_pyramid_floats(int32_t N, int32_t h, int32_t w);
int dtk_raft_corr_pyramid(const float* f1, const float* f2, int32_t N, int32_t h, int32_t w, int32_t C, int32_t mode, float* pyramid,
                          void* stream);
int dtk_raft_lookup(const float* pyramid, const float* flow, int64_t flow_stride, int32_t N, int32_t h, int32_t w, float* out,
                    int64_t out_stride, void* stream);
int dtk_raft_upsample(const float* flow, int64_t flow_stride, const float* mask, int32_t N, int32_t h, int32_t w, float* out,
                      void* stream);
size_t dtk_raft_workspace_bytes(int32_t N, int32_t H, int32_t W);
int dtk_raft_forward(const dtk_raft_model* model, const float* image1, const float* image2, int32_t N, int32_t H, int32_t W,
                     int32_t num_flow_updates, int32_t mode, float* flow_out, void* workspace, size_t workspace_bytes, void* stream);

#ifdef __cplusplus
}
#endif
#endif
```

Before: 536,900 query-points*frames/s.

## Store V row-major from QKV GEMM and transpose-read it in attention

The weight-stationary QKV GEMM epilogue now writes V in the same row-major per-head layout as Q and K, skipping the transposed V^T store path. Attention6 gains a VROWS variant that DMAs V rows into LDS and uses ds_read_b64_tr_b16 transposing LDS reads with pinned AGPR fragments to feed the PV MFMAs. The safe fallback pass reads V row-major element by element. The aim is to remove the cost of the transposed V store in the GEMM epilogue, in exchange for more LDS-read instructions and register pinning in the attention inner loop. It is on by default, and an env flag restores the old transposed layout.

Result: no change. 540,500 query-points*frames/s (median of 6 runs) (+0.7%).

```diff
diff --git a/dino_tracker_amd/_lib.py b/dino_tracker_amd/_lib.py
--- a/dino_tracker_amd/_lib.py
+++ b/dino_tracker_amd/_lib.py
@@ -42,8 +42,11 @@
 
 
 VIT_TILED_GEMMS, VIT_BF16, VIT_CHECK_RANGE, VIT_GEMM_WS_V1, VIT_ATTENTION_V4, VIT_GEMM_WIDE_V1, VIT_NO_LN_FUSION = 1, 2, 4, 16, 32, 64, 128
+VIT_V_TRANSPOSED = 256
 OPERAND_F16, OPERAND_BF16, OPERAND_ATTENTION_V4 = 0, 1, 0x2000
+OPERAND_V_ROWS = 0x4000
 VIT_GEMM_QKV, VIT_GEMM_QKV_FACET, VIT_GEMM_PROJ, VIT_GEMM_FC1, VIT_GEMM_FC2 = 0, 1, 2, 3, 4
+VIT_GEMM_QKV_VROWS = 7
 VIT_GEMM_FC1_SWIGLU, VIT_GEMM_FC2_SWIGLU = 5, 6
 VIT_FFN_GELU, VIT_FFN_SWIGLU = 0, 1
 
diff --git a/dino_tracker_amd/csrc/vit.hip b/dino_tracker_amd/csrc/vit.hip
--- a/dino_tracker_amd/csrc/vit.hip
+++ b/dino_tracker_amd/csrc/vit.hip
@@ -319,9 +319,15 @@
 }
 
 template <typename T>
-int attention_launch(const T* q, const T* k, const T* vt, T* o, int S, int Sp, int heads, int D, int FH, bool v4, hipStream_t st) {
+int attention_launch(const T* q, const T* k, const T* vt, T* o, int S, int Sp, int heads, int D, int FH, bool v4, bool v_rows,
+                     hipStream_t st) {
     int QB;
-    if (v4) {
+    DTK_REQUIRE(!(v4 && v_rows), "vit_attention: row-major V is attention6's (not with ATTENTION_V4)");
+    if (v_rows) {
+        const unsigned grid = attn::attention_grid(FH, S, 128 * attn::A6_NQ, &QB);
+        DTK_LAUNCH("vit_attention", (attn::attention6_kernel<T, 0, true>), dim3(grid), dim3(256), 0, st, q, k, vt, o, S, Sp, heads, D,
+                   FH, QB);
+    } else if (v4) {
         const unsigned grid = attn::attention_grid(FH, S, 256, &QB);
         DTK_LAUNCH("vit_attention", (attn::attention4_kernel<T, 0>), dim3(grid), dim3(256), 0, st, q, k, vt, o, S, Sp, heads, D,
                    FH, QB);
@@ -383,6 +389,9 @@
     return {tiled, ws, !tiled && D % W2_N == 0, ws_v1, wide_v1, fc2_ln, fc2_ln && !ws_v1};
 }
 inline GemmPath gemm_path(const dtk_vit_model* m) { return gemm_path(m->D, m->flags); }
+inline bool vit_v_rows(const GemmPath& path, int f, int S, long long rows) {
+    return path.ws && !path.ws_v1 && !(f & (DTK_VIT_ATTENTION_V4 | DTK_VIT_V_TRANSPOSED)) && (S >= WS_ROWS || rows <= S);
+}
 
 template <typename T, int EPI>
 int launch_gemm(const char* name, const GemmPath& path, const T* A, const T* W, long long rows, int N, int K, const GemmEpi<T>& e,
@@ -396,6 +405,9 @@
                 return DTK_OK;
             }
         }
+        if (EPI == EPI_QKV && e.v_rows)
+            DTK_REQUIRE(path.ws && !path.ws_v1 && K == WS_K && ws_fits && N % 64 == 0 && !DTK_DBG(e.no_store, 128),
+                        "%s: row-major V needs the hand-cut weight-stationary QKV GEMM (D = 384, none of TILED_GEMMS / GEMM_WS_V1, S >= 32 or one frame)", name);
         if (path.ws && K == WS_K && ws_fits) {
             const auto gr = gemm_ws_grid(N, rows);
             if (path.ws_v1)
@@ -514,6 +526,7 @@
                        x, video_h, video_w, ph, pw, D, m->patch, m->stride, S);
         }
         const GemmPath path = gemm_path(m);
+        const bool v_rows = vit_v_rows(path, m->flags, S, rows) && !DTK_DBG(dtk_dev_flags() >> 16, 128);
         const int dbg_ns = DTK_DBG(dtk_dev_flags() >> 16, 0xff);
         bool pending = false;
         bool ln1_done = false;
@@ -578,10 +591,10 @@
                 e = GemmEpi<T>{};
             }
             e.bias = L.qkv_b; e.q = q; e.k = k; e.vt = vt; e.S = S; e.Sp = Sp; e.heads = m->heads; e.D = D;
-            e.qscale = 0.125f * 1.4426950408889634f; e.no_store = dbg_ns; e.ovf = epi_ovf;
+            e.qscale = 0.125f * 1.4426950408889634f; e.no_store = dbg_ns; e.ovf = epi_ovf; e.v_rows = v_rows;
             if (launch_gemm<T, EPI_QKV>("vit_gemm_qkv", path, xn, qkv_w, rows, 3 * D, D, e, st)) return DTK_E_HIP;
             if (scan_all && scan_range(q, (long long)(p.ao - p.q) / 2, 2)) return DTK_E_HIP;
-            if (attention_launch(q, k, vt, ao, S, Sp, m->heads, D, nf * m->heads, (m->flags & DTK_VIT_ATTENTION_V4) != 0, st)) return DTK_E_HIP;
+            if (attention_launch(q, k, vt, ao, S, Sp, m->heads, D, nf * m->heads, (m->flags & DTK_VIT_ATTENTION_V4) != 0, v_rows, st)) return DTK_E_HIP;
             e = GemmEpi<T>{};
             e.bias = L.proj_b; e.delta = delta; e.gamma = L.ls1; e.no_store = dbg_ns;
             if (path.proj_ln) { e.ln_x = x; e.ln_w = L.ln2_w; e.ln_b = L.ln2_b; e.ln_out = xn; e.ln_eps = m->ln_eps; e.ln_ovf = ovf; }
@@ -634,6 +647,13 @@
     DTK_REQUIRE(g->a && g->w && (!split || (g->a_lo && g->w_lo)), "%s: null operand", who);
     const int D = g->D;
     switch (g->role) {
+        case DTK_VIT_GEMM_QKV_VROWS:
+            DTK_REQUIRE(!split, "%s: QKV_VROWS: the split blocks keep V^T", who);
+            DTK_REQUIRE(D == WS_K && !(g->flags & (DTK_VIT_TILED_GEMMS | DTK_VIT_GEMM_WS_V1)),
+                        "%s: QKV_VROWS is the hand-cut weight-stationary GEMM's: D = 384 without TILED_GEMMS / GEMM_WS_V1 (got D = %d, flags 0x%x)",
+                        who, D, (unsigned)g->flags);
+            DTK_REQUIRE(g->S >= WS_ROWS || g->rows <= g->S, "%s: QKV_VROWS needs S >= %d or a single frame", who, WS_ROWS);
+            [[fallthrough]];
         case DTK_VIT_GEMM_QKV:
             *N = 3 * D; *K = D;
             DTK_REQUIRE(g->q && g->k && g->vt && (!split || (g->q_lo && g->k_lo && g->vt_lo)), "%s: QKV needs q, k and vt", who);
@@ -680,8 +700,10 @@
     e.bias = g->bias;
     switch (g->role) {
         case DTK_VIT_GEMM_QKV:
+        case DTK_VIT_GEMM_QKV_VROWS:
             e.q = reinterpret_cast<T*>(g->q); e.k = reinterpret_cast<T*>(g->k); e.vt = reinterpret_cast<T*>(g->vt);
             e.S = g->S; e.Sp = g->Sp; e.heads = g->D / 64; e.D = g->D; e.qscale = 0.125f * 1.4426950408889634f; e.ovf = epi_ovf;
+            e.v_rows = g->role == DTK_VIT_GEMM_QKV_VROWS;
             return launch_gemm<T, EPI_QKV>("vit_gemm_qkv", path, A, W, g->rows, N, K, e, st);
         case DTK_VIT_GEMM_QKV_FACET:
             e.out_f32 = g->out_f32;
@@ -736,7 +758,7 @@
 }
 
 constexpr int VIT_KNOWN_FLAGS = DTK_VIT_TILED_GEMMS | DTK_VIT_BF16 | DTK_VIT_CHECK_RANGE | DTK_VIT_GEMM_WS_V1 | DTK_VIT_ATTENTION_V4 |
-                                DTK_VIT_GEMM_WIDE_V1 | DTK_VIT_NO_LN_FUSION;
+                                DTK_VIT_GEMM_WIDE_V1 | DTK_VIT_NO_LN_FUSION | DTK_VIT_V_TRANSPOSED;
 
 }
 
@@ -783,16 +805,17 @@
                                  int Sp, int operand_type, void* stream) {
     DTK_REQUIRE(q && k && vt && out, "dtk_vit_attention: null pointer");
     DTK_REQUIRE(frames > 0 && heads > 0 && S > 0 && Sp >= S && Sp % 64 == 0, "dtk_vit_attention: bad sizes (Sp %% 64 == 0, Sp >= S)");
-    const bool v4 = (operand_type & DTK_OPERAND_ATTENTION_V4) != 0;
-    operand_type &= ~DTK_OPERAND_ATTENTION_V4;
+    const bool v4 = (operand_type & DTK_OPERAND_ATTENTION_V4) != 0, v_rows = (operand_type & DTK_OPERAND_V_ROWS) != 0;
+    DTK_REQUIRE(!(v4 && v_rows), "dtk_vit_attention: DTK_OPERAND_V_ROWS is attention6's layout: not together with DTK_OPERAND_ATTENTION_V4");
+    operand_type &= ~(DTK_OPERAND_ATTENTION_V4 | DTK_OPERAND_V_ROWS);
     DTK_REQUIRE(operand_type == DTK_OPERAND_F16 || operand_type == DTK_OPERAND_BF16, "dtk_vit_attention: operand_type");
     if (operand_type == DTK_OPERAND_BF16)
         return attention_launch(reinterpret_cast<const __bf16*>(q), reinterpret_cast<const __bf16*>(k),
                                 reinterpret_cast<const __bf16*>(vt), reinterpret_cast<__bf16*>(out), S, Sp, heads, heads * 64,
-                                frames * heads, v4, dtk_stream(stream));
+                                frames * heads, v4, v_rows, dtk_stream(stream));
     return attention_launch(reinterpret_cast<const _Float16*>(q), reinterpret_cast<const _Float16*>(k),
                             reinterpret_cast<const _Float16*>(vt), reinterpret_cast<_Float16*>(out), S, Sp, heads, heads * 64,
-                            frames * heads, v4, dtk_stream(stream));
+                            frames * heads, v4, v_rows, dtk_stream(stream));
 }
 
 extern "C" int dtk_vit_attention_split(const void* q_hi, const void* q_lo, const void* k_hi, const void* k_lo, const void* vt_hi,
diff --git a/dino_tracker_amd/csrc/vit_attention6.h b/dino_tracker_amd/csrc/vit_attention6.h
--- a/dino_tracker_amd/csrc/vit_attention6.h
+++ b/dino_tracker_amd/csrc/vit_attention6.h
@@ -26,7 +26,46 @@
     asm volatile("ds_read_b128 %0, %1 offset:%2" : "=a"(dst) : "v"(addr), "i"(OFF) : "memory");
 }
 
-template <typename T, int ABL = 0>
+#define A6_VF_CASES(X) X(0, "224:225", "226:227", "224:227") X(1, "228:229", "230:231", "228:231") X(2, "232:233", "234:235", "232:235") \
+    X(3, "236:237", "238:239", "236:239") X(4, "240:241", "242:243", "240:243") X(5, "244:245", "246:247", "244:247")                 \
+    X(6, "248:249", "250:251", "248:251") X(7, "252:253", "254:255", "252:255")
+template <int OFF, typename V8>
+__device__ __forceinline__ void a6_lds_frag_tr(int j, V8& dst, unsigned addr) {
+    typedef __typeof__(__builtin_shufflevector(dst, dst, 0, 1, 2, 3)) V4;
+    V4 lo, hi;
+    switch (j) {
+#define A6_X(J, LO, HI, QUAD)                                                                                       \
+    case J:                                                                                                         \
+        asm volatile("ds_read_b64_tr_b16 %0, %2 offset:%3\n\tds_read_b64_tr_b16 %1, %2 offset:%4"                   \
+                     : "={a[" LO "]}"(lo), "={a[" HI "]}"(hi) : "v"(addr), "i"(OFF), "i"(OFF + 512) : "memory");    \
+        break;
+        A6_VF_CASES(A6_X)
+#undef A6_X
+    }
+    dst = __builtin_shufflevector(lo, hi, 0, 1, 2, 3, 4, 5, 6, 7);
+}
+template <typename T>
+__device__ __forceinline__ void a6_pv_pinned(int j, f16v& c, const typename Operand<T>::v8& a, const typename Operand<T>::v8& b) {
+    switch (j) {
+#define A6_X(J, LO, HI, QUAD)                                                                                                         \
+    case J:                                                                                                                           \
+        if constexpr (Operand<T>::F16) asm volatile("v_mfma_f32_32x32x16_f16 %0, %1, %2, %0" : "+a"(c) : "{a[" QUAD "]}"(a), "v"(b)); \
+        else asm volatile("v_mfma_f32_32x32x16_bf16 %0, %1, %2, %0" : "+a"(c) : "{a[" QUAD "]}"(a), "v"(b));                          \
+        break;
+        A6_VF_CASES(A6_X)
+#undef A6_X
+    }
+}
+template <typename V8>
+__device__ __forceinline__ void a6_vf_pin(int j, V8& v) {
+    switch (j) {
+#define A6_X(J, LO, HI, QUAD) case J: asm volatile("" : "+{a[" QUAD "]}"(v)); break;
+        A6_VF_CASES(A6_X)
+#undef A6_X
+    }
+}
+
+template <typename T, int ABL = 0, bool VROWS = false>
 __global__ __launch_bounds__(256, 1) void attention6_kernel(const T* __restrict__ Q, const T* __restrict__ Kg,
                                                             const T* __restrict__ Vt, T* __restrict__ O, int S, int Sp,
                                                             int heads, int D, int FH, int QB) {
@@ -73,7 +112,7 @@
     for (int r = 0; r < 2; ++r) {
         const int lrow = (w * 2 + r) * 8 + (lane >> 3), lpc = (lane & 7) ^ ((lrow >> 1) & 7);
         kvo[r] = (unsigned)(lrow * 64 + lpc * 8) * 2u;
-        vvo[r] = (unsigned)(lrow * Sp + lpc * 8) * 2u;
+        vvo[r] = VROWS ? (unsigned)(lrow * 64 + ((lane & 7) ^ (((lrow >> 1) & 1) << 2)) * 8) * 2u : (unsigned)(lrow * Sp + lpc * 8) * 2u;
     }
     const unsigned lds_base = (unsigned)(size_t)&tiles[0][0];
     const int ntiles = (S + 63) / 64;
@@ -85,7 +124,7 @@
         constexpr int BUF = decltype(buf_tag)::value;
         const unsigned tt = (unsigned)min(t, ntiles - 1);
         if (i < 2) dtk_buffer_lds16<BUF * TILE_BYTES>(srd_k, tt * 8192u, kvo[i & 1], dma_dst[i]);
-        else dtk_buffer_lds16<BUF * TILE_BYTES>(srd_v, tt * 128u, vvo[i & 1], dma_dst[i]);
+        else dtk_buffer_lds16<BUF * TILE_BYTES>(srd_v, VROWS ? tt * 8192u : tt * 128u, vvo[i & 1], dma_dst[i]);
     };
 #pragma unroll
     for (int j = 0; j < 4; ++j) {
@@ -157,7 +196,8 @@
     for (int g = 0; g < 8; ++g) {
 #pragma unroll
         for (int e = 0; e < 8; ++e) vf[g][e] = (T)0.f;
-        asm volatile("" : "+a"(vf[g]));
+        if constexpr (VROWS) a6_vf_pin(g, vf[g]);
+        else asm volatile("" : "+a"(vf[g]));
     }
     const int krow = (lq & 19) | ((lq & 4) << 1) | ((lq & 8) >> 1);
     unsigned ka[4], va[4];
@@ -168,6 +208,12 @@
         for (int j = 0; j < 4; ++j) {
             ka[j] = lds_base + (koff0 ^ (j << 5));
             va[j] = lds_base + (voff0 ^ (j << 5));
+        }
+        if constexpr (VROWS) {
+            const int q = (lane & 15) >> 2, p = lane & 3, pc = 2 * ((lane >> 4) & 1) + (p >> 1);
+#pragma unroll
+            for (int db = 0; db < 2; ++db)
+                va[db] = lds_base + 8192 + (8 * hi + q) * 128 + (((4 * db + pc) ^ ((q >> 1) << 2)) << 4) + 8 * (p & 1);
         }
     }
 #pragma unroll
@@ -254,11 +300,17 @@
                 if (j < 2) a6_s_first<T>(sc[SET][j & 1], kf[j], qf[U][j >> 1], negm[U]);
                 else a6_s_next<T>(sc[SET][j & 1], kf[j], qf[U][j >> 1]);
             } else {
-                a6_pv<T>(o[U][j & 1], vf[j], __builtin_bit_cast(op8, pf[U][j >> 1]));
+                if constexpr (VROWS) a6_pv_pinned<T>(j, o[U][j & 1], vf[j], __builtin_bit_cast(op8, pf[U][j >> 1]));
+                else a6_pv<T>(o[U][j & 1], vf[j], __builtin_bit_cast(op8, pf[U][j >> 1]));
             }
             if (!(ABL & 128) && REFILL) {
                 if (i & 1) {
-                    if (j & 1) a6_lds_frag<VB * TILE_BYTES + 4096>(vf[j], va[j >> 1]);
+                    if constexpr (VROWS) {
+                        if ((j >> 1) == 0) a6_lds_frag_tr<VB * TILE_BYTES>(j, vf[j], va[j & 1]);
+                        else if ((j >> 1) == 1) a6_lds_frag_tr<VB * TILE_BYTES + 2048>(j, vf[j], va[j & 1]);
+                        else if ((j >> 1) == 2) a6_lds_frag_tr<VB * TILE_BYTES + 4096>(j, vf[j], va[j & 1]);
+                        else a6_lds_frag_tr<VB * TILE_BYTES + 6144>(j, vf[j], va[j & 1]);
+                    } else if (j & 1) a6_lds_frag<VB * TILE_BYTES + 4096>(vf[j], va[j >> 1]);
                     else a6_lds_frag<VB * TILE_BYTES>(vf[j], va[j >> 1]);
                 } else {
                     if (j & 1) a6_lds_frag<KB * TILE_BYTES + 4096>(kf[j], ka[j >> 1]);
@@ -292,7 +344,8 @@
     };
     auto key_tile = [&](auto vb_tag, int t) {
         dtk_vm_wait<4>();
-        asm volatile("s_waitcnt lgkmcnt(8)" ::: "memory");
+        if constexpr (VROWS) asm volatile("s_waitcnt lgkmcnt(12)" ::: "memory");
+        else asm volatile("s_waitcnt lgkmcnt(8)" ::: "memory");
         if (!(ABL & 16)) __syncthreads();
         sub_step(std::integral_constant<int, 0>{}, vb_tag, t);
         sub_step(std::integral_constant<int, 1>{}, vb_tag, t);
@@ -321,14 +374,18 @@
         lsum[NQ - 1] = lta;
         pend[NQ - 1] = (ABL & 8) ? 0 : (__builtin_amdgcn_ballot_w64(!(lta < Op::RESC_T)) != 0ull);
         asm volatile("s_nop 4" ::: "memory");
-#pragma unroll
-        for (int g = 0; g < 8; ++g) a6_pv<T>(o[0][g & 1], vf[g], __builtin_bit_cast(op8, pf[0][g >> 1]));
-#pragma unroll
-        for (int g = 0; g < 8; ++g) a6_pv<T>(o[1][g & 1], vf[g], __builtin_bit_cast(op8, pf[1][g >> 1]));
-#pragma unroll
-        for (int g = 0; g < 8; ++g) a6_pv<T>(o[2][g & 1], vf[g], __builtin_bit_cast(op8, pf[2][g >> 1]));
-#pragma unroll
-        for (int g = 0; g < 8; ++g) a6_pv<T>(o[3][g & 1], vf[g], __builtin_bit_cast(op8, pf[3][g >> 1]));
+        auto pv_last = [&](int g, f16v& c, const dtk_u4& p) {
+            if constexpr (VROWS) a6_pv_pinned<T>(g, c, vf[g], __builtin_bit_cast(op8, p));
+            else a6_pv<T>(c, vf[g], __builtin_bit_cast(op8, p));
+        };
+#pragma unroll
+        for (int g = 0; g < 8; ++g) pv_last(g, o[0][g & 1], pf[0][g >> 1]);
+#pragma unroll
+        for (int g = 0; g < 8; ++g) pv_last(g, o[1][g & 1], pf[1][g >> 1]);
+#pragma unroll
+        for (int g = 0; g < 8; ++g) pv_last(g, o[2][g & 1], pf[2][g >> 1]);
+#pragma unroll
+        for (int g = 0; g < 8; ++g) pv_last(g, o[3][g & 1], pf[3][g >> 1]);
     }
     if (pend[0]) guard_tripped(std::integral_constant<int, 0>{}, std::integral_constant<int, 0>{}, lsum[0], false);
     if (pend[1]) guard_tripped(std::integral_constant<int, 1>{}, std::integral_constant<int, 0>{}, lsum[1], false);
@@ -346,7 +403,7 @@
         redo |= __any(!(l_tot[qt] > Op::LOW_T && l_tot[qt] < 0x1p120f));
     }
     if (redo && !(ABL & 8)) {
-        safe_pass<T, 6>(Qb, Kb, Vb, O + (size_t)frame * S * D + head * 64, q0, 32 * NQ, S, Sp, D);
+        safe_pass<T, 6, VROWS>(Qb, Kb, Vb, O + (size_t)frame * S * D + head * 64, q0, 32 * NQ, S, Sp, D);
         return;
     }
 #pragma unroll
diff --git a/dino_tracker_amd/csrc/vit_attention_common.h b/dino_tracker_amd/csrc/vit_attention_common.h
--- a/dino_tracker_amd/csrc/vit_attention_common.h
+++ b/dino_tracker_amd/csrc/vit_attention_common.h
@@ -40,7 +40,7 @@
     hi_all = __uint_as_float(r1);
 }
 
-template <typename T>
+template <typename T, bool VROWS = false>
 __device__ __forceinline__ void safe_pass_impl(const T* Qb, const T* Kb, const T* Vb, T* Ob, int q0, int nq, int S, int Sp,
                                                int D) {
     typedef Operand<T> Op;
@@ -104,7 +104,13 @@
                 }
 #pragma unroll
                 for (int db = 0; db < 2; ++db) {
-                    const op8 vf = *reinterpret_cast<const op8*>(Vb + (size_t)(db * 32 + lq) * Sp + t * 64 + bj * 16 + hi * 8);
+                    op8 vf;
+                    if constexpr (VROWS) {
+#pragma unroll
+                        for (int e = 0; e < 8; ++e) vf[e] = Vb[(size_t)(t * 64 + bj * 16 + hi * 8 + e) * 64 + db * 32 + lq];
+                    } else {
+                        vf = *reinterpret_cast<const op8*>(Vb + (size_t)(db * 32 + lq) * Sp + t * 64 + bj * 16 + hi * 8);
+                    }
                     oa[db] = Op::mfma(vf, pfr, oa[db]);
                 }
             }
@@ -126,9 +132,9 @@
         }
     }
 }
-template <typename T, int TAG>
+template <typename T, int TAG, bool VROWS = false>
 __device__ __noinline__ void safe_pass(const T* Qb, const T* Kb, const T* Vb, T* Ob, int q0, int nq, int S, int Sp, int D) {
-    safe_pass_impl(Qb, Kb, Vb, Ob, q0, nq, S, Sp, D);
+    safe_pass_impl<T, VROWS>(Qb, Kb, Vb, Ob, q0, nq, S, Sp, D);
 }
 
 template <typename T>
diff --git a/dino_tracker_amd/csrc/vit_gemm_common.h b/dino_tracker_amd/csrc/vit_gemm_common.h
--- a/dino_tracker_amd/csrc/vit_gemm_common.h
+++ b/dino_tracker_amd/csrc/vit_gemm_common.h
@@ -35,6 +35,7 @@
     T* q;
     T* k;
     T* vt;
+    int v_rows;
     int S, Sp, heads, D;
     float qscale;
     T* out;
diff --git a/dino_tracker_amd/csrc/vit_gemm_ws.h b/dino_tracker_amd/csrc/vit_gemm_ws.h
--- a/dino_tracker_amd/csrc/vit_gemm_ws.h
+++ b/dino_tracker_amd/csrc/vit_gemm_ws.h
@@ -165,7 +165,7 @@
                     up = e.vt + (((size_t)f0 * e.heads + head) * 64) * e.Sp + s0;
                     cross = (unsigned)(e.heads * 64 * e.Sp - e.S);
                 } else {
-                    up = (which == 0 ? e.q : e.k) + (((size_t)f0 * e.heads + head) * e.Sp + s0) * 64;
+                    up = (which == 0 ? e.q : which == 1 ? e.k : e.vt) + (((size_t)f0 * e.heads + head) * e.Sp + s0) * 64;
                     cross = (unsigned)((e.heads * e.Sp - e.S) * 64);
                 }
             }
@@ -350,7 +350,7 @@
             tail_flush(valid);
         };
         if constexpr (EPI == EPI_QKV) {
-            if (which == 2) run(Yes{});
+            if (which == 2 && !e.v_rows) run(Yes{});
             else run(No{});
         } else {
             run(No{});
diff --git a/dino_tracker_amd/extractor.py b/dino_tracker_amd/extractor.py
--- a/dino_tracker_amd/extractor.py
+++ b/dino_tracker_amd/extractor.py
@@ -10,7 +10,7 @@
 import torch.nn.functional as F
 
 from . import ops
-from ._lib import VIT_FFN_SWIGLU, VIT_ATTENTION_V4, VIT_GEMM_WIDE_V1, VIT_GEMM_WS_V1, VIT_NO_LN_FUSION, VIT_BF16, VIT_CHECK_RANGE, VIT_TILED_GEMMS, VitLayer, VitModel, check, lib
+from ._lib import VIT_FFN_SWIGLU, VIT_V_TRANSPOSED, VIT_ATTENTION_V4, VIT_GEMM_WIDE_V1, VIT_GEMM_WS_V1, VIT_NO_LN_FUSION, VIT_BF16, VIT_CHECK_RANGE, VIT_TILED_GEMMS, VitLayer, VitModel, check, lib
 from .synth import VIT_CONFIGS, make_vit_weights
 
 IMAGENET_MEAN = (0.485, 0.456, 0.406)
@@ -44,6 +44,7 @@
         self.attention_v4 = os.environ.get("DTK_VIT_ATTENTION_V4", "0") == "1"
         self.gemm_ws_v1 = False
         self.no_ln_fusion = os.environ.get("DTK_VIT_NO_LN_FUSION", "0") == "1"
+        self.v_transposed = os.environ.get("DTK_VIT_V_TRANSPOSED", "0") == "1"
         self.gemm_wide_v1 = os.environ.get("DTK_VIT_GEMM_WIDE_V1", "0") == "1"
         self.frame_batch = 0
         if model_name not in VIT_CONFIGS:
@@ -218,7 +219,7 @@
             flags = (VIT_TILED_GEMMS if self.tiled_gemms else 0) | (VIT_BF16 if operand_dtype == "bf16" else 0) | \
                 (VIT_CHECK_RANGE if self.check_range else 0) | (VIT_ATTENTION_V4 if self.attention_v4 else 0) | \
                 (VIT_GEMM_WS_V1 if self.gemm_ws_v1 else 0) | (VIT_GEMM_WIDE_V1 if self.gemm_wide_v1 else 0) | \
-                (VIT_NO_LN_FUSION if self.no_ln_fusion else 0)
+                (VIT_NO_LN_FUSION if self.no_ln_fusion else 0) | (VIT_V_TRANSPOSED if self.v_transposed else 0)
             m = VitModel(D, self.cfg["heads"], layer + 1, patch, self.stride, 1e-6, flags,
                          self._sd["patch_embed.proj.weight"].data_ptr(),
                          self._sd["patch_embed.proj.bias"].data_ptr(), cls_pos.data_ptr(), pos.data_ptr(), ms.data_ptr(),
diff --git a/include/dtk.h b/include/dtk.h
--- a/include/dtk.h
+++ b/include/dtk.h
@@ -85,9 +85,11 @@
 #define DTK_VIT_ATTENTION_V4 32
 #define DTK_VIT_NO_LN_FUSION 128
 #define DTK_VIT_GEMM_WIDE_V1 64
+#define DTK_VIT_V_TRANSPOSED 256
 #define DTK_OPERAND_F16 0
 #define DTK_OPERAND_BF16 1
 #define DTK_OPERAND_ATTENTION_V4 0x2000
+#define DTK_OPERAND_V_ROWS 0x4000
 
 size_t dtk_vit_workspace_bytes(const dtk_vit_model* m, int video_h, int video_w, int frames);
 int dtk_vit_forward(const dtk_vit_model* m, const float* frames, int nframes, int video_h, int video_w,
@@ -107,6 +109,7 @@
 #define DTK_VIT_GEMM_FC2 4
 #define DTK_VIT_GEMM_FC1_SWIGLU 5
 #define DTK_VIT_GEMM_FC2_SWIGLU 6
+#define DTK_VIT_GEMM_QKV_VROWS 7
 typedef struct dtk_vit_gemm_args {
     int32_t role, D, flags, operand_type;
     int64_t rows;
```
